# wen-yuan-zhang/Fast-Learning-NeRF

Measured on AMD Instinct MI355X. Metric: training rays/sec (Lego-like 800x800, 64+128 samples) + PSNR@N-iters, higher is better.
Workload: dtype f32; 1 GPU; nerf-ours Lego full 800x800 (BASELINE configs[1]), SURVEY 8(d) throughput protocol: 4096 uniformly drawn rays per GPU per step, 64+128 samples, use_viewdirs, white_bkgd, perturb=1, U[0,1) targets, random-init nets, leaf-error table on, fp32-width bf16x6 kernels, plain backward (FASTNERF_COMPACT=0); parallelism=dp1, math_mode=bf16x6, backward=plain (every sample)

## Files before the change

### fast-learning-nerf_amd/_lib.py

```python
import ctypes as C
import os

import torch

HERE = os.path.dirname(os.path.abspath(__file__))
LIB_PATH = os.environ.get('FASTNERF_LIB') or os.path.join(HERE, 'libfastnerf.so')

P = C.c_void_p
I = C.c_int
L = C.c_int64
F = C.c_float
D = C.c_double
U64 = C.c_uint64



class StepArgs(C.Structure):
    _fields_ = (
        [('n', L)] + [(k, P) for k in ('rays_o', 'rays_d', 'target', 't_rand', 'u', 'noise0', 'noise1')]
        + [('seed0', U64), ('seed1', U64), ('leaf_tag', P), ('table', P), ('net_floats', L)]
        + [(k, P) for k in ('params', 'grads', 'adam_m', 'adam_v', 'packed_fwd_c', 'packed_bwd_c', 'packed_fwd_f', 'packed_bwd_f',
                            'rays11', 'z0', 'raw0', 'act0', 'rgb0', 'disp0', 'acc0', 'w0', 'depth0',
                            'z1', 'z_samples', 'z_std', 'raw1', 'act1', 'rgb1', 'disp1', 'acc1', 'w1', 'depth1',
                            'g_rgb', 'g_rgb0', 'loss2', 'draw_ws', 'act_ws', 'dact_ws', 'partial_ws', 'live_ws', 'counts')]
        + [(k, D) for k in ('focal', 'lr', 'beta1', 'beta2', 'eps')]
        + [(k, F) for k in ('near_plane', 'far_plane', 'grad_scale')]
        + [(k, I) for k in ('math_mode', 'N_samples', 'N_importance', 'lindisp', 'perturb', 'white_bkgd', 'ndc', 'H', 'W', 'live',
                            'fwd_flags', 'max_leaves', 'adam_t')]
        + [('occ', P), ('occ_counts', P)])


class MapGrads(C.Structure):
    _fields_ = [(k, P) for k in ('g_disp1', 'g_acc1', 'g_depth1', 'g_disp0', 'g_acc0', 'g_depth0')]


class StepAux(C.Structure):
    _fields_ = ([(k, P) for k in ('depth_target', 'depth_weight', 'acc_target', 'acc_weight', 'g_depth1', 'g_acc1', 'g_depth0',
                                  'g_acc0', 'loss4')]
                + [('lambda_depth', F), ('lambda_acc', F)])


class OccGrid(C.Structure):
    _fields_ = [('words', P), ('lo', F * 3), ('inv', F * 3), ('n', C.c_int32 * 3), ('outside_occupied', C.c_int32)]


OCC_MAX_LEVELS = 8


class OccCascade(C.Structure):
    _fields_ = [('levels', C.c_int32), ('reserved', C.c_int32), ('level', OccGrid * OCC_MAX_LEVELS)]


STEP_FORWARD, STEP_BWD_FINE, STEP_BWD_COARSE, STEP_UPDATE = 1, 2, 4, 8

SIGNATURES = {
    'fastnerf_version': (I, []),
    'fastnerf_last_error': (C.c_char_p, []),
    'fastnerf_device_cus': (I, []),
    'fastnerf_x6_pair_launches': (L, []),
    'fastnerf_gen_rays': (I, [I, I, F, F, F, F, P, P, P, P]),
    'fastnerf_gen_rays_pixels': (I, [L, P, P, F, F, F, F, P, P, P]),
    'fastnerf_ndc_rays': (I, [L, I, I, D, F, P, P, P, P, P]),
    'fastnerf_pack_rays': (I, [L, P, P, F, F, I, I, I, D, P, P]),
    'fastnerf_sample_coarse': (I, [L, I, P, I, I, P, U64, P, P]),
    'fastnerf_posenc': (I, [L, I, P, P, P]),
    'fastnerf_mlp_pack': (I, [P, P, P, P]),
    'fastnerf_mlp_fwd': (I, [L, I, P, P, P, P, P, P, P]),
    'fastnerf_mlp_bwd_partial_floats': (L, []),
    'fastnerf_mlp_bwd': (I, [L, I, P, P, P, P, P, P, P, P]),
    'fastnerf_raw2outputs_fwd': (I, [L, I, P, P, P, P, I, P, P, P, P, P, P]),
    'fastnerf_raw2outputs_bwd': (I, [L, I, P, P, P, P, I, P, P, P]),
    'fastnerf_raw2outputs_bwd_full': (I, [L, I, P, P, P, P, I, P, P, P, P, P, P, P, P, P]),
    'fastnerf_sample_pdf_merge': (I, [L, I, I, P, P, I, P, U64, P, P, P, P]),
    'fastnerf_sample_pdf': (I, [L, I, I, P, P, I, P, U64, P, P]),
    'fastnerf_mse_leafmax': (I, [L, P, P, P, F, P, P, P, P, I, P, P]),
    'fastnerf_aux_loss': (I, [L] + [P] * 8 + [F, F, F] + [P] * 5 + [P]),
    'fastnerf_adam_step': (I, [L, P, P, P, P, D, D, D, D, I, P]),
    'fastnerf_net_floats': (L, [I, I]),
    'fastnerf_mlp_act_floats': (L, [I, L]),
    'fastnerf_mlp_pack_ex': (I, [I, P, P, P, P]),
    'fastnerf_mlp_fwd_ex': (I, [I, L, I, P, P, P, P, P, P, P]),
    'fastnerf_mlp_bwd_ex': (I, [I, L, I, P, P, P, P, P, P, P, P]),
    'fastnerf_mlp_bf16_floats': (L, [I, I, L]),
    'fastnerf_mlp_bf16_partial_floats': (L, []),
    'fastnerf_mlp_bf16_pack': (I, [I, P, P, P, P]),
    'fastnerf_mlp_bf16_fwd': (I, [I, L, I, P, P, P, P, P, P, P]),
    'fastnerf_mlp_bf16_bwd': (I, [I, L, I, P, P, P, P, P, P, P, P]),
    'fastnerf_render_rays_fwd': (I, [I, L, I, I, P, I, I, I, I, P, P, P, P, U64, U64, P, P, P, P] + [P] * 18 + [P]),
    'fastnerf_render_rays_fwd_ex': (I, [I, L, I, I, P, I, I, I, I, P, P, P, P, U64, U64, P, P, P, P] + [P] * 18 + [I, P]),
    'fastnerf_mlp_bf16_fwd_flags': (I, [I, L, I, P, P, P, P, P, I, P]),
    'fastnerf_mlp_fwd_flags_ex': (I, [I, L, I, P, P, P, P, P, I, P]),
    'fastnerf_render_rays_bwd': (I, [I, L, I, I, P, I] + [P] * 20),
    'fastnerf_render_rays_bwd_maps': (I, [I, L, I, I, P, I] + [P] * 19 + [P] * 4 + [C.POINTER(MapGrads), P]),
    'fastnerf_pp_intersect_sphere': (I, [L, P, P, P, P]),
    'fastnerf_pp_fg_depths': (I, [L, I, F, P, I, P, U64, P, P]),
    'fastnerf_pp_sample_pdf_merge': (I, [L, I, I, P, P, I, P, U64, P, P, P]),
    'fastnerf_pp_perturb_samples': (I, [L, I, P, P, U64, P, P]),
    'fastnerf_pp_sample_pdf': (I, [L, I, I, P, P, I, P, U64, P, P]),
    'fastnerf_pp_depth2pts_outside': (I, [L, I, P, P, P, P, P, P]),
    'fastnerf_pp_composite_fwd': (I, [L, I, I, P, P, P, P, P, P, P, P, P]),
    'fastnerf_pp_composite_bwd': (I, [L, I, I, P, P, P, P, P, P, P, P]),
    'fastnerf_pp_gen_rays': (I, [I, I, P, P, P, P, P]),
    'fastnerf_leaf_sumcount': (I, [L, P, P, P, I, P, P, P]),
    'fastnerf_tree_adjust_mean': (L, [P, P, P, I, D]),
    'fastnerf_tree_create': (P, [I, I, I, I]),
    'fastnerf_tree_destroy': (None, [P]),
    'fastnerf_tree_num_leaves': (I, [P, I]),
    'fastnerf_tree_max_leaves': (I, [P]),
    'fastnerf_tree_min_area': (D, [P, I]),
    'fastnerf_tree_get_leaves': (I, [P, I, P]),
    'fastnerf_tree_set_leaves': (I, [P, I, I, P, D]),
    'fastnerf_tree_leaf_plan': (I, [P, I, D, I, P]),
    'fastnerf_tree_adjust': (L, [P, P, I, D]),
    'fastnerf_tree_epoch_plan': (L, [P, D, I, P, P]),
    'fastnerf_epoch_rays': (I, [L, I, P, P, P, P, I, I, I, F, F, F, F, U64, I] + [P] * 10 + [P]),
    'fastnerf_epoch_rays_shard': (I, [L, I, P, P, P, P, I, I, I, F, F, F, F, U64, I] + [P] * 5 + [L, I, I] + [P] * 5 + [P]),
    'fastnerf_epoch_shard_rows': (L, [L, L, I, I]),
    'fastnerf_gauss_noise': (I, [L, F, U64, P, P]),
    'fastnerf_compact_ws_ints': (L, [L]),
    'fastnerf_compact_live': (I, [L, P, P, P, P, P]),
    'fastnerf_mlp_bf16_fwd_live': (I, [I, L, I, P, P, P, P, P, P, P, P]),
    'fastnerf_mlp_bf16_bwd_live': (I, [I, L, I, P, P, P, P, P, P, P, P, P, P]),
    'fastnerf_mlp_fwd_live_ex': (I, [I, L, I, P, P, P, P, P, P, P, P]),
    'fastnerf_mlp_bwd_live_ex': (I, [I, L, I, P, P, P, P, P, P, P, P, P, P]),
    'fastnerf_render_rays_bwd_live': (I, [I, L, I, I, P, I] + [P] * 22 + [P]),
    'fastnerf_render_rays_bwd_live_maps': (I, [I, L, I, I, P, I] + [P] * 22 + [P] * 4 + [C.POINTER(MapGrads), P]),
    'fastnerf_mlp_x6_packed_floats': (L, [I, I]),
    'fastnerf_mlp_x6_pack': (I, [I, P, P, P, P]),
    'fastnerf_mlp_fold_offset': (L, [I, I]),
    'fastnerf_mlp_x6_fwd': (I, [I, L, I, P, P, P, P, P, P, I, P]),
    'fastnerf_mlp_x6_bwd': (I, [I, L, I, P, P, P, P, P, P, P, P]),
    'fastnerf_mlp_x6_fwd_live': (I, [I, L, I, P, P, P, P, P, P, P, P]),
    'fastnerf_mlp_x6_bwd_live': (I, [I, L, I, P, P, P, P, P, P, P, P, P, P]),
    'fastnerf_step_args_size': (L, []),
    'fastnerf_train_step': (I, [C.POINTER(StepArgs), I, P]),
    'fastnerf_step_aux_size': (L, []),
    'fastnerf_train_step_aux': (I, [C.POINTER(StepArgs), C.POINTER(StepAux), I, P]),
    'fastnerf_comm_unique_id': (I, [C.c_char_p]),
    'fastnerf_comm_init': (I, [C.POINTER(P), C.c_char_p, I, I]),
    'fastnerf_comm_destroy': (I, [P]),
    'fastnerf_allreduce_grads': (I, [P, P, L, C.c_float, P]),
    'fastnerf_allreduce_leaf_table': (I, [P, P, L, P]),
    'fastnerf_allreduce_leaf_sumcount': (I, [P, P, P, L, P]),
    'fastnerf_leaf_table_reset': (I, [P, L, P]),
    'fastnerf_leaf_table_read': (I, [P, P, L, P]),
    'fastnerf_grid_points': (I, [L, L, P, L, P, L, P, L, P, P]),
    'fastnerf_grid_sigma': (I, [L, P, P, P]),
    'fastnerf_mc_ws_bytes': (L, [L, L, L]),
    'fastnerf_mc_count': (I, [P, L, L, L, F, P, P, P]),
    'fastnerf_mc_emit': (I, [P, L, L, L, F, P, P, P, P]),
    'fastnerf_mc_tables': (I, [P, P]),
    'fastnerf_occ_words': (L, [L, L, L]),
    'fastnerf_occ_build': (I, [P, L, L, L, F, I, P, P, P]),
    'fastnerf_occ_from_mask': (I, [P, L, L, L, P, P]),
    'fastnerf_occ_query': (I, [C.POINTER(OccGrid), L, P, P, P]),
    'fastnerf_occ_classify': (I, [C.POINTER(OccGrid), L, I, P, P, P, P, P, P, P]),
    'fastnerf_occ_query_cascade': (I, [C.POINTER(OccCascade), L, P, P, P]),
    'fastnerf_occ_classify_cascade': (I, [C.POINTER(OccCascade), L, I, P, P, P, P, P, P, P]),
    'fastnerf_occ_cell_points': (I, [C.POINTER(OccGrid), L, L, U64, P, P]),
    'fastnerf_occ_update': (I, [P, P, L, L, L, L, L, F, F, I, P, P, P, P]),
    'fastnerf_mlp_fwd_list_ex': (I, [I, L, I, P, P, P, P, P, P, P, I, P]),
    'fastnerf_mlp_bf16_fwd_list': (I, [I, L, I, P, P, P, P, P, P, P, I, P]),
    'fastnerf_mlp_x6_fwd_list': (I, [I, L, I, P, P, P, P, P, P, P, I, P]),
    'fastnerf_render_rays_fwd_occ': (I, [I, L, I, I, P, I, I, I, I, P, P, U64, U64, P, P, P, P, C.POINTER(OccGrid), P, P] + [P] * 16 + [I, P]),
    'fastnerf_render_rays_fwd_occ_cascade': (I, [I, L, I, I, P, I, I, I, I, P, P, U64, U64, P, P, P, P, C.POINTER(OccCascade), P, P] + [P] * 16 + [I, P]),
    'fastnerf_ert_classify': (I, [C.POINTER(OccGrid), C.POINTER(OccCascade), L, I, I, I, P, P, P, F, P, P, P, P, P]),
    'fastnerf_ert_advance': (I, [L, I, I, I, P, P, P, I, P, P, P, P]),
    'fastnerf_render_rays_fwd_ert': (I, [I, L, I, I, P, I, I, I, I, P, P, U64, U64, P, P, P, P, C.POINTER(OccGrid), C.POINTER(OccCascade), F, I,
                                         P, P, P] + [P] * 16 + [I, P]),
    'fastnerf_mlp_sigma_grad_ws_floats': (L, [I, L]),
    'fastnerf_mlp_sigma_grad': (I, [I, I, L, I, P, P, P, P, P, P, P, P, P]),
    'fastnerf_ray_grad_ws_floats': (L, [I, L, I]),
    'fastnerf_ray_grad': (I, [I, I, L, I, P, P, P, P, P, P, P, P, P, I, P, P]),
}

_lib = None


def lib():
    global _lib
    if _lib is None:
        if not os.path.exists(LIB_PATH):
            raise RuntimeError(
                f'{LIB_PATH} not found: build it with `python -c "import __graft_entry__ as g; g.build()"` '
                '(the HIP path has no CPU fallback)')
        l = C.CDLL(LIB_PATH)
        for name, (res, args) in SIGNATURES.items():
            fn = getattr(l, name)
            fn.restype = res
            fn.argtypes = args
        if l.fastnerf_step_args_size() != C.sizeof(StepArgs):
            raise RuntimeError('fn_step_args: the ctypes mirror does not match the library (stale libfastnerf.so?)')
        if l.fastnerf_step_aux_size() != C.sizeof(StepAux):
            raise RuntimeError('fn_step_aux: the ctypes mirror does not match the library (stale libfastnerf.so?)')
        _lib = l
    return _lib


def check(rc, what):
    if rc is None or rc < 0:
        msg = lib().fastnerf_last_error()
        raise RuntimeError(f'{what} failed ({rc}): {msg.decode() if msg else "?"}')
    return rc


def ptr(t):
    if t is None:
        return None
    assert t.is_contiguous(), 'tensor must be contiguous'
    return t.data_ptr()


def stream():
    return torch.cuda.current_stream().cuda_stream


def require_gpu(*tensors):
    for t in tensors:
        if t is not None and not t.is_cuda:
            raise RuntimeError('fastnerf ops run on the GPU only (no CPU fallback): got a CPU tensor')
```

### fast-learning-nerf_amd/csrc/composite.hip

```cpp
#include "common.h"

#define WAVE 64
#define MAXC 8

__device__ __forceinline__ float wave_sum(float v) {
#pragma unroll
  for (int o = 32; o > 0; o >>= 1) v += __shfl_xor(v, o, WAVE);
  return v;
}

__device__ __forceinline__ float wave_scan_mul(float v, int lane) {
#pragma unroll
  for (int o = 1; o < WAVE; o <<= 1) {
    float t = __shfl_up(v, o, WAVE);
    if (lane >= o) v *= t;
  }
  return v;
}
__device__ __forceinline__ float wave_suffix_add(float v, int lane) {
#pragma unroll
  for (int o = 1; o < WAVE; o <<= 1) {
    const float t = __shfl_down(v, o, WAVE);
    if (lane + o < WAVE) v += t;
  }
  const float above = __shfl_down(v, 1, WAVE);
  return lane == WAVE - 1 ? 0.0f : above;
}

__device__ __forceinline__ void wave_suffix_add2(float& a, float& b, int lane) {
#pragma unroll
  for (int o = 1; o < WAVE; o <<= 1) {
    const float ta = __shfl_down(a, o, WAVE), tb = __shfl_down(b, o, WAVE);
    if (lane + o < WAVE) {
      a += ta;
      b += tb;
    }
  }
  const float aa = __shfl_down(a, 1, WAVE), ab = __shfl_down(b, 1, WAVE);
  a = lane == WAVE - 1 ? 0.0f : aa;
  b = lane == WAVE - 1 ? 0.0f : ab;
}

__device__ __forceinline__ float sigmoidf(float x) { return 1.0f / (1.0f + expf(-x)); }

struct SampleVals {
  float alpha, t, dist, z, sig;
  float c[3];
};

struct CompCfg {
  int act_abs;
  float eps;
  int last_mode;
  int use_dnorm;
  int flip;
};
__device__ __forceinline__ CompCfg nerf_cfg() { return CompCfg{0, 1e-10f, 0, 1, 0}; }

template <bool WITH_RGB>
__device__ __forceinline__ void eval_chunk(int S, int C, int lane, const float* __restrict__ raw,
                                           const float* __restrict__ z, const float* __restrict__ noise, float dnorm,
                                           SampleVals v[MAXC], int& cnt, const CompCfg cfg, float far) {
  const int s0 = lane * C;
  cnt = 0;
#pragma unroll
  for (int j = 0; j < MAXC; ++j) {
    if (j >= C) break;
    const int s = s0 + j;
    if (s >= S) break;
    const float4 r = *reinterpret_cast<const float4*>(raw + (int64_t)s * 4);
    const float zs = cfg.flip ? z[S - 1 - s] : z[s];
    float dist;
    if (s + 1 < S) {
      const float zn = cfg.flip ? z[S - 2 - s] : z[s + 1];
      dist = cfg.flip ? fsub(zs, zn) : fsub(zn, zs);
    } else {
      dist = cfg.last_mode ? fsub(far, zs) : 1e10f;
    }
    if (cfg.use_dnorm) dist = fmul(dist, dnorm);
    float sig = r.w;
    if (noise) sig = fadd(sig, noise[s]);
    const float rs = cfg.act_abs ? fabsf(sig) : fmaxf(sig, 0.0f);
    const float alpha = fsub(1.0f, expf(-fmul(rs, dist)));
    v[j].alpha = alpha;
    v[j].t = fadd(fsub(1.0f, alpha), cfg.eps);
    v[j].dist = dist;
    v[j].z = zs;
    v[j].sig = sig;
    if (WITH_RGB) {
      v[j].c[0] = sigmoidf(r.x);
      v[j].c[1] = sigmoidf(r.y);
      v[j].c[2] = sigmoidf(r.z);
    }
    cnt = j + 1;
  }
}

__global__ void __launch_bounds__(256) raw2outputs_fwd_kernel(int64_t n, int S, const float* __restrict__ raw,
                                                               const float* __restrict__ z,
                                                               const float* __restrict__ rays,
                                                               const float* __restrict__ noise, int white,
                                                               float* __restrict__ rgb_map, float* __restrict__ disp,
                                                               float* __restrict__ acc, float* __restrict__ weights,
                                                               float* __restrict__ depth, const CompCfg cfg,
                                                               const float* __restrict__ far,
                                                               float* __restrict__ lambda) {
  const int lane = threadIdx.x & 63;
  const int C = (S + WAVE - 1) / WAVE;
  const int64_t wave0 = ((int64_t)blockIdx.x * blockDim.x + threadIdx.x) >> 6;
  const int64_t nwaves = ((int64_t)gridDim.x * blockDim.x) >> 6;
  for (int64_t r = wave0; r < n; r += nwaves) {
    const float* rr = rays + r * 11;
    const float dnorm = sqrtf(fadd(fadd(fmul(rr[3], rr[3]), fmul(rr[4], rr[4])), fmul(rr[5], rr[5])));
    SampleVals v[MAXC];
    int cnt;
    eval_chunk<true>(S, C, lane, raw + r * S * 4, z + r * S, noise ? noise + r * S : nullptr, dnorm, v, cnt, cfg,
                     far ? far[r] : 0.f);
    float prod = 1.0f;
#pragma unroll
    for (int j = 0; j < MAXC; ++j)
      if (j < cnt) prod *= v[j].t;
    const float incl = wave_scan_mul(prod, lane);
    float T = __shfl_up(incl, 1, WAVE);
    if (lane == 0) T = 1.0f;
    if (lambda) {
      const float tot = __shfl(incl, WAVE - 1, WAVE);
      if (lane == 0) lambda[r] = tot;
    }
    float sr = 0.f, sg = 0.f, sb = 0.f, sd = 0.f, sa = 0.f;
#pragma unroll
    for (int j = 0; j < MAXC; ++j) {
      if (j < cnt) {
        const float w = v[j].alpha * T;
        if (weights) weights[r * S + lane * C + j] = w;
        sr += w * v[j].c[0];
        sg += w * v[j].c[1];
        sb += w * v[j].c[2];
        sd += w * v[j].z;
        sa += w;
        T *= v[j].t;
      }
    }
    sr = wave_sum(sr); sg = wave_sum(sg); sb = wave_sum(sb); sd = wave_sum(sd); sa = wave_sum(sa);
    if (lane == 0) {
      if (white) {
        const float bg = fsub(1.0f, sa);
        sr = fadd(sr, bg); sg = fadd(sg, bg); sb = fadd(sb, bg);
      }
      rgb_map[r * 3 + 0] = sr; rgb_map[r * 3 + 1] = sg; rgb_map[r * 3 + 2] = sb;
      if (disp) {
        const float q = sd / sa;
        disp[r] = (q != q) ? q : 1.0f / fmaxf(1e-10f, q);
      }
      if (acc) acc[r] = sa;
      if (depth) depth[r] = sd;
    }
  }
}

__global__ void __launch_bounds__(256) raw2outputs_bwd_kernel(int64_t n, int S, const float* __restrict__ raw,
                                                               const float* __restrict__ z,
                                                               const float* __restrict__ rays,
                                                               const float* __restrict__ noise, int white,
                                                               const float* __restrict__ g_rgb,
                                                               float* __restrict__ draw, const CompCfg cfg,
                                                               const float* __restrict__ far,
                                                               const float* __restrict__ g_lambda) {
  const int lane = threadIdx.x & 63;
  const int C = (S + WAVE - 1) / WAVE;
  const int64_t wave0 = ((int64_t)blockIdx.x * blockDim.x + threadIdx.x) >> 6;
  const int64_t nwaves = ((int64_t)gridDim.x * blockDim.x) >> 6;
  for (int64_t r = wave0; r < n; r += nwaves) {
    const float* rr = rays + r * 11;
    const float dnorm = sqrtf(fadd(fadd(fmul(rr[3], rr[3]), fmul(rr[4], rr[4])), fmul(rr[5], rr[5])));
    const float g0 = g_rgb[r * 3], g1 = g_rgb[r * 3 + 1], g2 = g_rgb[r * 3 + 2];
    const float gbg = white ? (g0 + g1 + g2) : 0.0f;
    SampleVals v[MAXC];
    int cnt;
    eval_chunk<true>(S, C, lane, raw + r * S * 4, z + r * S, noise ? noise + r * S : nullptr, dnorm, v, cnt, cfg,
                     far ? far[r] : 0.f);
    float prod = 1.0f;
#pragma unroll
    for (int j = 0; j < MAXC; ++j)
      if (j < cnt) prod *= v[j].t;
    const float incl = wave_scan_mul(prod, lane);
    float T0 = __shfl_up(incl, 1, WAVE);
    if (lane == 0) T0 = 1.0f;
    const float lam_term = g_lambda ? g_lambda[r] * __shfl(incl, WAVE - 1, WAVE) : 0.0f;
    float w[MAXC], G[MAXC], Tj[MAXC];
    float gw_chunk = 0.f;
    float T = T0;
#pragma unroll
    for (int j = 0; j < MAXC; ++j) {
      if (j < cnt) {
        Tj[j] = T;
        w[j] = v[j].alpha * T;
        G[j] = g0 * v[j].c[0] + g1 * v[j].c[1] + g2 * v[j].c[2] - gbg;
        gw_chunk += G[j] * w[j];
        T *= v[j].t;
      }
    }
    float suffix = wave_suffix_add(gw_chunk, lane);
    float4 out[MAXC];
#pragma unroll
    for (int j = MAXC - 1; j >= 0; --j) {
      if (j < cnt) {
        const float dalpha = G[j] * Tj[j] - (suffix + lam_term) / v[j].t;
        const float dact = dalpha * v[j].dist * (1.0f - v[j].alpha);
        const float dsig = cfg.act_abs ? ((v[j].sig > 0.0f) ? dact : ((v[j].sig < 0.0f) ? -dact : 0.0f))
                                       : ((v[j].sig > 0.0f) ? dact : 0.0f);
        out[j].x = g0 * w[j] * v[j].c[0] * (1.0f - v[j].c[0]);
        out[j].y = g1 * w[j] * v[j].c[1] * (1.0f - v[j].c[1]);
        out[j].z = g2 * w[j] * v[j].c[2] * (1.0f - v[j].c[2]);
        out[j].w = dsig;
        suffix += G[j] * w[j];
      }
    }
#pragma unroll
    for (int j = 0; j < MAXC; ++j)
      if (j < cnt) *reinterpret_cast<float4*>(draw + (r * S + lane * C + j) * 4) = out[j];
  }
}

__global__ void __launch_bounds__(256) raw2outputs_bwd_full_kernel(
    int64_t n, int S, const float* __restrict__ raw, const float* __restrict__ z, const float* __restrict__ rays,
    const float* __restrict__ noise, int white, const float* __restrict__ acc_f, const float* __restrict__ depth_f,
    const float* __restrict__ g_rgb, const float* __restrict__ g_disp, const float* __restrict__ g_acc,
    const float* __restrict__ g_w, const float* __restrict__ g_depth, float* __restrict__ draw) {
  const CompCfg cfg = nerf_cfg();
  const int lane = threadIdx.x & 63;
  const int C = (S + WAVE - 1) / WAVE;
  const int64_t wave0 = ((int64_t)blockIdx.x * blockDim.x + threadIdx.x) >> 6;
  const int64_t nwaves = ((int64_t)gridDim.x * blockDim.x) >> 6;
  const bool ray_terms = g_acc || g_depth || g_disp;
  for (int64_t r = wave0; r < n; r += nwaves) {
    const float* rr = rays + r * 11;
    const float dnorm = sqrtf(fadd(fadd(fmul(rr[3], rr[3]), fmul(rr[4], rr[4])), fmul(rr[5], rr[5])));
    const float g0 = g_rgb ? g_rgb[r * 3] : 0.0f, g1 = g_rgb ? g_rgb[r * 3 + 1] : 0.0f, g2 = g_rgb ? g_rgb[r * 3 + 2] : 0.0f;
    const float gbg = white ? (g0 + g1 + g2) : 0.0f;
    const float ga0 = g_acc ? g_acc[r] : 0.0f, gd0 = g_depth ? g_depth[r] : 0.0f;
    float ga = ga0, gd = gd0;
    float kd = 0.0f;
    if (g_disp) {
      const float gq = g_disp[r];
      if (gq != 0.0f) {
        const float a = acc_f[r], dep = depth_f[r], q = dep / a;
        if (q != q) {
          ga = q; gd = q;
        } else if (q >= 1e-10f) {
          const float disp = 1.0f / q;
          const float gqe = q == 1e-10f ? 0.5f * gq : gq;
          const float k = gqe * disp / a;
          ga += k;
          gd -= k * disp;
          kd = gqe / dep / dep;
        }
      }
    }
    const float zlast = ray_terms ? z[r * S + S - 1] : 0.0f;
    SampleVals v[MAXC];
    int cnt;
    eval_chunk<true>(S, C, lane, raw + r * S * 4, z + r * S, noise ? noise + r * S : nullptr, dnorm, v, cnt, cfg, 0.f);
    float prod = 1.0f;
#pragma unroll
    for (int j = 0; j < MAXC; ++j)
      if (j < cnt) prod *= v[j].t;
    const float incl = wave_scan_mul(prod, lane);
    float T0 = __shfl_up(incl, 1, WAVE);
    if (lane == 0) T0 = 1.0f;
    float zprev = 0.0f;
#pragma unroll
    for (int j = 0; j < MAXC; ++j)
      if (j < cnt) zprev = v[j].z;
    zprev = __shfl_up(zprev, 1, WAVE);
    float w[MAXC], G[MAXC], Tj[MAXC], h[MAXC];
    float gw_chunk = 0.f, h_chunk = 0.f, dlast = 0.f;
    float T = T0;
#pragma unroll
    for (int j = 0; j < MAXC; ++j) {
      if (j < cnt) {
        Tj[j] = T;
        w[j] = v[j].alpha * T;
        G[j] = g0 * v[j].c[0] + g1 * v[j].c[1] + g2 * v[j].c[2] - gbg;
        if (g_w) G[j] = G[j] + g_w[r * S + lane * C + j];
        gw_chunk += G[j] * w[j];
        if (ray_terms) {
          const float dz = v[j].z - zprev;
          h[j] = (ga * cfg.eps + gd * (dz + cfg.eps * v[j].z)) * T;
          h_chunk += h[j];
          zprev = v[j].z;
          dlast += w[j] * (zlast - v[j].z);
        }
        T *= v[j].t;
      }
    }
    float suffix = gw_chunk, suffix_h = h_chunk, end_term = 0.f;
    if (ray_terms)
      wave_suffix_add2(suffix, suffix_h, lane);
    else
      suffix = wave_suffix_add(gw_chunk, lane);
    if (ray_terms) {
      float coef = ga + gd * zlast;
      if (kd != 0.0f) coef = (ga0 + gd0 * zlast) - kd * wave_sum(dlast);
      end_term = coef * __shfl(incl, WAVE - 1, WAVE);
    }
    float4 out[MAXC];
#pragma unroll
    for (int j = MAXC - 1; j >= 0; --j) {
      if (j < cnt) {
        float dalpha;
        if (ray_terms) {
          dalpha = G[j] * Tj[j] - (suffix - (end_term - suffix_h)) / v[j].t;
          suffix_h += h[j];
        } else {
          dalpha = G[j] * Tj[j] - (suffix + 0.0f) / v[j].t;
        }
        const float dact = dalpha * v[j].dist * (1.0f - v[j].alpha);
        out[j].x = g0 * w[j] * v[j].c[0] * (1.0f - v[j].c[0]);
        out[j].y = g1 * w[j] * v[j].c[1] * (1.0f - v[j].c[1]);
        out[j].z = g2 * w[j] * v[j].c[2] * (1.0f - v[j].c[2]);
        out[j].w = (v[j].sig > 0.0f) ? dact : 0.0f;
        suffix += G[j] * w[j];
      }
    }
#pragma unroll
    for (int j = 0; j < MAXC; ++j)
      if (j < cnt) *reinterpret_cast<float4*>(draw + (r * S + lane * C + j) * 4) = out[j];
  }
}

__device__ __forceinline__ int lower_bound_f(const float* a, int n, float x) {
  int lo = 0, hi = n;
  while (lo < hi) {
    const int mid = (lo + hi) >> 1;
    if (a[mid] < x) lo = mid + 1; else hi = mid;
  }
  return lo;
}
__device__ __forceinline__ int upper_bound_f(const float* a, int n, float x) {
  int lo = 0, hi = n;
  while (lo < hi) {
    const int mid = (lo + hi) >> 1;
    if (a[mid] <= x) lo = mid + 1; else hi = mid;
  }
  return lo;
}

__global__ void __launch_bounds__(256) sample_pdf_merge_kernel(int64_t n, int S, int Ni, int NP, int bins_mode,
                                                                int variant,
                                                                const float* __restrict__ z,
                                                                const float* __restrict__ weights, int det,
                                                                const float* __restrict__ u_in, uint64_t seed,
                                                                float* __restrict__ z_out,
                                                                float* __restrict__ z_samples,
                                                                float* __restrict__ z_std) {
  extern __shared__ __attribute__((aligned(16))) float smem[];
  const int lane = threadIdx.x & 63;
  const int wib = threadIdx.x >> 6;
  const int per_wave = 3 * S + NP;
  float* zs = smem + wib * per_wave;
  float* cdf = zs + S;
  float* bins = cdf + S;
  float* smp = bins + S;
  const int M = S - 1;
  const int NW = S - 2;
  const int CW = (NW + WAVE - 1) / WAVE;
  const int64_t wave0 = ((int64_t)blockIdx.x * blockDim.x + threadIdx.x) >> 6;
  const int64_t nwaves = ((int64_t)gridDim.x * blockDim.x) >> 6;
  for (int64_t r = wave0; r < n; r += nwaves) {
    if (bins_mode) {
      for (int k = lane; k < M; k += WAVE) bins[k] = z[r * M + k];
    } else {
      for (int s = lane; s < S; s += WAVE) zs[s] = z[r * S + s];
      __builtin_amdgcn_wave_barrier();
      for (int k = lane; k < M; k += WAVE) bins[k] = fmul(0.5f, fadd(zs[k + 1], zs[k]));
    }
    float wl[MAXC];
    double csum = 0.0;
#pragma unroll
    for (int j = 0; j < MAXC; ++j) {
      const int k = lane * CW + j;
      wl[j] = (j < CW && k < NW) ? fadd(bins_mode ? weights[r * NW + k] : weights[r * S + k + 1], variant ? 1e-6f : 1e-5f) : 0.f;
      csum += (double)wl[j];
    }
    double totd = csum;
#pragma unroll
    for (int o = 32; o > 0; o >>= 1) totd += __shfl_xor(totd, o, WAVE);
    const float tot = (float)totd;
    double run = 0.0;
#pragma unroll
    for (int j = 0; j < MAXC; ++j) {
      wl[j] = wl[j] / tot;
      run += (double)wl[j];
    }
    double incl = run;
#pragma unroll
    for (int o = 1; o < WAVE; o <<= 1) {
      const double t = __shfl_up(incl, o, WAVE);
      if (lane >= o) incl += t;
    }
    double base = incl - run;
    if (lane == 0) cdf[0] = 0.f;
#pragma unroll
    for (int j = 0; j < MAXC; ++j) {
      const int k = lane * CW + j;
      if (j < CW && k < NW) {
        base += (double)wl[j];
        cdf[k + 1] = (float)base;
      }
    }
    __builtin_amdgcn_wave_barrier();
    float lsum = 0.f;
    for (int i = lane; i < NP; i += WAVE) {
      float smpl = __builtin_inff();
      if (i < Ni) {
        float u;
        if (u_in) {
          u = u_in[r * Ni + i];
        } else if (det) {
          const float step = 1.0f / (float)(Ni - 1);
          u = (Ni == 1) ? 0.0f : ((i < Ni / 2) ? fmul(step, (float)i) : fsub(1.0f, fmul(step, (float)(Ni - 1 - i))));
        } else {
          uint32_t o[4];
          const uint64_t idx = (uint64_t)r * Ni + i;
          philox4x32((uint32_t)idx, (uint32_t)(idx >> 32), 0x70646673u, 0u, (uint32_t)seed, (uint32_t)(seed >> 32), o);
          u = u01(o[0]);
        }
        const int inds = upper_bound_f(cdf, variant ? NW : M, u);
        const int below = inds - 1 > 0 ? inds - 1 : 0;
        const int above = inds < M - 1 ? inds : M - 1;
        const float c0 = cdf[below], c1 = cdf[above];
        const float b0 = bins[below], b1 = bins[above];
        float denom = fsub(c1, c0);
        if (denom < (variant ? 1e-6f : 1e-5f)) denom = 1.0f;
        const float t = fsub(u, c0) / denom;
        smpl = variant ? fadd(b0, fmul(t, fadd(fsub(b1, b0), 1e-6f))) : fadd(b0, fmul(t, fsub(b1, b0)));
        if (z_samples) z_samples[r * Ni + i] = smpl;
        lsum += smpl;
      }
      smp[i] = smpl;
    }
    if (z_std) {
      const float mean = wave_sum(lsum) / (float)Ni;
      float lv = 0.f;
      for (int i = lane; i < Ni; i += WAVE) {
        const float d = smp[i] - mean;
        lv += d * d;
      }
      const float var = wave_sum(lv) / (float)Ni;
      if (lane == 0) z_std[r] = sqrtf(var);
    }
    __builtin_amdgcn_wave_barrier();
    if (bins_mode) continue;
    for (int k = 2; k <= NP; k <<= 1) {
      for (int j = k >> 1; j > 0; j >>= 1) {
        for (int i = lane; i < NP; i += WAVE) {
          const int ixj = i ^ j;
          if (ixj > i) {
            const float a = smp[i], b = smp[ixj];
            const bool up = ((i & k) == 0);
            if ((a > b) == up) { smp[i] = b; smp[ixj] = a; }
          }
        }
        __builtin_amdgcn_wave_barrier();
      }
    }
    const int So = S + Ni;
    for (int s = lane; s < S; s += WAVE) {
      const float x = zs[s];
      z_out[r * So + s + lower_bound_f(smp, Ni, x)] = x;
    }
    for (int i = lane; i < Ni; i += WAVE) {
      const float x = smp[i];
      z_out[r * So + i + upper_bound_f(zs, S, x)] = x;
    }
    __builtin_amdgcn_wave_barrier();
  }
}

static inline int grid_waves(int64_t n) {
  int64_t g = (n + 3) / 4;
  if (g < 1) g = 1;
  if (g > 4096) g = 4096;
  return (int)g;
}

extern "C" int fastnerf_raw2outputs_fwd(int64_t n, int S, const float* raw, const float* z, const float* rays11,
                                        const float* noise, int white_bkgd, float* rgb_map, float* disp, float* acc,
                                        float* weights, float* depth, fn_stream_t stream) {
  FN_CHECK_ARG(n >= 0 && S >= 1 && S <= WAVE * MAXC, "n>=0, 1<=S<=512");
  FN_CHECK_ARG(n == 0 || (raw && z && rays11 && rgb_map), "null pointer");
  if (n == 0) return 0;
  hipLaunchKernelGGL(raw2outputs_fwd_kernel, dim3(grid_waves(n)), dim3(256), 0, fn::S(stream), n, S, raw, z, rays11,
                     noise, white_bkgd, rgb_map, disp, acc, weights, depth, CompCfg{0, 1e-10f, 0, 1, 0},
                     (const float*)nullptr, (float*)nullptr);
  FN_LAUNCH_CHECK();
  return 0;
}

extern "C" int fastnerf_raw2outputs_bwd(int64_t n, int S, const float* raw, const float* z, const float* rays11,
                                        const float* noise, int white_bkgd, const float* g_rgb, float* draw,
                                        fn_stream_t stream) {
  FN_CHECK_ARG(n >= 0 && S >= 1 && S <= WAVE * MAXC, "n>=0, 1<=S<=512");
  FN_CHECK_ARG(n == 0 || (raw && z && rays11 && g_rgb && draw), "null pointer");
  if (n == 0) return 0;
  hipLaunchKernelGGL(raw2outputs_bwd_kernel, dim3(grid_waves(n)), dim3(256), 0, fn::S(stream), n, S, raw, z, rays11,
                     noise, white_bkgd, g_rgb, draw, CompCfg{0, 1e-10f, 0, 1, 0}, (const float*)nullptr,
                     (const float*)nullptr);
  FN_LAUNCH_CHECK();
  return 0;
}

extern "C" int fastnerf_raw2outputs_bwd_full(int64_t n, int S, const float* raw, const float* z, const float* rays11,
                                             const float* noise, int white_bkgd, const float* acc, const float* depth,
                                             const float* g_rgb, const float* g_disp, const float* g_acc, const float* g_w,
                                             const float* g_depth, float* draw, fn_stream_t stream) {
  FN_CHECK_ARG(n >= 0 && S >= 1 && S <= WAVE * MAXC, "n>=0, 1<=S<=512");
  FN_CHECK_ARG(n == 0 || (raw && z && rays11 && draw && (!g_disp || (acc && depth))), "null pointer");
  if (n == 0) return 0;
  hipLaunchKernelGGL(raw2outputs_bwd_full_kernel, dim3(grid_waves(n)), dim3(256), 0, fn::S(stream), n, S, raw, z, rays11,
                     noise, white_bkgd, acc, depth, g_rgb, g_disp, g_acc, g_w, g_depth, draw);
  FN_LAUNCH_CHECK();
  return 0;
}

__global__ void __launch_bounds__(256) ert_advance_kernel(int64_t n, int S, int s0, int s1, const float* __restrict__ raw,
                                                           const float* __restrict__ z, const float* __restrict__ rays, int first,
                                                           float* __restrict__ trans, const int* __restrict__ seg_count,
                                                           int* __restrict__ total) {
  const int lane = threadIdx.x & 63;
  const int W = s1 - s0;
  const int C = (W + WAVE - 1) / WAVE;
  const int64_t wave0 = ((int64_t)blockIdx.x * blockDim.x + threadIdx.x) >> 6;
  const int64_t nwaves = ((int64_t)gridDim.x * blockDim.x) >> 6;
  const CompCfg cfg = nerf_cfg();
  for (int64_t r = wave0; r < n; r += nwaves) {
    const float* rr = rays + r * 11;
    const float dnorm = sqrtf(fadd(fadd(fmul(rr[3], rr[3]), fmul(rr[4], rr[4])), fmul(rr[5], rr[5])));
    SampleVals v[MAXC];
    int cnt;
    eval_chunk<false>(S - s0 < W + 1 ? S - s0 : W + 1, C, lane, raw + (r * S + s0) * 4, z + r * S + s0, nullptr, dnorm, v, cnt, cfg, 0.f);
    float prod = 1.0f;
#pragma unroll
    for (int j = 0; j < MAXC; ++j)
      if (j < cnt && lane * C + j < W) prod *= v[j].t;
#pragma unroll
    for (int o = 32; o > 0; o >>= 1) prod *= __shfl_xor(prod, o, WAVE);
    if (lane == 0) trans[r] = first ? prod : trans[r] * prod;
  }
  if (total && blockIdx.x == 0 && threadIdx.x == 0) {
    total[0] = (first ? 0 : total[0]) + seg_count[0];
    total[1] = (int)(n * S);
  }
}

extern "C" int fastnerf_ert_advance(int64_t n, int S, int s0, int s1, const float* raw, const float* z, const float* rays11, int first,
                                    float* trans, const int32_t* seg_count, int32_t* total, fn_stream_t stream) {
  FN_CHECK_ARG(n > 0 && S >= 1 && S <= WAVE * MAXC && n * (int64_t)S < ((int64_t)1 << 31), "n > 0, 1 <= S <= 512, n * S < 2^31");
  FN_CHECK_ARG(s0 >= 0 && s0 < s1 && s1 <= S, "0 <= s0 < s1 <= S");
  FN_CHECK_ARG(raw && z && rays11 && trans && (!total || seg_count), "non-null pointers (seg_count with total)");
  hipLaunchKernelGGL(ert_advance_kernel, dim3(grid_waves(n)), dim3(256), 0, fn::S(stream), n, S, s0, s1, raw, z, rays11, first ? 1 : 0,
                     trans, seg_count, total);
  FN_LAUNCH_CHECK();
  return 0;
}

extern "C" int fastnerf_sample_pdf_merge(int64_t n, int S, int Ni, const float* z, const float* weights, int det,
                                         const float* u, uint64_t seed, float* z_out, float* z_samples, float* z_std,
                                         fn_stream_t stream) {
  FN_CHECK_ARG(n >= 0 && S >= 3 && S <= WAVE * MAXC && Ni >= 1 && Ni <= 1024, "n>=0, 3<=S<=512, 1<=Ni<=1024");
  FN_CHECK_ARG(n == 0 || (z && weights && z_out), "null pointer");
  if (n == 0) return 0;
  int NP = 1;
  while (NP < Ni) NP <<= 1;
  const size_t lds = (size_t)4 * (3 * S + NP) * sizeof(float);
  hipLaunchKernelGGL(sample_pdf_merge_kernel, dim3(grid_waves(n)), dim3(256), lds, fn::S(stream), n, S, Ni, NP, 0, 0, z,
                     weights, det, u, seed, z_out, z_samples, z_std);
  FN_LAUNCH_CHECK();
  return 0;
}

extern "C" int fastnerf_sample_pdf(int64_t n, int M, int Ni, const float* bins, const float* weights, int det,
                                   const float* u, uint64_t seed, float* samples, fn_stream_t stream) {
  FN_CHECK_ARG(n >= 0 && M >= 2 && M + 1 <= WAVE * MAXC && Ni >= 1 && Ni <= 1024, "n>=0, 2<=M<=511, 1<=Ni<=1024");
  FN_CHECK_ARG(n == 0 || (bins && weights && samples), "null pointer");
  if (n == 0) return 0;
  int NP = 1;
  while (NP < Ni) NP <<= 1;
  const int S = M + 1;
  const size_t lds = (size_t)4 * (3 * S + NP) * sizeof(float);
  hipLaunchKernelGGL(sample_pdf_merge_kernel, dim3(grid_waves(n)), dim3(256), lds, fn::S(stream), n, S, Ni, NP, 1, 0,
                     bins, weights, det, u, seed, (float*)nullptr, samples, (float*)nullptr);
  FN_LAUNCH_CHECK();
  return 0;
}


static inline CompCfg pp_cfg(int part) { return part == 0 ? CompCfg{1, 1e-6f, 1, 1, 0} : CompCfg{1, 1e-6f, 0, 0, 1}; }

extern "C" int fastnerf_pp_composite_fwd(int64_t n, int S, int part, const float* raw, const float* z,
                                         const float* rays11, const float* fg_far, float* rgb_map, float* weights,
                                         float* depth, float* lambda, fn_stream_t stream) {
  FN_CHECK_ARG(n >= 0 && S >= 2 && S <= WAVE * MAXC && (part == 0 || part == 1), "n>=0, 2<=S<=512, part in {0,1}");
  FN_CHECK_ARG(n == 0 || (raw && z && rays11 && rgb_map && (part == 1 || fg_far)), "null pointer");
  if (n == 0) return 0;
  hipLaunchKernelGGL(raw2outputs_fwd_kernel, dim3(grid_waves(n)), dim3(256), 0, fn::S(stream), n, S, raw, z, rays11,
                     (const float*)nullptr, 0, rgb_map, (float*)nullptr, (float*)nullptr, weights, depth, pp_cfg(part),
                     part == 0 ? fg_far : (const float*)nullptr, part == 0 ? lambda : (float*)nullptr);
  FN_LAUNCH_CHECK();
  return 0;
}

extern "C" int fastnerf_pp_composite_bwd(int64_t n, int S, int part, const float* raw, const float* z,
                                         const float* rays11, const float* fg_far, const float* g_rgb,
                                         const float* g_lambda, float* draw, fn_stream_t stream) {
  FN_CHECK_ARG(n >= 0 && S >= 2 && S <= WAVE * MAXC && (part == 0 || part == 1), "n>=0, 2<=S<=512, part in {0,1}");
  FN_CHECK_ARG(n == 0 || (raw && z && rays11 && g_rgb && draw && (part == 1 || fg_far)), "null pointer");
  if (n == 0) return 0;
  hipLaunchKernelGGL(raw2outputs_bwd_kernel, dim3(grid_waves(n)), dim3(256), 0, fn::S(stream), n, S, raw, z, rays11,
                     (const float*)nullptr, 0, g_rgb, draw, pp_cfg(part), part == 0 ? fg_far : (const float*)nullptr,
                     part == 0 ? g_lambda : (const float*)nullptr);
  FN_LAUNCH_CHECK();
  return 0;
}

extern "C" int fastnerf_pp_sample_pdf_merge(int64_t n, int S, int Ni, const float* z, const float* weights, int det,
                                            const float* u, uint64_t seed, float* z_out, float* z_samples,
                                            fn_stream_t stream) {
  FN_CHECK_ARG(n >= 0 && S >= 3 && S <= WAVE * MAXC && Ni >= 1 && Ni <= 1024, "n>=0, 3<=S<=512, 1<=Ni<=1024");
  FN_CHECK_ARG(n == 0 || (z && weights && z_out), "null pointer");
  if (n == 0) return 0;
  int NP = 1;
  while (NP < Ni) NP <<= 1;
  const size_t lds = (size_t)4 * (3 * S + NP) * sizeof(float);
  hipLaunchKernelGGL(sample_pdf_merge_kernel, dim3(grid_waves(n)), dim3(256), lds, fn::S(stream), n, S, Ni, NP, 0, 1, z,
                     weights, det, u, seed, z_out, z_samples, (float*)nullptr);
  FN_LAUNCH_CHECK();
  return 0;
}

extern "C" int fastnerf_pp_sample_pdf(int64_t n, int M, int Ni, const float* bins, const float* weights, int det, const float* u,
                                      uint64_t seed, float* samples, fn_stream_t stream) {
  FN_CHECK_ARG(n >= 0 && M >= 2 && M + 1 <= WAVE * MAXC && Ni >= 1 && Ni <= 1024, "n>=0, 2<=M<=511, 1<=Ni<=1024");
  FN_CHECK_ARG(n == 0 || (bins && weights && samples), "null pointer");
  if (n == 0) return 0;
  int NP = 1;
  while (NP < Ni) NP <<= 1;
  const int S = M + 1;
  const size_t lds = (size_t)4 * (3 * S + NP) * sizeof(float);
  hipLaunchKernelGGL(sample_pdf_merge_kernel, dim3(grid_waves(n)), dim3(256), lds, fn::S(stream), n, S, Ni, NP, 1, 1,
                     bins, weights, det, u, seed, (float*)nullptr, samples, (float*)nullptr);
  FN_LAUNCH_CHECK();
  return 0;
}
```

### fast-learning-nerf_amd/csrc/dw_pair.h

```cpp
#pragma once
#include <stdint.h>

struct DwJobDesc { int NO, KI, bias, rank1; };
inline DwJobDesc dw_job(int j, int pe_pad) {
  switch (j) {
    case 0: return {256, pe_pad, 1, 0};
    case 8: return {256, pe_pad, 0, 0};
    case 9: return {256, 256, 1, 1};
    case 10: return {128, 256, 1, 0};
    case 11: return {128, 32, 0, 0};
    default: return {256, 256, 1, 0};
  }
}
#define HEAD_MAX_WG 1024
inline int64_t dw_job_floats(int j, int pe_pad) {
  const DwJobDesc d = dw_job(j, pe_pad);
  return (int64_t)d.NO * d.KI + (d.bias ? d.NO : 0) + (d.rank1 ? d.KI : 0);
}
inline int64_t dw_job_base(int j, int ncu, int pe_pad) {
  static const int order[12] = {0, 8, 1, 2, 3, 4, 5, 6, 7, 9, 10, 11};
  int64_t o = 0;
  for (int i = 0; i < 12; ++i) {
    if (order[i] == j) return o;
    o += dw_job_floats(order[i], pe_pad) * ncu;
  }
  return o;
}
inline int64_t dw_partial_floats(int ncu) { return dw_job_base(12, ncu, 96) + (int64_t)HEAD_MAX_WG * 388; }

#define DW_TRUNK_JOBS 7
struct DwTrunk {
  const float* dY[DW_TRUNK_JOBS];
  const float* X[DW_TRUNK_JOBS];
  float* pw[DW_TRUNK_JOBS];
  float* pb[DW_TRUNK_JOBS];
};

struct RedSeg {
  int64_t src;
  int64_t wg_stride;
  int64_t dst;
  int nwg, rows, cols, ld, valid_cols;
  int dyn;
  int sc_cols;
  int64_t sc_dst;
};
#define MAX_SEGS 32
struct RedTable {
  RedSeg s[MAX_SEGS];
  int n;
};

struct DwDeferred {
  DwTrunk J;
  RedTable T;
  int64_t P, g_off;
  const float* params;
  float *partial, *grads;
  int kind;
};
```

### fast-learning-nerf_amd/csrc/mlp_bwd_dw.hip

```cpp
#include "mlp_common.h"
#include "dw_pair.h"
#include <atomic>

int fn_launch_dx(int mm, int grid, hipStream_t st, int64_t P, const float* draw, const float* act, const float* params, const float* packed_bwd,
                 float* dact, const NetLayout& L, const int* live_idx, const int* live_cnt, float* headws);

#define DW_MT 32

template <int WO, int WI, int TO, int TI, bool BIAS, bool RANK1>
__global__ void __launch_bounds__(WO * WI * 64, WO * WI / 4)
mlp_bwd_dw_kernel(int64_t P, const float* __restrict__ dY, int ldy, const float* __restrict__ X, int ldx,
                  const float* __restrict__ draw , float* __restrict__ partial_w,
                  float* __restrict__ partial_b, float* __restrict__ partial_r, const int* __restrict__ live_idx,
                  const int* __restrict__ live_cnt) {
  if (live_idx) P = (int64_t)__builtin_amdgcn_readfirstlane(*live_cnt);
  constexpr int NO = WO * TO * 32, KI = WI * TI * 32;
  constexpr int NTD = WO * WI * 64;
  constexpr int STAGE = DW_MT * (NO + KI) + DW_MT;
  extern __shared__ __attribute__((aligned(16))) float smem[];
  const int tid = threadIdx.x;
  const int lane = tid & 63;
  const int wave = __builtin_amdgcn_readfirstlane(tid >> 6);
  const int wo = wave / WI, wi = wave % WI;
  const int64_t ntile_all = (P + DW_MT - 1) / DW_MT;
  const int64_t per = (ntile_all + gridDim.x - 1) / gridDim.x;
  const int64_t t0 = blockIdx.x * per;
  int64_t t1 = t0 + per;
  if (t1 > ntile_all) t1 = ntile_all;

  f32x16 acc[TO][TI];
#pragma unroll
  for (int a = 0; a < TO; ++a)
#pragma unroll
    for (int b = 0; b < TI; ++b)
#pragma unroll
      for (int r = 0; r < 16; ++r) acc[a][b][r] = 0.f;
  float bsum = 0.f, rsum = 0.f;

  constexpr int YV = (DW_MT * NO / 4 + NTD - 1) / NTD;
  constexpr int XV = (DW_MT * KI / 4 + NTD - 1) / NTD;
  static_assert(DW_MT * NO % 4 == 0 && DW_MT * KI % 4 == 0 && NO <= NTD && KI <= NTD, "stage split");
  float4 ry[YV], rx[XV];
  float rda = 0.f;

  auto load_stage = [&](int64_t t) {
    const int64_t pbase = t * DW_MT;
#pragma unroll
    for (int i = 0; i < YV; ++i) {
      const int e = (i * NTD + tid) * 4;
      const int m = e / NO, c = e % NO;
      const int64_t p = pbase + m;
      ry[i] = (e < DW_MT * NO && p < P) ? *reinterpret_cast<const float4*>(dY + p * ldy + c)
                                        : make_float4(0.f, 0.f, 0.f, 0.f);
    }
#pragma unroll
    for (int i = 0; i < XV; ++i) {
      const int e = (i * NTD + tid) * 4;
      const int m = e / KI, c = e % KI;
      const int64_t p = pbase + m;
      rx[i] = (e < DW_MT * KI && p < P) ? *reinterpret_cast<const float4*>(X + p * ldx + c)
                                        : make_float4(0.f, 0.f, 0.f, 0.f);
    }
    if (RANK1 && tid < DW_MT) {
      const int64_t p = pbase + tid;
      rda = (p < P) ? draw[(live_idx ? (int64_t)live_idx[p] : p) * 4 + 3] : 0.f;
    }
  };
  auto store_stage = [&](float* st) {
#pragma unroll
    for (int i = 0; i < YV; ++i)
      if ((i * NTD + tid) * 4 < DW_MT * NO) *reinterpret_cast<float4*>(st + (i * NTD + tid) * 4) = ry[i];
#pragma unroll
    for (int i = 0; i < XV; ++i)
      if ((i * NTD + tid) * 4 < DW_MT * KI) *reinterpret_cast<float4*>(st + DW_MT * NO + (i * NTD + tid) * 4) = rx[i];
    if (RANK1 && tid < DW_MT) st[DW_MT * (NO + KI) + tid] = rda;
  };

  if (t0 < t1) {
    load_stage(t0);
    store_stage(smem);
  }
  __syncthreads();
  for (int64_t t = t0; t < t1; ++t) {
    float* cur = smem + ((t - t0) & 1) * STAGE;
    float* nxt = smem + (((t - t0) & 1) ^ 1) * STAGE;
    if (t + 1 < t1) load_stage(t + 1);
    const float* Ys = cur;
    const float* Xs = cur + DW_MT * NO;
    {
      float fa0[TO], fb0[TI], fa1[TO], fb1[TI];
      auto ldf = [&](float (&a)[TO], float (&b)[TI], int k2) {
        const int m = k2 * 2 + (lane >> 5);
#pragma unroll
        for (int i = 0; i < TO; ++i) a[i] = Ys[m * NO + (wo * TO + i) * 32 + (lane & 31)];
#pragma unroll
        for (int j = 0; j < TI; ++j) b[j] = Xs[m * KI + (wi * TI + j) * 32 + (lane & 31)];
      };
      auto mm = [&](const float (&a)[TO], const float (&b)[TI]) {
#pragma unroll
        for (int i = 0; i < TO; ++i)
#pragma unroll
          for (int j = 0; j < TI; ++j) acc[i][j] = mfma(a[i], b[j], acc[i][j]);
      };
      ldf(fa0, fb0, 0);
#pragma unroll
      for (int k2 = 0; k2 < DW_MT / 2; k2 += 2) {
        ldf(fa1, fb1, k2 + 1);
        __builtin_amdgcn_sched_barrier(0);
        mm(fa0, fb0);
        __builtin_amdgcn_sched_barrier(0);
        if (k2 + 2 < DW_MT / 2) ldf(fa0, fb0, k2 + 2);
        __builtin_amdgcn_sched_barrier(0);
        mm(fa1, fb1);
        __builtin_amdgcn_sched_barrier(0);
      }
    }
    if (BIAS) {
      if (tid < NO) {
#pragma unroll 8
        for (int m = 0; m < DW_MT; ++m) bsum += Ys[m * NO + tid];
      }
    }
    if (RANK1) {
      if (tid < KI) {
        const float* da = cur + DW_MT * (NO + KI);
#pragma unroll 8
        for (int m = 0; m < DW_MT; ++m) rsum = fmaf(da[m], Xs[m * KI + tid], rsum);
      }
    }
    if (t + 1 < t1) store_stage(nxt);
    __syncthreads();
  }
  float* pw = partial_w + (int64_t)blockIdx.x * NO * KI;
#pragma unroll
  for (int i = 0; i < TO; ++i)
#pragma unroll
    for (int j = 0; j < TI; ++j)
#pragma unroll
      for (int r = 0; r < 16; ++r) {
        const int o = (wo * TO + i) * 32 + crow(r, lane);
        const int c = (wi * TI + j) * 32 + (lane & 31);
        pw[(int64_t)o * KI + c] = acc[i][j][r];
      }
  if (BIAS && tid < NO) partial_b[(int64_t)blockIdx.x * NO + tid] = bsum;
  if (RANK1 && tid < KI) partial_r[(int64_t)blockIdx.x * KI + tid] = rsum;
}

template <int WO, int WI, int TO, int TI, bool BIAS, bool RANK1, int CTI2 = 0, int CTO2 = 0>
__device__ __forceinline__ void dw6_body(const int64_t P, const float* __restrict__ dY, const float* __restrict__ X,
                                         const float* __restrict__ draw, float* __restrict__ partial_w, float* __restrict__ partial_b,
                                         float* __restrict__ partial_r, const int* __restrict__ live_idx,
                                         const float* __restrict__ X2, const float* __restrict__ dY2, const int wg, const int nwg) {
  constexpr int NO = WO * TO * 32, KI = WI * TI * 32;
  constexpr int CTO = WO * TO, CTI = WI * TI, NTILE = CTO + CTI;
  constexpr int NW = WO * WI;
  constexpr int TPW = (NTILE + NW - 1) / NW;
  extern __shared__ __attribute__((aligned(16))) uint4 S6[];
  float* const DA = reinterpret_cast<float*>(S6 + 2 * NTILE * 192);
  const int tid = threadIdx.x;
  const int lane = tid & 63;
  const int wave = __builtin_amdgcn_readfirstlane(tid >> 6);
  const int wo = wave / WI, wi = wave % WI;
  const int64_t nq_all = (P + 15) / 16;
  const int64_t per = (nq_all + nwg - 1) / nwg;
  const int64_t q0 = wg * per;
  int64_t q1 = q0 + per;
  if (q1 > nq_all) q1 = nq_all;
  const int nq = (int)(q1 - q0);
  int64_t Pend = q1 * 16;
  if (Pend > P) Pend = P;

  f32x16 acc[TO][TI];
#pragma unroll
  for (int a = 0; a < TO; ++a)
#pragma unroll
    for (int b = 0; b < TI; ++b)
#pragma unroll
      for (int r = 0; r < 16; ++r) acc[a][b][r] = 0.f;
  float ssum[TPW];
#pragma unroll
  for (int k = 0; k < TPW; ++k) ssum[k] = 0.f;

  constexpr int CTI1 = CTI - CTI2, KI1 = CTI1 * 32, KI2 = CTI2 * 32;
  constexpr int CTO1 = CTO - CTO2, NO1 = CTO1 * 32, NO2 = CTO2 * 32;
  static_assert(!(RANK1 && CTO2) && !(CTI2 && CTO2), "one second tensor per job");
  const float* tsrc[TPW];
  bool tisy[TPW], tis2[TPW];
  constexpr bool KNOWN = (CTO % NW == 0) && (NTILE % NW == 0) && CTO2 == 0 && CTI2 == 0;
#pragma unroll
  for (int k = 0; k < TPW; ++k) {
    const int t = k * NW + wave;
    tisy[k] = KNOWN ? (k * NW < CTO) : (t < CTO);
    tis2[k] = (CTI2 > 0 && t >= CTO + CTI1) || (CTO2 > 0 && t >= CTO1 && t < CTO);
    tsrc[k] = tisy[k] ? (tis2[k] ? dY2 + q0 * (16 * NO2) + (t - CTO1) * 32 : dY + q0 * (16 * NO1) + t * 32)
                      : (tis2[k] ? X2 + q0 * (16 * KI2) + (t - CTO - CTI1) * 32 : X + q0 * (16 * KI1) + (t - CTO) * 32);
  }
  const int relmax = (int)(Pend - q0 * 16) - 1;
  const int col = lane & 31, half8 = (lane >> 5) * 8;
  const unsigned boffy = (unsigned)(half8 * NO1 + col) * 4u, boffy2 = (unsigned)(half8 * NO2 + col) * 4u,
                 boffx = (unsigned)(half8 * KI1 + col) * 4u, boffx2 = (unsigned)(half8 * KI2 + col) * 4u;
  struct Raw { float v[TPW][8]; };
  auto ldb = [](const float* base, unsigned byte_off) __attribute__((always_inline)) -> float {
    return *reinterpret_cast<const float*>(reinterpret_cast<const char*>(base) + byte_off);
  };
  auto load_raw = [&](Raw& r, int st, auto whole) __attribute__((always_inline)) {
    if constexpr (decltype(whole)::value) {
#pragma unroll
      for (int k = 0; k < TPW; ++k) {
        const int t = k * NW + wave;
        if (NTILE % NW == 0 || t < NTILE) {
          if (tisy[k] && CTO2 > 0 && tis2[k]) {
            const float* b = tsrc[k] + (int64_t)st * (16 * NO2);
#pragma unroll
            for (int e = 0; e < 8; ++e) r.v[k][e] = ldb(b, boffy2 + (unsigned)(e * NO2 * 4));
          } else if (tisy[k]) {
            const float* b = tsrc[k] + (int64_t)st * (16 * NO1);
#pragma unroll
            for (int e = 0; e < 8; ++e) r.v[k][e] = ldb(b, boffy + (unsigned)(e * NO1 * 4));
          } else if (CTI2 > 0 && tis2[k]) {
            const float* b = tsrc[k] + (int64_t)st * (16 * KI2);
#pragma unroll
            for (int e = 0; e < 8; ++e) r.v[k][e] = ldb(b, boffx2 + (unsigned)(e * KI2 * 4));
          } else {
            const float* b = tsrc[k] + (int64_t)st * (16 * KI1);
#pragma unroll
            for (int e = 0; e < 8; ++e) r.v[k][e] = ldb(b, boffx + (unsigned)(e * KI1 * 4));
          }
        }
      }
    } else {
      unsigned row[8];
#pragma unroll
      for (int e = 0; e < 8; ++e) { const int rr = st * 16 + half8 + e; row[e] = (unsigned)(rr < relmax ? rr : relmax); }
#pragma unroll
      for (int k = 0; k < TPW; ++k) {
        const int t = k * NW + wave;
        if (NTILE % NW == 0 || t < NTILE) {
#pragma unroll
          for (int e = 0; e < 8; ++e)
            r.v[k][e] = ldb(tsrc[k], (row[e] * (unsigned)(tisy[k] ? (tis2[k] ? NO2 : NO1) : (tis2[k] ? KI2 : KI1)) + (unsigned)col) * 4u);
        }
      }
    }
  };
  const int* const li = live_idx ? live_idx : reinterpret_cast<const int*>(draw);
  auto load_ix = [&](int st) __attribute__((always_inline)) -> int64_t {
    const int rr = st * 16 + (lane & 15);
    const int64_t p = q0 * 16 + (rr < relmax ? rr : relmax);
    const int64_t lv = li[p];
    return live_idx ? lv : p;
  };
  auto split_store = [&](const Raw& r, int buf, int st, auto whole) __attribute__((always_inline)) {
    const int nv = relmax + 1 - (st * 16 + half8);
#pragma unroll
    for (int k = 0; k < TPW; ++k) {
      const int t = k * NW + wave;
      if (NTILE % NW == 0 || t < NTILE) {
        float v[8];
#pragma unroll
        for (int e = 0; e < 8; ++e) v[e] = r.v[k][e];
        if constexpr (!decltype(whole)::value) {
#pragma unroll
          for (int e = 0; e < 8; ++e) v[e] = e < nv ? v[e] : 0.f;
        }
        uint4 h, m, l;
        uint4* d = S6 + ((buf * NTILE + t) * 3) * 64 + lane;
        split3_frag(make_float4(v[0], v[1], v[2], v[3]), make_float4(v[4], v[5], v[6], v[7]), h, m, l);
        d[0] = h; d[64] = m; d[128] = l;
        if (BIAS && (KNOWN ? (k * NW < CTO) : (t < CTO1))) ssum[k] += ((v[0] + v[1]) + (v[2] + v[3])) + ((v[4] + v[5]) + (v[6] + v[7]));
        if (RANK1 && (KNOWN ? (k * NW >= CTO) : (t >= CTO && t < CTO + CTI1))) {
          const float4 d0 = *reinterpret_cast<const float4*>(DA + (st & 1) * 16 + half8);
          const float4 d1 = *reinterpret_cast<const float4*>(DA + (st & 1) * 16 + half8 + 4);
          const float da[8] = {d0.x, d0.y, d0.z, d0.w, d1.x, d1.y, d1.z, d1.w};
#pragma unroll
          for (int e = 0; e < 8; ++e) ssum[k] = fmaf(da[e], v[e], ssum[k]);
        }
      }
    }
  };
  auto multiply = [&](int buf) __attribute__((always_inline)) {
    const uint4* Sb = S6 + buf * NTILE * 192 + lane;
    uint4 a[TO][3];
#pragma unroll
    for (int i = 0; i < TO; ++i)
#pragma unroll
      for (int pl = 0; pl < 3; ++pl) a[i][pl] = Sb[((wo * TO + i) * 3 + pl) * 64];
    constexpr int PA[6] = {2, 0, 1, 1, 0, 0}, PB[6] = {0, 2, 1, 0, 1, 0};
    constexpr int JP = TI >= 2 ? 2 : 1;
#pragma unroll
    for (int j0 = 0; j0 < TI; j0 += JP) {
      uint4 b[JP][3];
#pragma unroll
      for (int jj = 0; jj < JP; ++jj)
#pragma unroll
        for (int pl = 0; pl < 3; ++pl)
          if (j0 + jj < TI) b[jj][pl] = Sb[((CTO + wi * TI + j0 + jj) * 3 + pl) * 64];
#pragma unroll
      for (int t = 0; t < 6; ++t)
#pragma unroll
        for (int jj = 0; jj < JP; ++jj)
#pragma unroll
          for (int i = 0; i < TO; ++i)
            if (j0 + jj < TI) acc[i][j0 + jj] = mfma_bf16(a[i][PA[t]], b[jj][PB[t]], acc[i][j0 + jj]);
    }
  };
  auto publish = [&]() __attribute__((always_inline)) {
    asm volatile("s_waitcnt lgkmcnt(0)\n\ts_barrier" ::: "memory");
  };

  if (nq > 0) {
    constexpr std::true_type WHOLE{};
    constexpr std::false_type ANY{};
    Raw r0, r1;
    load_raw(r0, 0, ANY);
    load_raw(r1, 1, ANY);
    float dr0 = 0.f, dr1 = 0.f;
    int64_t ix0 = 0, ix1 = 0;
    const bool da_lane = RANK1 && wave == 0 && lane < 16;
    if (da_lane) {
      DA[lane] = draw[load_ix(0) * 4 + 3];
      DA[16 + lane] = draw[load_ix(1) * 4 + 3];
      dr0 = draw[load_ix(2) * 4 + 3];
      dr1 = draw[load_ix(3) * 4 + 3];
      ix0 = load_ix(4);
      ix1 = load_ix(5);
    }
    if (RANK1) publish();
    split_store(r0, 0, 0, ANY);
    load_raw(r0, 2, ANY);
    publish();
    auto mix = [&](auto sync) __attribute__((always_inline)) {
      if constexpr (KNOWN && !RANK1) interleave6<0, TO * TI * 6, TPW * 4 * 11 + (BIAS ? 8 : 0), decltype(sync)::value>();
    };
    auto pair = [&](int d, auto whole) __attribute__((always_inline)) {
      const int st = 2 * d;
      if (da_lane) { DA[lane] = dr0; dr0 = draw[ix0 * 4 + 3]; ix0 = load_ix(st + 6); }
      multiply(0);
      split_store(r1, 1, st + 1, whole);
      mix(std::integral_constant<int, 1>{});
      load_raw(r1, st + 3, whole);
      publish();
      if (da_lane) { DA[16 + lane] = dr1; dr1 = draw[ix1 * 4 + 3]; ix1 = load_ix(st + 7); }
      multiply(1);
      split_store(r0, 0, st + 2, whole);
      mix(std::integral_constant<int, 2>{});
      load_raw(r0, st + 4, whole);
      publish();
    };
    const int n2 = (nq + 1) / 2;
    const int nwhole = (relmax + 1) / 16;
    int dmain = nwhole >= 5 ? (nwhole - 3) / 2 : 0;
    if (dmain > n2) dmain = n2;
#pragma unroll 1
    for (int d = 0; d < dmain; ++d) pair(d, WHOLE);
#pragma unroll 1
    for (int d = dmain; d < n2; ++d) pair(d, ANY);
  }
  float* pw = partial_w + (int64_t)wg * NO * KI;
#pragma unroll
  for (int i = 0; i < TO; ++i)
#pragma unroll
    for (int j = 0; j < TI; ++j)
#pragma unroll
      for (int r = 0; r < 16; ++r) {
        const int o = (wo * TO + i) * 32 + crow(r, lane);
        const int c = (wi * TI + j) * 32 + (lane & 31);
        pw[(int64_t)o * KI + c] = acc[i][j][r];
      }
  if (BIAS || RANK1) {
#pragma unroll
    for (int k = 0; k < TPW; ++k) {
      const int t = k * NW + wave;
      if (NTILE % NW == 0 || t < NTILE) {
        const float sv = ssum[k] + __shfl_xor(ssum[k], 32, 64);
        if (lane < 32) {
          if (BIAS && t < CTO1) partial_b[(int64_t)wg * NO1 + t * 32 + lane] = sv;
          if (RANK1 && t >= CTO && t < CTO + CTI1) partial_r[(int64_t)wg * KI1 + (t - CTO) * 32 + lane] = sv;
        }
      }
    }
  }
}

template <int WO, int WI, int TO, int TI, bool BIAS, bool RANK1, int CTI2 = 0, int CTO2 = 0>
__global__ void __launch_bounds__(WO * WI * 64, WO * WI / 4)
mlp_bwd_dw6_kernel(int64_t P, const float* __restrict__ dY, const float* __restrict__ X,
                   const float* __restrict__ draw, float* __restrict__ partial_w, float* __restrict__ partial_b,
                   float* __restrict__ partial_r, const int* __restrict__ live_idx, const int* __restrict__ live_cnt,
                   const float* __restrict__ X2 = nullptr, const float* __restrict__ dY2 = nullptr) {
  if (live_idx) P = (int64_t)__builtin_amdgcn_readfirstlane(*live_cnt);
  dw6_body<WO, WI, TO, TI, BIAS, RANK1, CTI2, CTO2>(P, dY, X, draw, partial_w, partial_b, partial_r, live_idx, X2, dY2, (int)blockIdx.x,
                                                    (int)gridDim.x);
}

#define DW_QMAX 256
__host__ __device__ static inline int dw_trunk_chunks(int64_t P, int ncu) {
  const int unit = ncu >= 8 ? ncu / 8 : 1;
  const int64_t nq = (P + 15) / 16;
  int64_t k = (nq + (int64_t)unit * DW_QMAX - 1) / ((int64_t)unit * DW_QMAX);
  k = k < 1 ? 1 : (k > 8 ? 8 : k);
  return unit * (int)k;
}
__global__ void __launch_bounds__(512, 2)
mlp_bwd_dw6_trunk_kernel(int64_t P, DwTrunk J, const int* __restrict__ live_idx, const int* __restrict__ live_cnt, int ncu) {
  if (live_idx) P = (int64_t)__builtin_amdgcn_readfirstlane(*live_cnt);
  const int nact = dw_trunk_chunks(P, ncu);
  if ((int)blockIdx.x >= nact) return;
  const int job = (int)blockIdx.y;
  dw6_body<4, 2, 2, 4, true, false>(P, J.dY[job], J.X[job], nullptr, J.pw[job], J.pb[job], nullptr, live_idx, nullptr, nullptr,
                                    (int)blockIdx.x, nact);
}

struct DwTrunkPair {
  DwTrunk J[2];
  int64_t P[2];
};
__global__ void __launch_bounds__(512, 2)
mlp_bwd_dw6_trunk_pair_kernel(DwTrunkPair A, int ncu) {
  const int c0 = dw_trunk_chunks(A.P[0], ncu);
  int b = (int)blockIdx.x;
  const int pass = b >= DW_TRUNK_JOBS * c0 ? 1 : 0;
  if (pass) b -= DW_TRUNK_JOBS * c0;
  const int64_t P = A.P[pass];
  const int nact = pass ? dw_trunk_chunks(P, ncu) : c0;
  const int job = b / nact;
  if (job >= DW_TRUNK_JOBS) return;
  const DwTrunk& J = A.J[pass];
  dw6_body<4, 2, 2, 4, true, false>(P, J.dY[job], J.X[job], nullptr, J.pw[job], J.pb[job], nullptr, nullptr, nullptr, nullptr, b - job * nact,
                                    nact);
}

__global__ void __launch_bounds__(128) head_grads_kernel(int64_t P, const float* __restrict__ draw,
                                                          const float* __restrict__ hv,
                                                          float* __restrict__ partial, const int* __restrict__ live_idx,
                                                          const int* __restrict__ live_cnt) {
  const int k = threadIdx.x;
  if (live_idx) P = *live_cnt;
  auto dptr = [&](int64_t q) { return draw + (live_idx ? (int64_t)live_idx[q] : q) * 4; };
  const int64_t per = (P + gridDim.x - 1) / gridDim.x;
  const int64_t pa = blockIdx.x * per;
  int64_t pb = pa + per;
  if (pb > P) pb = P;
  float s0 = 0.f, s1 = 0.f, s2 = 0.f, sb = 0.f;
  int64_t p = pa;
  constexpr int NF = 16;
  for (; p + NF <= pb; p += NF) {
    float4 d[NF];
    float h[NF];
#pragma unroll
    for (int i = 0; i < NF; ++i) {
      d[i] = *reinterpret_cast<const float4*>(dptr(p + i));
      h[i] = hv[(p + i) * 128 + k];
    }
#pragma unroll
    for (int i = 0; i < NF; ++i) {
      s0 = fmaf(d[i].x, h[i], s0); s1 = fmaf(d[i].y, h[i], s1); s2 = fmaf(d[i].z, h[i], s2);
      if (k < 4) sb += (k == 0) ? d[i].x : (k == 1) ? d[i].y : (k == 2) ? d[i].z : d[i].w;
    }
  }
  for (; p < pb; ++p) {
    const float4 d = *reinterpret_cast<const float4*>(dptr(p));
    const float h = hv[p * 128 + k];
    s0 = fmaf(d.x, h, s0); s1 = fmaf(d.y, h, s1); s2 = fmaf(d.z, h, s2);
    if (k < 4) sb += (k == 0) ? d.x : (k == 1) ? d.y : (k == 2) ? d.z : d.w;
  }
  float* o = partial + (int64_t)blockIdx.x * 388;
  o[k] = s0; o[128 + k] = s1; o[256 + k] = s2;
  if (k < 4) o[384 + k] = sb;
}

#define HEAD_ROWS 256
__host__ __device__ static inline int head_group(int64_t ntiles) {
  const int64_t g = (ntiles + HEAD_ROWS - 1) / HEAD_ROWS;
  return g < 1 ? 1 : (int)g;
}
__host__ __device__ static inline int head_rows(int64_t P) {
  const int64_t ntiles = (P + TM - 1) / TM;
  const int g = head_group(ntiles);
  return (int)((ntiles + g - 1) / g);
}
__global__ void __launch_bounds__(128) head_group_kernel(int64_t P, const float* __restrict__ ws, float* __restrict__ out,
                                                          const int* __restrict__ live_cnt) {
  if (live_cnt) P = (int64_t)*live_cnt;
  const int64_t ntiles = (P + TM - 1) / TM;
  const int g = head_group(ntiles);
  const int col = (int)blockIdx.y * 128 + (int)threadIdx.x;
  const int64_t t0 = (int64_t)blockIdx.x * g;
  if (t0 >= ntiles || col >= 388) return;
  const int n = (int)(ntiles - t0 < g ? ntiles - t0 : g);
  const float* src = ws + t0 * 388 + col;
  constexpr int NF = 16;
  float s = 0.f;
  int i = 0;
  for (; i + NF <= n; i += NF) {
    float v[NF];
#pragma unroll
    for (int j = 0; j < NF; ++j) v[j] = src[(int64_t)(i + j) * 388];
#pragma unroll
    for (int j = 0; j < NF; ++j) s += v[j];
  }
  for (; i < n; ++i) s += src[(int64_t)i * 388];
  out[(int64_t)blockIdx.x * 388 + col] = s;
}


__global__ void __launch_bounds__(256) reduce_all_kernel(RedTable tab, const float* __restrict__ partial, float* __restrict__ grads,
                                                          float* __restrict__ scratch, int64_t P, const int* __restrict__ live_cnt, int ncu) {
  RedSeg sg = tab.s[blockIdx.y];
  if (sg.dyn) {
    if (live_cnt) P = (int64_t)*live_cnt;
    const int n = sg.dyn == 2 ? head_rows(P) : dw_trunk_chunks(P, ncu);
    sg.nwg = n < sg.nwg ? n : sg.nwg;
  }
  const int64_t total = (int64_t)sg.rows * sg.cols;
  const float* src = partial + sg.src;
  for (int64_t e = blockIdx.x * (int64_t)blockDim.x + threadIdx.x; e < total; e += (int64_t)gridDim.x * blockDim.x) {
    const int r = (int)(e / sg.cols), c = (int)(e % sg.cols);
    if (c >= sg.valid_cols) continue;
    constexpr int RS = 16;
    float a[RS];
#pragma unroll
    for (int i = 0; i < RS; ++i) a[i] = 0.f;
    int w = 0;
    for (; w + RS <= sg.nwg; w += RS) {
#pragma unroll
      for (int i = 0; i < RS; ++i) a[i] += src[(int64_t)(w + i) * sg.wg_stride + e];
    }
#pragma unroll
    for (int i = 0; i < RS - 1; ++i)
      if (w + i < sg.nwg) a[i] += src[(int64_t)(w + i) * sg.wg_stride + e];
#pragma unroll
    for (int h = RS / 2; h >= 1; h >>= 1)
#pragma unroll
      for (int i = 0; i < h; ++i) a[i] += a[i + h];
    if (c < sg.sc_cols) scratch[sg.sc_dst + (int64_t)r * sg.sc_cols + c] = a[0];
    else grads[sg.dst + (int64_t)r * sg.ld + c] = a[0];
  }
}

__global__ void __launch_bounds__(256) unfold_kernel(const float* __restrict__ G, const float* __restrict__ params, float* __restrict__ grads,
                                                      int64_t VW, int64_t VB, int64_t FW, int64_t FB) {
  __shared__ double As[16][17], Bs[16][17];
  const int tx = threadIdx.x & 15, ty = threadIdx.x >> 4;
  const int b = blockIdx.x;
  if (b == 384) {
    const int i = threadIdx.x;
    double s = 0.0;
    for (int o = 0; o < 128; ++o) s = fma((double)params[VW + (int64_t)o * 283 + i], (double)grads[VB + o], s);
    grads[FB + i] = (float)s;
    return;
  }
  const bool wf = b < 256;
  const int r0 = wf ? (b >> 4) * 16 : ((b - 256) >> 4) * 16, c0 = (b & 15) * 16;
  const int K = wf ? 128 : 256;
  double s = 0.0;
  for (int k0 = 0; k0 < K; k0 += 16) {
    if (wf) {
      As[ty][tx] = (double)params[VW + (int64_t)(k0 + ty) * 283 + r0 + tx];
      Bs[ty][tx] = (double)G[(k0 + ty) * 256 + c0 + tx];
    } else {
      As[tx][ty] = (double)G[(r0 + ty) * 256 + k0 + tx];
      Bs[tx][ty] = (double)params[FW + (int64_t)(c0 + ty) * 256 + k0 + tx];
    }
    __syncthreads();
#pragma unroll
    for (int k = 0; k < 16; ++k) s = fma(As[k][ty], Bs[k][tx], s);
    __syncthreads();
  }
  if (wf) grads[FW + (int64_t)(r0 + ty) * 256 + c0 + tx] = (float)s;
  else grads[VW + (int64_t)(r0 + ty) * 283 + c0 + tx] = (float)fma((double)grads[VB + r0 + ty], (double)params[FB + c0 + tx], s);
}

extern "C" int64_t fastnerf_mlp_bwd_partial_floats(void) {
  return dw_partial_floats(fn::device_cus());
}

template <int WO, int WI, int TO, int TI, bool BIAS, bool RANK1, int MM = MM_F32, int CTI2 = 0, int CTO2 = 0>
static int launch_dw(int64_t P, const float* dY, int ldy, const float* X, int ldx, const float* draw, float* base,
                     int nwg, hipStream_t st, const int* live_idx = nullptr, const int* live_cnt = nullptr,
                     const float* X2 = nullptr, const float* dY2 = nullptr, float* pr_at = nullptr) {
  constexpr int NO = WO * TO * 32, KI = WI * TI * 32;
  float* pw = base;
  float* pb = base + (int64_t)nwg * NO * KI;
  float* pr = pr_at ? pr_at : pb + (BIAS ? (int64_t)nwg * (NO - CTO2 * 32) : 0);
  if constexpr (MM == MM_X6) {
    if (ldy != NO - CTO2 * 32 || ldx != KI - CTI2 * 32 || (CTI2 > 0) != (X2 != nullptr) || (CTO2 > 0) != (dY2 != nullptr)) {
      fn::set_error("launch_dw: the bf16x6 dW kernel needs ld == width (and X2 / dY2 exactly when CTI2 / CTO2 > 0)");
      return -1;
    }
    constexpr int lds6 = 2 * (WO * TO + WI * TI) * 3 * 1024 + 128;
    auto kern6 = mlp_bwd_dw6_kernel<WO, WI, TO, TI, BIAS, RANK1, CTI2, CTO2>;
    static fn::DevOnce once6;
    if (int rc = fn::set_dyn_lds(reinterpret_cast<const void*>(kern6), once6, lds6)) return rc;
    hipLaunchKernelGGL(kern6, dim3(nwg), dim3(WO * WI * 64), lds6, st, P, dY, X, draw, pw, pb, pr, live_idx, live_cnt, X2, dY2);
    FN_LAUNCH_CHECK();
    return 0;
  } else {
    static_assert(MM == MM_F32 && CTI2 == 0 && CTO2 == 0, "two-tensor jobs exist for the bf16x6 dW kernel only");
    constexpr int STAGE = DW_MT * (NO + KI) + DW_MT;
    const size_t lds = 2 * STAGE * sizeof(float);
    auto kern = mlp_bwd_dw_kernel<WO, WI, TO, TI, BIAS, RANK1>;
    static fn::DevOnce once;
    if (int rc = fn::set_dyn_lds(reinterpret_cast<const void*>(kern), once, (int)lds)) return rc;
    hipLaunchKernelGGL(kern, dim3(nwg), dim3(WO * WI * 64), lds, st, P, dY, ldy, X, ldx, draw, pw, pb, pr, live_idx, live_cnt);
    FN_LAUNCH_CHECK();
    return 0;
  }
}

static void add_seg(RedTable& T, int64_t src, int64_t wg_stride, int nwg, int rows, int cols, int64_t dst, int ld,
                    int valid_cols, int dyn = 0, int sc_cols = 0, int64_t sc_dst = 0) {
  RedSeg& s = T.s[T.n++];
  s.src = src; s.wg_stride = wg_stride; s.nwg = nwg; s.rows = rows; s.cols = cols; s.dst = dst; s.ld = ld;
  s.valid_cols = valid_cols; s.dyn = dyn; s.sc_cols = sc_cols; s.sc_dst = sc_dst;
}

constexpr int DW_TRUNK_LDS = 2 * 16 * 3 * 1024 + 128;
static int trunk_chunks_fit(int64_t P, int ncu, int nwg) {
  if (dw_trunk_chunks(P, ncu) > nwg) {
    fn::set_error("mlp_bwd: the trunk launch needs %d chunks per job, the partial regions hold %d (a device with fewer than 8 CUs?)",
                  dw_trunk_chunks(P, ncu), nwg);
    return -1;
  }
  return 0;
}

static int bwd_reduce(const RedTable& T, const NetLayout& L, int64_t P, const float* params, float* partial, float* grads, int64_t g_off,
                      const int* live_cnt, int ncu, hipStream_t st) {
  hipLaunchKernelGGL(reduce_all_kernel, dim3(256, T.n), dim3(256), 0, st, T, partial, grads, partial, P, live_cnt, ncu);
  FN_LAUNCH_CHECK();
  hipLaunchKernelGGL(unfold_kernel, dim3(385), dim3(256), 0, st, partial + g_off, params, grads, L.VW, L.VB, L.FW, L.FB);
  FN_LAUNCH_CHECK();
  return 0;
}

namespace fn {
static float* head_workspace(int64_t ntiles, hipStream_t st) {
  const char* e = getenv("FASTNERF_HEAD_FROM_DX");
  if (e && e[0] == '0') return nullptr;
  static const WsName what = {
      "fastnerf: no memory for the per-tile head partials of the backward (%.1f MB): this stream keeps the head_grads launch\n", 1e-6};
  const StreamWs w = stream_ws(WS_HEAD_TILES, st, (ntiles > 0 ? ntiles : 1) * 388, what);
  if (w.p && e && e[0] == 'n') (void)hipMemsetAsync(w.p, 0xFF, sizeof(float) * (size_t)w.cap, st);
  return w.p;
}
}

template <int MM>
static int bwd_launch_t(int kind, int64_t n, int S, const float* draw, const float* act, const float* params,
                      const float* packed_bwd, float* dact, float* partial, float* grads, const int* live_idx,
                      const int* live_cnt, fn_stream_t stream, DwDeferred* defer = nullptr) {
  constexpr int MW = MM;
  const NetLayout& L = layout_of(kind);
  const int PEP = L.pe_pad;
  hipStream_t st = fn::S(stream);
  const int64_t P = n * S;
  const int64_t ntiles = (P + TM - 1) / TM;
  const int ncu = fn::device_cus();
  int grid = ncu * WG_PER_CU;
  if (ntiles < grid) grid = (int)ntiles;
  float* const headws = fn::head_workspace(ntiles, st);
  if (int rc_dx = fn_launch_dx(MM, grid, st, P, draw, act, params, packed_bwd, dact, L, live_idx, live_cnt, headws)) return rc_dx;

  const int nwg = ncu;
  RedTable T;
  T.n = 0;
  int rc;
  const float* a_pe = act + act_pe(P, PEP);
  auto region = [&](int j) { return partial + dw_job_base(j, ncu, PEP); };
  auto segs = [&](int j, int64_t dstW, int ld, int validc, int64_t dstB, int64_t dstR, int dyn = 0) {
    const DwJobDesc d = dw_job(j, PEP);
    const int64_t b = dw_job_base(j, ncu, PEP);
    add_seg(T, b, (int64_t)d.NO * d.KI, nwg, d.NO, d.KI, dstW, ld, validc, dyn);
    int64_t o = b + (int64_t)nwg * d.NO * d.KI;
    if (d.bias) { add_seg(T, o, d.NO, nwg, 1, d.NO, dstB, d.NO, d.NO, dyn); o += (int64_t)nwg * d.NO; }
    if (d.rank1) add_seg(T, o, d.KI, nwg, 1, d.KI, dstR, d.KI, d.KI, dyn);
  };
  if constexpr (MW == MM_X6) {
    if (PEP == 64) rc = launch_dw<8, 2, 2, 1, true, false, MW, 0, 8>(P, dact + dact_y(P, 0), 256, a_pe, 64, nullptr, region(0), nwg, st, live_idx, live_cnt, nullptr, dact + dact_y(P, 5));
    else rc = launch_dw<8, 1, 2, 3, true, false, MW, 0, 8>(P, dact + dact_y(P, 0), 256, a_pe, 96, nullptr, region(0), nwg, st, live_idx, live_cnt, nullptr, dact + dact_y(P, 5));
    if (rc) return rc;
    const int64_t b0 = dw_job_base(0, ncu, PEP);
    add_seg(T, b0, (int64_t)512 * PEP, nwg, 256, PEP, L.LW[0], L.in_pe, L.in_pe);
    add_seg(T, b0 + (int64_t)256 * PEP, (int64_t)512 * PEP, nwg, 256, PEP, L.LW[5], 256 + L.in_pe, L.in_pe);
    add_seg(T, b0 + (int64_t)nwg * 512 * PEP, 256, nwg, 1, 256, L.LB[0], 256, 256);
  } else {
    if (PEP == 64) rc = launch_dw<4, 1, 2, 2, true, false, MW>(P, dact + dact_y(P, 0), 256, a_pe, 64, nullptr, region(0), nwg, st, live_idx, live_cnt);
    else rc = launch_dw<4, 1, 2, 3, true, false, MW>(P, dact + dact_y(P, 0), 256, a_pe, 96, nullptr, region(0), nwg, st, live_idx, live_cnt);
    if (rc) return rc;
    segs(0, L.LW[0], L.in_pe, L.in_pe, L.LB[0], 0);
  }
  if constexpr (MW != MM_X6) {
    for (int l = 1; l < 8; ++l) {
      if ((rc = launch_dw<4, 2, 2, 4, true, false, MW>(P, dact + dact_y(P, l), 256, act + act_h(P, PEP, l - 1), 256, nullptr, region(l), nwg, st, live_idx, live_cnt))) return rc;
      segs(l, L.LW[l] + (l == 5 ? L.in_pe : 0), l == 5 ? 256 + L.in_pe : 256, 256, L.LB[l], 0);
    }
  }
  if constexpr (MW != MM_X6) {
    if (PEP == 64) rc = launch_dw<4, 1, 2, 2, false, false, MW>(P, dact + dact_y(P, 5), 256, a_pe, 64, nullptr, region(8), nwg, st, live_idx, live_cnt);
    else rc = launch_dw<4, 1, 2, 3, false, false, MW>(P, dact + dact_y(P, 5), 256, a_pe, 96, nullptr, region(8), nwg, st, live_idx, live_cnt);
    if (rc) return rc;
    segs(8, L.LW[5], 256 + L.in_pe, L.in_pe, 0, 0);
  }
  if constexpr (MW == MM_X6) {
    DwTrunk J;
    for (int l = 1; l < 8; ++l) {
      J.dY[l - 1] = dact + dact_y(P, l);
      J.X[l - 1] = act + act_h(P, PEP, l - 1);
      J.pw[l - 1] = region(l);
      J.pb[l - 1] = region(l) + (int64_t)nwg * 256 * 256;
    }
    if ((rc = trunk_chunks_fit(P, ncu, nwg))) return rc;
    if (defer) {
      defer->J = J;
    } else {
      static fn::DevOnce once_t;
      if ((rc = fn::set_dyn_lds(reinterpret_cast<const void*>(mlp_bwd_dw6_trunk_kernel), once_t, DW_TRUNK_LDS))) return rc;
      hipLaunchKernelGGL(mlp_bwd_dw6_trunk_kernel, dim3(dw_trunk_chunks(P, ncu), DW_TRUNK_JOBS), dim3(512), DW_TRUNK_LDS, st, P, J, live_idx, live_cnt, ncu);
      FN_LAUNCH_CHECK();
    }
    for (int l = 1; l < 8; ++l) segs(l, L.LW[l] + (l == 5 ? L.in_pe : 0), l == 5 ? 256 + L.in_pe : 256, 256, L.LB[l], 0, 1);
  }
  float* const pr_view = region(9);
  const int64_t g_off = dw_job_base(9, ncu, PEP) + (int64_t)nwg * 256;
  if constexpr (MW == MM_X6) {
    if ((rc = launch_dw<4, 3, 1, 3, true, true, MW, 1, 0>(P, dact + dact_yv(P), 128, act + act_h(P, PEP, 7), 256, draw, region(10), nwg, st,
                                                    live_idx, live_cnt, act + act_vpe(P, PEP), nullptr, pr_view))) return rc;
    const int64_t b10 = dw_job_base(10, ncu, PEP);
    add_seg(T, b10, 128 * 288, nwg, 128, 288, L.VW, 283, 283, 0, 256, g_off);
    add_seg(T, b10 + (int64_t)nwg * 128 * 288, 128, nwg, 1, 128, L.VB, 128, 128);
  } else {
    if ((rc = launch_dw<2, 4, 2, 2, true, true, MW>(P, dact + dact_yv(P), 128, act + act_h(P, PEP, 7), 256, draw, region(10), nwg, st, live_idx, live_cnt,
                                              nullptr, nullptr, pr_view))) return rc;
    const int64_t b10 = dw_job_base(10, ncu, PEP);
    add_seg(T, b10, 128 * 256, nwg, 128, 256, L.VW, 283, 256, 0, 256, g_off);
    add_seg(T, b10 + (int64_t)nwg * 128 * 256, 128, nwg, 1, 128, L.VB, 128, 128);
    if ((rc = launch_dw<4, 1, 1, 1, false, false, MW>(P, dact + dact_yv(P), 128, act + act_vpe(P, PEP), 32, nullptr, region(11), nwg, st, live_idx, live_cnt))) return rc;
    segs(11, L.VW + 256, 283, 27, 0, 0);
  }
  add_seg(T, dw_job_base(9, ncu, PEP), 256, nwg, 1, 256, L.AW, 256, 256);
  if (headws != nullptr) {
    const int64_t hb = dw_job_base(12, ncu, PEP);
    const int rows = ntiles < HEAD_ROWS ? (int)ntiles : HEAD_ROWS;
    hipLaunchKernelGGL(head_group_kernel, dim3(rows, 4), dim3(128), 0, st, P, headws, partial + hb, live_cnt);
    FN_LAUNCH_CHECK();
    add_seg(T, hb, 388, rows, 1, 388, L.RW, 388, 387, 2);
    add_seg(T, hb + 387, 388, rows, 1, 1, L.AB, 1, 1, 2);
  } else {
    const int hg = HEAD_MAX_WG;
    const int64_t hb = dw_job_base(12, ncu, PEP);
    hipLaunchKernelGGL(head_grads_kernel, dim3(hg), dim3(128), 0, st, P, draw, act + act_hv(P, PEP), partial + hb, live_idx, live_cnt);
    FN_LAUNCH_CHECK();
    add_seg(T, hb, 388, hg, 1, 388, L.RW, 388, 387);
    add_seg(T, hb + 387, 388, hg, 1, 1, L.AB, 1, 1);
  }
  if (defer) {
    defer->T = T; defer->P = P; defer->g_off = g_off; defer->params = params; defer->partial = partial; defer->grads = grads; defer->kind = kind;
    return 0;
  }
  return bwd_reduce(T, L, P, params, partial, grads, g_off, live_cnt, ncu, st);
}

namespace fn {
static std::atomic<int64_t> g_pair_launches{0};

bool x6_pair_workspace(int64_t P_coarse, fn_stream_t stream, float** dact2, float** partial2) {
  static const WsName what = {
      "fastnerf: no memory for the side workspace of the paired bf16x6 backward (%.2f GB): this stream keeps the per-pass trunk launches\n", 1e-9};
  const StreamWs d = stream_ws(WS_PAIR_DACT, S(stream), P_coarse * (int64_t)DACT_FLOATS, what);
  if (!d.p) return false;
  const StreamWs p = stream_ws(WS_PAIR_PARTIAL, S(stream), fastnerf_mlp_bwd_partial_floats(), what);
  if (!p.p) return false;
  *dact2 = d.p;
  *partial2 = p.p;
  return true;
}

int x6_pair_pass(DwDeferred* d, int64_t n, int S, const float* draw, const float* act, const float* params, const float* packed_bwd,
                 float* dact, float* partial, float* grads, fn_stream_t stream) {
  FN_CHECK_ARG(d && n > 0 && S >= 1, "d != NULL, n>0, S>=1");
  FN_CHECK_ARG(draw && act && params && packed_bwd && dact && partial && grads, "null pointer");
  return bwd_launch_t<MM_X6>(0, n, S, draw, act, params, packed_bwd, dact, partial, grads, nullptr, nullptr, stream, d);
}

int x6_pair_finish(const DwDeferred* fine, const DwDeferred* coarse, fn_stream_t stream) {
  hipStream_t st = S(stream);
  const int ncu = fn::device_cus();
  const DwDeferred* d[2] = {fine, coarse};
  DwTrunkPair A;
  int nwg = 0;
  for (int k = 0; k < 2; ++k) {
    A.J[k] = d[k]->J;
    A.P[k] = d[k]->P;
    nwg += DW_TRUNK_JOBS * dw_trunk_chunks(A.P[k], ncu);
  }
  static DevOnce once_p;
  if (int rc = set_dyn_lds(reinterpret_cast<const void*>(mlp_bwd_dw6_trunk_pair_kernel), once_p, DW_TRUNK_LDS)) return rc;
  hipLaunchKernelGGL(mlp_bwd_dw6_trunk_pair_kernel, dim3(nwg), dim3(512), DW_TRUNK_LDS, st, A, ncu);
  FN_LAUNCH_CHECK();
  g_pair_launches.fetch_add(1, std::memory_order_relaxed);
  for (int k = 0; k < 2; ++k)
    if (int rc = bwd_reduce(d[k]->T, layout_of(d[k]->kind), d[k]->P, d[k]->params, d[k]->partial, d[k]->grads, d[k]->g_off, nullptr, ncu, st)) return rc;
  return 0;
}
}
extern "C" int64_t fastnerf_x6_pair_launches(void) { return fn::g_pair_launches.load(std::memory_order_relaxed); }

static int bwd_launch(int kind, int64_t n, int S, const float* draw, const float* act, const float* params,
                      const float* packed_bwd, float* dact, float* partial, float* grads, const int* live_idx,
                      const int* live_cnt, fn_stream_t stream, int mm = MM_F32) {
  return mm == MM_X6 ? bwd_launch_t<MM_X6>(kind, n, S, draw, act, params, packed_bwd, dact, partial, grads, live_idx, live_cnt, stream)
                     : bwd_launch_t<MM_F32>(kind, n, S, draw, act, params, packed_bwd, dact, partial, grads, live_idx, live_cnt, stream);
}
extern "C" int fastnerf_mlp_bwd_ex(int kind, int64_t n, int S, const float* draw, const float* act,
                                   const float* params, const float* packed_bwd, float* dact, float* partial,
                                   float* grads, fn_stream_t stream) {
  FN_CHECK_ARG(kind >= 0 && kind <= 2 && n > 0 && S >= 1, "kind in 0..2, n>0, S>=1");
  FN_CHECK_ARG(draw && act && params && packed_bwd && dact && partial && grads, "null pointer");
  return bwd_launch(kind, n, S, draw, act, params, packed_bwd, dact, partial, grads, nullptr, nullptr, stream);
}
extern "C" int fastnerf_mlp_bwd_live_ex(int kind, int64_t n, int S, const float* draw, const float* act,
                                        const float* params, const float* packed_bwd, float* dact, float* partial,
                                        float* grads, const int32_t* live_idx, const int32_t* live_cnt,
                                        fn_stream_t stream) {
  FN_CHECK_ARG(kind >= 0 && kind <= 2 && n > 0 && S >= 1, "kind in 0..2, n>0, S>=1");
  FN_CHECK_ARG(draw && act && params && packed_bwd && dact && partial && grads && live_idx && live_cnt, "null pointer");
  return bwd_launch(kind, n, S, draw, act, params, packed_bwd, dact, partial, grads, live_idx, live_cnt, stream);
}
extern "C" int fastnerf_mlp_bwd(int64_t n, int S, const float* draw, const float* act, const float* params,
                                const float* packed_bwd, float* dact, float* partial, float* grads,
                                fn_stream_t stream) {
  return fastnerf_mlp_bwd_ex(0, n, S, draw, act, params, packed_bwd, dact, partial, grads, stream);
}

extern "C" int fastnerf_mlp_x6_bwd(int kind, int64_t n, int S, const float* draw, const float* act, const float* params,
                                   const float* packed_bwd, float* dact, float* partial, float* grads, fn_stream_t stream) {
  FN_CHECK_ARG(kind >= 0 && kind <= 2 && n > 0 && S >= 1, "kind in 0..2, n>0, S>=1");
  FN_CHECK_ARG(draw && act && params && packed_bwd && dact && partial && grads, "null pointer");
  return bwd_launch(kind, n, S, draw, act, params, packed_bwd, dact, partial, grads, nullptr, nullptr, stream, MM_X6);
}
extern "C" int fastnerf_mlp_x6_bwd_live(int kind, int64_t n, int S, const float* draw, const float* act, const float* params,
                                        const float* packed_bwd, float* dact, float* partial, float* grads,
                                        const int32_t* live_idx, const int32_t* live_cnt, fn_stream_t stream) {
  FN_CHECK_ARG(kind >= 0 && kind <= 2 && n > 0 && S >= 1, "kind in 0..2, n>0, S>=1");
  FN_CHECK_ARG(draw && act && params && packed_bwd && dact && partial && grads && live_idx && live_cnt, "null pointer");
  return bwd_launch(kind, n, S, draw, act, params, packed_bwd, dact, partial, grads, live_idx, live_cnt, stream, MM_X6);
}
```

### fast-learning-nerf_amd/csrc/mlp_pack.hip

```cpp
#include "mlp_common.h"

struct PackDesc {
  int64_t src_off;
  int64_t dst_off;
  int ld;
  int n_rows;
  int n_cols;
  int segA_pad, segA_valid, segB_valid;
  int col0;
  int transposed;
  int fold;
};
#define N_PACK 21
struct PackTable {
  PackDesc d[N_PACK];
  int64_t m_off;
};

__global__ void __launch_bounds__(256) fold_kernel(const float* __restrict__ params, int64_t VW, int64_t VB, int64_t FW, int64_t FB,
                                                    float* __restrict__ m_out, float* __restrict__ b_out, bool slack) {
  const int e = blockIdx.x * 256 + threadIdx.x;
  if (e < 128 * 256) {
    const int o = e >> 8, j = e & 255;
    const float* wv = params + VW + (int64_t)o * 283;
    const float* wf = params + FW + j;
    double s = 0.0;
#pragma unroll 8
    for (int i = 0; i < 256; ++i) s = fma((double)wv[i], (double)wf[(int64_t)i * 256], s);
    m_out[e] = (float)s;
    if (slack && e < 128 * 256 / 2) m_out[128 * 256 + e] = 0.f;
  } else if (e < 128 * 256 + 128) {
    const int o = e - 128 * 256;
    const float* wv = params + VW + (int64_t)o * 283;
    double s = (double)params[VB + o];
    for (int i = 0; i < 256; ++i) s = fma((double)wv[i], (double)params[FB + i], s);
    b_out[o] = (float)s;
    if (slack && o < 128 / 2) b_out[128 + o] = 0.f;
  }
}
static void launch_fold(const NetLayout& L, const float* params, float* packed_fwd, bool x6, hipStream_t st) {
  hipLaunchKernelGGL(fold_kernel, dim3(129), dim3(256), 0, st, params, L.VW, L.VB, L.FW, L.FB, packed_fwd + fold_plain(L.PFR, x6),
                     packed_fwd + fold_plain(L.PFB, x6), x6);
}

__global__ void __launch_bounds__(256) pack_kernel(PackTable tab, const float* __restrict__ params,
                                                    float* pf, float* __restrict__ pb) {
  const PackDesc d = tab.d[blockIdx.y];
  const int64_t total = (int64_t)d.n_rows * d.n_cols;
  float* dst = (d.transposed ? pb : pf) + d.dst_off;
  const float* src = params + d.src_off;
  const float* mraw = pf + tab.m_off;
  for (int64_t e = blockIdx.x * (int64_t)blockDim.x + threadIdx.x; e < total; e += (int64_t)gridDim.x * blockDim.x) {
    const int t = (int)(e & 3);
    const int l = (int)((e >> 2) & 63);
    const int64_t blk = e >> 8;
    float v = 0.f;
    if (!d.transposed) {
      const int KS = d.n_cols / 8;
      const int nt = (int)(blk / KS), ks = (int)(blk % KS);
      const int n = nt * 32 + (l & 31);
      const int kp = ks * 8 + (l >> 5) * 4 + t;
      int col = -1;
      if (kp < d.segA_pad) {
        if (kp < d.segA_valid) col = kp;
      } else {
        const int q = kp - d.segA_pad;
        if (q < d.segB_valid) col = d.segA_valid + q;
      }
      if (col >= 0) v = (d.fold && kp < d.segA_pad) ? mraw[n * 256 + col] : src[(int64_t)n * d.ld + col];
    } else {
      const int KS = d.n_rows / 8;
      const int jt = (int)(blk / KS), ks = (int)(blk % KS);
      const int o = ks * 8 + (l >> 5) * 4 + t;
      const int c = d.col0 + jt * 32 + (l & 31);
      v = d.fold ? mraw[o * 256 + c] : src[(int64_t)o * d.ld + c];
    }
    dst[e] = v;
  }
}

__global__ void __launch_bounds__(256) pack6_kernel(PackTable tab, const float* __restrict__ params,
                                                     uint4* pf, uint4* __restrict__ pb) {
  const PackDesc d = tab.d[blockIdx.y];
  constexpr int TW = 16, KW = 32;
  const int KS = (d.transposed ? d.n_rows : d.n_cols) / KW;
  const int NTL = (d.transposed ? d.n_cols : d.n_rows) / TW;
  const int64_t total = (int64_t)NTL * KS * 64;
  uint4* dst = (d.transposed ? pb : pf) + d.dst_off * 3 / 8;
  const float* src = params + d.src_off;
  const float* mraw = reinterpret_cast<const float*>(pf) + tab.m_off;
  for (int64_t e = blockIdx.x * (int64_t)blockDim.x + threadIdx.x; e < total; e += (int64_t)gridDim.x * blockDim.x) {
    const int l = (int)(e & 63);
    const int64_t blk = e >> 6;
    const int tile = (int)(blk / KS), ks = (int)(blk % KS);
    float v[8];
#pragma unroll
    for (int j = 0; j < 8; ++j) {
      const int kp = ks * KW + (l / TW) * 8 + j;
      v[j] = 0.f;
      if (!d.transposed) {
        const int n = tile * TW + (l % TW);
        int col = -1;
        if (kp < d.segA_pad) { if (kp < d.segA_valid) col = kp; }
        else { const int q = kp - d.segA_pad; if (q < d.segB_valid) col = d.segA_valid + q; }
        if (col >= 0) v[j] = (d.fold && kp < d.segA_pad) ? mraw[n * 256 + col] : src[(int64_t)n * d.ld + col];
      } else {
        const int c = d.col0 + tile * TW + (l % TW);
        v[j] = d.fold ? mraw[kp * 256 + c] : src[(int64_t)kp * d.ld + c];
      }
    }
    unsigned h[4], m[4], lo[4];
#pragma unroll
    for (int q = 0; q < 4; ++q) {
      split3_pair(v[2 * q], v[2 * q + 1], h[q], m[q], lo[q]);
    }
    uint4* o = dst + (blk * 3) * 64 + l;
    o[0] = make_uint4(h[0], h[1], h[2], h[3]);
    o[64] = make_uint4(m[0], m[1], m[2], m[3]);
    o[128] = make_uint4(lo[0], lo[1], lo[2], lo[3]);
  }
}

static PackTable make_pack_table(const NetLayout& L, bool x6) {
  PackTable T;
  T.m_off = fold_plain(L.PFR, x6);
  int n = 0;
  for (int l = 0; l < 8; ++l) {
    PackDesc d{};
    d.src_off = L.LW[l]; d.dst_off = L.PF[l]; d.n_rows = 256;
    d.ld = (l == 0) ? L.in_pe : (l == 5 ? 256 + L.in_pe : 256);
    d.n_cols = (l == 0) ? L.pe_pad : (l == 5 ? L.pe_pad + 256 : 256);
    if (l == 0) { d.segA_pad = L.pe_pad; d.segA_valid = L.in_pe; d.segB_valid = 0; }
    else if (l == 5) { d.segA_pad = L.pe_pad; d.segA_valid = L.in_pe; d.segB_valid = 256; }
    else { d.segA_pad = 256; d.segA_valid = 256; d.segB_valid = 0; }
    T.d[n++] = d;
  }
  { PackDesc d{}; d.src_off = L.FW; d.dst_off = L.PF[8]; d.ld = 256; d.n_rows = 256; d.n_cols = 256;
    d.segA_pad = 256; d.segA_valid = 256; T.d[n++] = d; }
  { PackDesc d{}; d.src_off = L.VW; d.dst_off = L.PF[9]; d.ld = 283; d.n_rows = 128; d.n_cols = 288;
    d.segA_pad = 256; d.segA_valid = 256; d.segB_valid = 27; T.d[n++] = d; }
  { PackDesc d{}; d.transposed = 1; d.src_off = L.VW; d.dst_off = L.PB[0]; d.ld = 283; d.n_rows = 128; d.n_cols = 256; d.col0 = 0; T.d[n++] = d; }
  { PackDesc d{}; d.transposed = 1; d.src_off = L.FW; d.dst_off = L.PB[1]; d.ld = 256; d.n_rows = 256; d.n_cols = 256; d.col0 = 0; T.d[n++] = d; }
  const int order[7] = {7, 6, 5, 4, 3, 2, 1};
  for (int j = 0; j < 7; ++j) {
    const int l = order[j];
    PackDesc d{}; d.transposed = 1; d.src_off = L.LW[l]; d.dst_off = L.PB[2 + j]; d.n_rows = 256; d.n_cols = 256;
    d.ld = (l == 5) ? 256 + L.in_pe : 256;
    d.col0 = (l == 5) ? L.in_pe : 0;
    T.d[n++] = d;
  }
  { PackDesc d{}; d.fold = 1; d.src_off = L.VW; d.dst_off = L.PFM; d.ld = 283; d.n_rows = 128; d.n_cols = 288;
    d.segA_pad = 256; d.segA_valid = 256; d.segB_valid = 27; T.d[n++] = d; }
  { PackDesc d{}; d.fold = 1; d.transposed = 1; d.src_off = L.VW; d.dst_off = L.PBM; d.ld = 256; d.n_rows = 128; d.n_cols = 256; d.col0 = 0; T.d[n++] = d; }
  return T;
}


extern "C" int64_t fastnerf_net_floats(int kind, int what) {
  if (kind < 0 || kind > 2) return -1;
  const NetLayout& L = layout_of(kind);
  return what == 0 ? L.n_params : what == 1 ? L.pf_total : what == 2 ? L.pb_total : what == 3 ? L.pe_pad : -1;
}
extern "C" int64_t fastnerf_mlp_act_floats(int kind, int64_t P) {
  if (kind < 0 || kind > 2 || P < 0) return -1;
  return act_floats(P, layout_of(kind).pe_pad);
}

extern "C" int fastnerf_mlp_pack_ex(int kind, const float* params, float* packed_fwd, float* packed_bwd,
                                    fn_stream_t stream) {
  FN_CHECK_ARG(kind >= 0 && kind <= 2 && params && packed_fwd && packed_bwd, "kind in 0..2, non-null pointers");
  static const PackTable T[3] = {make_pack_table(layout_of(0), false), make_pack_table(layout_of(1), false),
                                 make_pack_table(layout_of(2), false)};
  launch_fold(layout_of(kind), params, packed_fwd, false, fn::S(stream));
  FN_LAUNCH_CHECK();
  hipLaunchKernelGGL(pack_kernel, dim3(64, N_PACK), dim3(256), 0, fn::S(stream), T[kind], params, packed_fwd, packed_bwd);
  FN_LAUNCH_CHECK();
  return 0;
}
extern "C" int64_t fastnerf_mlp_x6_packed_floats(int kind, int which) {
  if (kind < 0 || kind > 2 || (which != 1 && which != 2)) return -1;
  const NetLayout& L = layout_of(kind);
  return (which == 1 ? L.pf_total : L.pb_total) * 3 / 2;
}
extern "C" int fastnerf_mlp_x6_pack(int kind, const float* params, float* packed_fwd, float* packed_bwd, fn_stream_t stream) {
  FN_CHECK_ARG(kind >= 0 && kind <= 2 && params && packed_fwd && packed_bwd, "kind in 0..2, non-null pointers");
  static const PackTable T[3] = {make_pack_table(layout_of(0), true), make_pack_table(layout_of(1), true),
                                 make_pack_table(layout_of(2), true)};
  launch_fold(layout_of(kind), params, packed_fwd, true, fn::S(stream));
  FN_LAUNCH_CHECK();
  hipLaunchKernelGGL(pack6_kernel, dim3(32, N_PACK), dim3(256), 0, fn::S(stream), T[kind], params,
                     reinterpret_cast<uint4*>(packed_fwd), reinterpret_cast<uint4*>(packed_bwd));
  FN_LAUNCH_CHECK();
  return 0;
}
extern "C" int fastnerf_mlp_pack(const float* params, float* packed_fwd, float* packed_bwd, fn_stream_t stream) {
  return fastnerf_mlp_pack_ex(0, params, packed_fwd, packed_bwd, stream);
}


extern "C" int64_t fastnerf_mlp_fold_offset(int kind, int what) {
  if (kind < 0 || kind > 2) return -1;
  const NetLayout& L = layout_of(kind);
  return what == 0 ? L.PFM : what == 1 ? L.PFB : what == 2 ? L.PFR : what == 3 ? L.PBM : -1;
}
```

### fast-learning-nerf_amd/csrc/render.cpp

```cpp
#include <stdint.h>
#include "../../include/fastnerf.h"
#include "dw_pair.h"

namespace fn {
void set_error(const char* fmt, ...);
const char* occ_cascade_fault(const fn_occ_cascade* c);
const char* occ_grid_fault(const fn_occ_grid* g);
bool x6_pair_workspace(int64_t P_coarse, fn_stream_t stream, float** dact2, float** partial2);
int x6_pair_pass(DwDeferred* d, int64_t n, int S, const float* draw, const float* act, const float* params, const float* packed_bwd,
                 float* dact, float* partial, float* grads, fn_stream_t stream);
int x6_pair_finish(const DwDeferred* fine, const DwDeferred* coarse, fn_stream_t stream);
}

struct MlpMode {
  int (*pack)(int kind, const float* params, float* packed_fwd, float* packed_bwd, fn_stream_t);
  int (*fwd)(int kind, int64_t n, int S, const float* rays11, const float* z, const float* params, const float* packed_fwd, float* raw,
             float* act, int flags, fn_stream_t);
  int (*fwd_list)(int kind, int64_t n, int S, const float* rays11, const float* z, const float* params, const float* packed_fwd,
                  float* raw, const int32_t* live_idx, const int32_t* live_cnt, int flags, fn_stream_t);
  int (*fwd_live)(int kind, int64_t n, int S, const float* rays11, const float* z, const float* params, const float* packed_fwd,
                  float* act, const int32_t* live_idx, const int32_t* live_cnt, fn_stream_t);
  int (*bwd)(int kind, int64_t n, int S, const float* draw, const float* act, const float* params, const float* packed_bwd, float* dact,
             float* partial, float* grads, fn_stream_t);
  int (*bwd_live)(int kind, int64_t n, int S, const float* draw, const float* act, const float* params, const float* packed_bwd,
                  float* dact, float* partial, float* grads, const int32_t* live_idx, const int32_t* live_cnt, fn_stream_t);
};

static int fwd_fp32(int kind, int64_t n, int S, const float* rays11, const float* z, const float* params, const float* packed_fwd,
                    float* raw, float* act, int flags, fn_stream_t stream) {
  return act ? fastnerf_mlp_fwd_ex(kind, n, S, rays11, z, params, packed_fwd, raw, act, stream)
             : fastnerf_mlp_fwd_flags_ex(kind, n, S, rays11, z, params, packed_fwd, raw, flags, stream);
}

static int fwd_bf16(int kind, int64_t n, int S, const float* rays11, const float* z, const float* params, const float* packed_fwd,
                    float* raw, float* act, int flags, fn_stream_t stream) {
  return act ? fastnerf_mlp_bf16_fwd(kind, n, S, rays11, z, params, packed_fwd, raw, act, stream)
             : fastnerf_mlp_bf16_fwd_flags(kind, n, S, rays11, z, params, packed_fwd, raw, flags, stream);
}

static const MlpMode modes[3] = {
    {fastnerf_mlp_pack_ex, fwd_fp32, fastnerf_mlp_fwd_list_ex, fastnerf_mlp_fwd_live_ex, fastnerf_mlp_bwd_ex, fastnerf_mlp_bwd_live_ex},
    {fastnerf_mlp_bf16_pack, fwd_bf16, fastnerf_mlp_bf16_fwd_list, fastnerf_mlp_bf16_fwd_live, fastnerf_mlp_bf16_bwd,
     fastnerf_mlp_bf16_bwd_live},
    {fastnerf_mlp_x6_pack, fastnerf_mlp_x6_fwd, fastnerf_mlp_x6_fwd_list, fastnerf_mlp_x6_fwd_live, fastnerf_mlp_x6_bwd,
     fastnerf_mlp_x6_bwd_live},
};

struct RrFwd {
  const char* fname;
  int math_mode;
  int64_t n;
  int N_samples, N_importance;
  const float* rays11;
  int lindisp, perturb, det, white_bkgd;
  const float *t_rand, *u, *noise0, *noise1;
  uint64_t seed0, seed1;
  const float *params_c, *packed_c, *params_f, *packed_f;
  float *z0, *raw0, *rgb0, *disp0, *acc0, *w0, *depth0, *z1, *z_samples, *z_std, *raw1, *rgb1, *disp1, *acc1, *w1, *depth1;
  int flags;
  fn_stream_t stream;
};

static bool rr_fwd_scalars(const RrFwd& a) {
  if (a.math_mode < 0 || a.math_mode > 2 || a.n < 0 || a.N_samples < 2 || a.N_importance < 0) {
    fn::set_error("%s: bad argument: math_mode in {0,1,2}, n>=0, N_samples>=2, N_importance>=0", a.fname);
    return false;
  }
  if (a.N_importance > 0 && a.N_samples < 3) {
    fn::set_error("%s: hierarchical sampling needs N_samples >= 3 (the inner weights of 2 samples are empty)", a.fname);
    return false;
  }
  return true;
}

static bool rr_fwd_coarse_ptrs(const RrFwd& a) {
  return a.rays11 && a.params_c && a.packed_c && a.z0 && a.raw0 && a.rgb0 && a.disp0 && a.acc0 && a.w0 && a.depth0;
}

template <class Net>
static int rr_fwd_chain(const RrFwd& a, Net&& net) {
  int rc;
  if ((rc = fastnerf_sample_coarse(a.n, a.N_samples, a.rays11, a.lindisp, a.perturb, a.t_rand, a.seed0, a.z0, a.stream))) return rc;
  if ((rc = net(0, a.N_samples, a.z0, a.params_c, a.packed_c, a.raw0, a.noise0))) return rc;
  if ((rc = fastnerf_raw2outputs_fwd(a.n, a.N_samples, a.raw0, a.z0, a.rays11, a.noise0, a.white_bkgd, a.rgb0, a.disp0, a.acc0, a.w0,
                                     a.depth0, a.stream)))
    return rc;
  if (a.N_importance == 0) return 0;
  if (!a.params_f || !a.packed_f || !a.z1 || !a.z_samples || !a.z_std || !a.raw1 || !a.rgb1 || !a.disp1 || !a.acc1 || !a.w1 ||
      !a.depth1) {
    fn::set_error("%s: null pointer (fine pass)", a.fname);
    return -1;
  }
  const int S1 = a.N_samples + a.N_importance;
  if ((rc = fastnerf_sample_pdf_merge(a.n, a.N_samples, a.N_importance, a.z0, a.w0, a.det, a.u, a.seed1, a.z1, a.z_samples, a.z_std,
                                      a.stream)))
    return rc;
  if ((rc = net(1, S1, a.z1, a.params_f, a.packed_f, a.raw1, a.noise1))) return rc;
  return fastnerf_raw2outputs_fwd(a.n, S1, a.raw1, a.z1, a.rays11, a.noise1, a.white_bkgd, a.rgb1, a.disp1, a.acc1, a.w1, a.depth1,
                                  a.stream);
}

extern "C" int fastnerf_render_rays_fwd_ex(int math_mode, int64_t n, int N_samples, int N_importance, const float* rays11,
                                        int lindisp, int perturb, int det, int white_bkgd, const float* t_rand, const float* u,
                                        const float* noise0, const float* noise1, uint64_t seed0, uint64_t seed1,
                                        const float* params_c, const float* packed_c, const float* params_f,
                                        const float* packed_f, float* z0, float* raw0, float* act0, float* rgb0,
                                        float* disp0, float* acc0, float* w0, float* depth0, float* z1,
                                        float* z_samples, float* z_std, float* raw1, float* act1, float* rgb1,
                                        float* disp1, float* acc1, float* w1, float* depth1, int flags, fn_stream_t stream) {
  const RrFwd a = {"fastnerf_render_rays_fwd", math_mode, n, N_samples, N_importance, rays11, lindisp, perturb, det, white_bkgd, t_rand,
                   u, noise0, noise1, seed0, seed1, params_c, packed_c, params_f, packed_f, z0, raw0, rgb0, disp0, acc0, w0, depth0, z1,
                   z_samples, z_std, raw1, rgb1, disp1, acc1, w1, depth1, flags, stream};
  if (!rr_fwd_scalars(a)) return -1;
  if (n == 0) return 0;
  if (!rr_fwd_coarse_ptrs(a)) {
    fn::set_error("%s: null pointer (coarse pass)", a.fname);
    return -1;
  }
  return rr_fwd_chain(a, [&](int pass, int S, const float* z, const float* params, const float* packed, float* raw, const float* noise) {
    float* act = pass ? act1 : act0;
    return modes[math_mode].fwd(0, n, S, rays11, z, params, packed, raw, act, (!act && !noise) ? flags : 0, stream);
  });
}

static int rr_fwd_occ(const RrFwd& a, const fn_occ_grid* grid, const fn_occ_cascade* cascade, int32_t* live_ws, int32_t* counts_out) {
  if (!rr_fwd_scalars(a)) return -1;
  if (a.n == 0) return 0;
  const int64_t P1 = a.n * (int64_t)(a.N_samples + a.N_importance);
  if (P1 >= ((int64_t)1 << 31)) {
    fn::set_error("%s: bad argument: n * (N_samples + N_importance) < 2^31 (lists index points with int32)", a.fname);
    return -1;
  }
  if (!rr_fwd_coarse_ptrs(a) || (!grid && !cascade) || !live_ws || !counts_out) {
    fn::set_error("%s: null pointer (coarse pass)", a.fname);
    return -1;
  }
  if (const char* fault = cascade ? fn::occ_cascade_fault(cascade) : nullptr) {
    fn::set_error("%s: bad argument: %s", a.fname, fault);
    return -1;
  }
  int32_t* idx = live_ws;
  int32_t* cws = live_ws + P1;
  return rr_fwd_chain(a, [&](int pass, int S, const float* z, const float* params, const float* packed, float* raw, const float*) {
    int32_t* cnt = counts_out + 2 * pass;
    if (int rc = cascade ? fastnerf_occ_classify_cascade(cascade, a.n, S, a.rays11, z, idx, cnt, raw, cws, a.stream)
                         : fastnerf_occ_classify(grid, a.n, S, a.rays11, z, idx, cnt, raw, cws, a.stream))
      return rc;
    return modes[a.math_mode].fwd_list(0, a.n, S, a.rays11, z, params, packed, raw, idx, cnt, a.flags, a.stream);
  });
}

extern "C" int fastnerf_render_rays_fwd_occ(int math_mode, int64_t n, int N_samples, int N_importance, const float* rays11, int lindisp,
                                            int perturb, int det, int white_bkgd, const float* t_rand, const float* u, uint64_t seed0,
                                            uint64_t seed1, const float* params_c, const float* packed_c, const float* params_f,
                                            const float* packed_f, const fn_occ_grid* grid, int32_t* live_ws, int32_t* counts_out,
                                            float* z0, float* raw0, float* rgb0, float* disp0, float* acc0, float* w0, float* depth0,
                                            float* z1, float* z_samples, float* z_std, float* raw1, float* rgb1, float* disp1,
                                            float* acc1, float* w1, float* depth1, int flags, fn_stream_t stream) {
  return rr_fwd_occ({"fastnerf_render_rays_fwd_occ", math_mode, n, N_samples, N_importance, rays11, lindisp, perturb, det, white_bkgd,
                     t_rand, u, nullptr, nullptr, seed0, seed1, params_c, packed_c, params_f, packed_f, z0, raw0, rgb0, disp0, acc0, w0,
                     depth0, z1, z_samples, z_std, raw1, rgb1, disp1, acc1, w1, depth1, flags, stream},
                    grid, nullptr, live_ws, counts_out);
}

extern "C" int fastnerf_render_rays_fwd_occ_cascade(int math_mode, int64_t n, int N_samples, int N_importance, const float* rays11,
                                                    int lindisp, int perturb, int det, int white_bkgd, const float* t_rand,
                                                    const float* u, uint64_t seed0, uint64_t seed1, const float* params_c,
                                                    const float* packed_c, const float* params_f, const float* packed_f,
                                                    const fn_occ_cascade* cascade, int32_t* live_ws, int32_t* counts_out, float* z0,
                                                    float* raw0, float* rgb0, float* disp0, float* acc0, float* w0, float* depth0,
                                                    float* z1, float* z_samples, float* z_std, float* raw1, float* rgb1, float* disp1,
                                                    float* acc1, float* w1, float* depth1, int flags, fn_stream_t stream) {
  return rr_fwd_occ({"fastnerf_render_rays_fwd_occ_cascade", math_mode, n, N_samples, N_importance, rays11, lindisp, perturb, det,
                     white_bkgd, t_rand, u, nullptr, nullptr, seed0, seed1, params_c, packed_c, params_f, packed_f, z0, raw0, rgb0,
                     disp0, acc0, w0, depth0, z1, z_samples, z_std, raw1, rgb1, disp1, acc1, w1, depth1, flags, stream},
                    nullptr, cascade, live_ws, counts_out);
}

extern "C" int fastnerf_render_rays_fwd_ert(int math_mode, int64_t n, int N_samples, int N_importance, const float* rays11, int lindisp,
                                            int perturb, int det, int white_bkgd, const float* t_rand, const float* u, uint64_t seed0,
                                            uint64_t seed1, const float* params_c, const float* packed_c, const float* params_f,
                                            const float* packed_f, const fn_occ_grid* grid, const fn_occ_cascade* cascade, float eps,
                                            int block, float* trans_ws, int32_t* live_ws, int32_t* counts_out, float* z0, float* raw0,
                                            float* rgb0, float* disp0, float* acc0, float* w0, float* depth0, float* z1,
                                            float* z_samples, float* z_std, float* raw1, float* rgb1, float* disp1, float* acc1,
                                            float* w1, float* depth1, int flags, fn_stream_t stream) {
  const RrFwd a = {"fastnerf_render_rays_fwd_ert", math_mode, n, N_samples, N_importance, rays11, lindisp, perturb, det, white_bkgd,
                   t_rand, u, nullptr, nullptr, seed0, seed1, params_c, packed_c, params_f, packed_f, z0, raw0, rgb0, disp0, acc0, w0,
                   depth0, z1, z_samples, z_std, raw1, rgb1, disp1, acc1, w1, depth1, flags, stream};
  if (!rr_fwd_scalars(a)) return -1;
  if (!(eps >= 0.f && eps < 1.f) || block < 1) {
    fn::set_error("%s: bad argument: 0 <= eps < 1, block >= 1", a.fname);
    return -1;
  }
  if (grid && cascade) {
    fn::set_error("%s: bad argument: at most one of grid / cascade", a.fname);
    return -1;
  }
  if (n == 0) return 0;
  const int S_img = N_samples + N_importance;
  const int64_t P1 = n * (int64_t)S_img;
  if (P1 >= ((int64_t)1 << 31) || S_img > 512) {
    fn::set_error("%s: bad argument: n * (N_samples + N_importance) < 2^31 (lists index points with int32), at most 512 samples per ray", a.fname);
    return -1;
  }
  if (!rr_fwd_coarse_ptrs(a) || !trans_ws || !live_ws || !counts_out) {
    fn::set_error("%s: null pointer (coarse pass)", a.fname);
    return -1;
  }
  if (N_importance > 0 && (!params_f || !packed_f || !z1 || !z_samples || !z_std || !raw1 || !rgb1 || !disp1 || !acc1 || !w1 || !depth1)) {
    fn::set_error("%s: null pointer (fine pass)", a.fname);
    return -1;
  }
  if (const char* fault = cascade ? fn::occ_cascade_fault(cascade) : (grid ? fn::occ_grid_fault(grid) : nullptr)) {
    fn::set_error("%s: bad argument: %s", a.fname, fault);
    return -1;
  }
  int32_t* idx = live_ws;
  int32_t* cws = live_ws + P1;
  int32_t* seg = cws + fastnerf_compact_ws_ints(P1);
  const int img = N_importance > 0 ? 1 : 0;
  return rr_fwd_chain(a, [&](int pass, int S, const float* z, const float* params, const float* packed, float* raw, const float*) {
    int32_t* cnt = counts_out + 2 * pass;
    int rc;
    if (pass != img) {
      if (!grid && !cascade) return modes[math_mode].fwd(0, n, S, rays11, z, params, packed, raw, nullptr, flags, stream);
      if ((rc = cascade ? fastnerf_occ_classify_cascade(cascade, n, S, rays11, z, idx, cnt, raw, cws, stream)
                        : fastnerf_occ_classify(grid, n, S, rays11, z, idx, cnt, raw, cws, stream)))
        return rc;
      return modes[math_mode].fwd_list(0, n, S, rays11, z, params, packed, raw, idx, cnt, flags, stream);
    }
    for (int s0 = 0; s0 < S; s0 += block) {
      const int s1 = (S - s0 > block) ? s0 + block : S;
      if ((rc = fastnerf_ert_classify(grid, cascade, n, S, s0, s1, rays11, z, s0 ? trans_ws : nullptr, eps, idx, seg, raw, cws, stream)))
        return rc;
      if ((rc = modes[math_mode].fwd_list(0, n, S, rays11, z, params, packed, raw, idx, seg, flags, stream))) return rc;
      if ((rc = fastnerf_ert_advance(n, S, s0, s1, raw, z, rays11, s0 == 0, trans_ws, seg, cnt, stream))) return rc;
    }
    return 0;
  });
}

extern "C" int fastnerf_render_rays_fwd(int math_mode, int64_t n, int N_samples, int N_importance, const float* rays11,
                                        int lindisp, int perturb, int det, int white_bkgd, const float* t_rand, const float* u,
                                        const float* noise0, const float* noise1, uint64_t seed0, uint64_t seed1,
                                        const float* params_c, const float* packed_c, const float* params_f,
                                        const float* packed_f, float* z0, float* raw0, float* act0, float* rgb0,
                                        float* disp0, float* acc0, float* w0, float* depth0, float* z1,
                                        float* z_samples, float* z_std, float* raw1, float* act1, float* rgb1,
                                        float* disp1, float* acc1, float* w1, float* depth1, fn_stream_t stream) {
  return fastnerf_render_rays_fwd_ex(math_mode, n, N_samples, N_importance, rays11, lindisp, perturb, det, white_bkgd, t_rand, u,
                                     noise0, noise1, seed0, seed1, params_c, packed_c, params_f, packed_f, z0, raw0, act0, rgb0,
                                     disp0, acc0, w0, depth0, z1, z_samples, z_std, raw1, act1, rgb1, disp1, acc1, w1, depth1, 0,
                                     stream);
}

struct PassMaps {
  const float *acc, *depth, *g_disp, *g_acc, *g_depth;
  bool any() const { return g_disp || g_acc || g_depth; }
};
static PassMaps pass_maps(const fn_map_grads* m, int pass, const float* acc, const float* depth) {
  if (!m) return {acc, depth, nullptr, nullptr, nullptr};
  return pass ? PassMaps{acc, depth, m->g_disp1, m->g_acc1, m->g_depth1} : PassMaps{acc, depth, m->g_disp0, m->g_acc0, m->g_depth0};
}
static int comp_bwd(int64_t n, int S, const float* raw, const float* z, const float* rays11, const float* noise, int white_bkgd,
                    const float* g_rgb, const PassMaps& m, float* draw, fn_stream_t stream) {
  if (!m.any()) return fastnerf_raw2outputs_bwd(n, S, raw, z, rays11, noise, white_bkgd, g_rgb, draw, stream);
  return fastnerf_raw2outputs_bwd_full(n, S, raw, z, rays11, noise, white_bkgd, m.acc, m.depth, g_rgb, m.g_disp, m.g_acc, nullptr,
                                       m.g_depth, draw, stream);
}

static int rr_bwd(int math_mode, int64_t n, int N_samples, int N_importance, const float* rays11,
                  int white_bkgd, const float* g_rgb, const float* g_rgb0, const float* noise0,
                  const float* noise1, const float* z0, const float* raw0, const float* act0,
                  const float* z1, const float* raw1, const float* act1, const float* params_c,
                  const float* packed_bwd_c, const float* params_f, const float* packed_bwd_f,
                  float* draw_ws, float* dact_ws, float* partial_ws, float* grads_c, float* grads_f,
                  const float* acc0, const float* depth0, const float* acc1, const float* depth1, const fn_map_grads* mg,
                  int passes, fn_stream_t stream) {
  if (math_mode < 0 || math_mode > 2 || n <= 0 || N_samples < 2 || N_importance < 0) {
    fn::set_error("fastnerf_render_rays_bwd: bad argument: math_mode in {0,1,2}, n>0, N_samples>=2, N_importance>=0");
    return -1;
  }
  if (!rays11 || !z0 || !raw0 || !act0 || !params_c || !packed_bwd_c || !draw_ws || !dact_ws || !partial_ws || !grads_c) {
    fn::set_error("fastnerf_render_rays_bwd: null pointer (coarse pass)");
    return -1;
  }
  int rc;
  auto mlp = [&](int S, const float* act, const float* params, const float* packed, float* grads) {
    return modes[math_mode].bwd(0, n, S, draw_ws, act, params, packed, dact_ws, partial_ws, grads, stream);
  };
  const float* g_coarse = g_rgb;
  PassMaps m_coarse = pass_maps(mg, 1, acc0, depth0);
  if (N_importance > 0) {
    const PassMaps m_fine = pass_maps(mg, 1, acc1, depth1);
    m_coarse = pass_maps(mg, 0, acc0, depth0);
    if ((!g_rgb && !m_fine.any()) || (!g_rgb0 && !m_coarse.any()) || !z1 || !raw1 || !act1 || !params_f || !packed_bwd_f || !grads_f) {
      fn::set_error("fastnerf_render_rays_bwd: null pointer (fine pass)");
      return -1;
    }
    if ((m_fine.g_disp && (!acc1 || !depth1)) || (m_coarse.g_disp && (!acc0 || !depth0))) {
      fn::set_error("fastnerf_render_rays_bwd: a disparity gradient needs the forward's acc and depth of its pass");
      return -1;
    }
    const int S1 = N_samples + N_importance;
    float *dact2 = nullptr, *partial2 = nullptr;
    if (passes == 3 && math_mode == 2 && fn::x6_pair_workspace(n * (int64_t)N_samples, stream, &dact2, &partial2)) {
      DwDeferred d_fine, d_coarse;
      if ((rc = comp_bwd(n, S1, raw1, z1, rays11, noise1, white_bkgd, g_rgb, m_fine, draw_ws, stream))) return rc;
      if ((rc = fn::x6_pair_pass(&d_fine, n, S1, draw_ws, act1, params_f, packed_bwd_f, dact_ws, partial_ws, grads_f, stream))) return rc;
      if ((rc = comp_bwd(n, N_samples, raw0, z0, rays11, noise0, white_bkgd, g_rgb0, m_coarse, draw_ws, stream))) return rc;
      if ((rc = fn::x6_pair_pass(&d_coarse, n, N_samples, draw_ws, act0, params_c, packed_bwd_c, dact2, partial2, grads_c, stream))) return rc;
      return fn::x6_pair_finish(&d_fine, &d_coarse, stream);
    }
    if (passes & 1) {
      if ((rc = comp_bwd(n, S1, raw1, z1, rays11, noise1, white_bkgd, g_rgb, m_fine, draw_ws, stream))) return rc;
      if ((rc = mlp(S1, act1, params_f, packed_bwd_f, grads_f))) return rc;
    }
    g_coarse = g_rgb0;
  }
  if (!g_coarse && !m_coarse.any()) {
    fn::set_error("fastnerf_render_rays_bwd: null gradient");
    return -1;
  }
  if (m_coarse.g_disp && (!acc0 || !depth0)) {
    fn::set_error("fastnerf_render_rays_bwd: a disparity gradient needs the forward's acc and depth of its pass");
    return -1;
  }
  if (!(passes & 2)) return 0;
  if ((rc = comp_bwd(n, N_samples, raw0, z0, rays11, noise0, white_bkgd, g_coarse, m_coarse, draw_ws, stream))) return rc;
  return mlp(N_samples, act0, params_c, packed_bwd_c, grads_c);
}

extern "C" int fastnerf_render_rays_bwd(int math_mode, int64_t n, int N_samples, int N_importance, const float* rays11,
                                        int white_bkgd, const float* g_rgb, const float* g_rgb0, const float* noise0,
                                        const float* noise1, const float* z0, const float* raw0, const float* act0,
                                        const float* z1, const float* raw1, const float* act1, const float* params_c,
                                        const float* packed_bwd_c, const float* params_f, const float* packed_bwd_f,
                                        float* draw_ws, float* dact_ws, float* partial_ws, float* grads_c, float* grads_f,
                                        fn_stream_t stream) {
  return rr_bwd(math_mode, n, N_samples, N_importance, rays11, white_bkgd, g_rgb, g_rgb0, noise0, noise1, z0, raw0, act0, z1, raw1,
                act1, params_c, packed_bwd_c, params_f, packed_bwd_f, draw_ws, dact_ws, partial_ws, grads_c, grads_f, nullptr, nullptr,
                nullptr, nullptr, nullptr, 3, stream);
}

extern "C" int fastnerf_render_rays_bwd_maps(int math_mode, int64_t n, int N_samples, int N_importance, const float* rays11,
                                             int white_bkgd, const float* g_rgb, const float* g_rgb0, const float* noise0,
                                             const float* noise1, const float* z0, const float* raw0, const float* act0,
                                             const float* z1, const float* raw1, const float* act1, const float* params_c,
                                             const float* packed_bwd_c, const float* params_f, const float* packed_bwd_f,
                                             float* draw_ws, float* dact_ws, float* partial_ws, float* grads_c, float* grads_f,
                                             const float* acc0, const float* depth0, const float* acc1, const float* depth1,
                                             const fn_map_grads* maps, fn_stream_t stream) {
  return rr_bwd(math_mode, n, N_samples, N_importance, rays11, white_bkgd, g_rgb, g_rgb0, noise0, noise1, z0, raw0, act0, z1, raw1,
                act1, params_c, packed_bwd_c, params_f, packed_bwd_f, draw_ws, dact_ws, partial_ws, grads_c, grads_f, acc0, depth0,
                acc1, depth1, maps, 3, stream);
}


static int rr_bwd_live(int math_mode, int64_t n, int N_samples, int N_importance, const float* rays11, int white_bkgd,
                       const float* g_rgb, const float* g_rgb0, const float* noise0, const float* noise1,
                       const float* z0, const float* raw0, const float* z1, const float* raw1,
                       const float* params_c, const float* packed_fwd_c, const float* packed_bwd_c,
                       const float* params_f, const float* packed_fwd_f, const float* packed_bwd_f,
                       float* draw_ws, float* act_ws, float* dact_ws, float* partial_ws, int32_t* live_ws,
                       float* grads_c, float* grads_f, int32_t* counts_out, const float* acc0, const float* depth0,
                       const float* acc1, const float* depth1, const fn_map_grads* mg, int passes, fn_stream_t stream) {
  if (math_mode < 0 || math_mode > 2 || n <= 0 || N_samples < 2 || N_importance < 0) {
    fn::set_error("fastnerf_render_rays_bwd_live: bad argument: math_mode in {0,1,2}, n>0, N_samples>=2, N_importance>=0");
    return -1;
  }
  if (!rays11 || !z0 || !raw0 || !params_c || !packed_fwd_c || !packed_bwd_c || !draw_ws || !act_ws || !dact_ws ||
      !partial_ws || !live_ws || !grads_c) {
    fn::set_error("fastnerf_render_rays_bwd_live: null pointer (coarse pass)");
    return -1;
  }
  const int S1 = N_samples + N_importance;
  int32_t* cnt = live_ws;
  int32_t* idx = live_ws + 4;
  int32_t* cws = idx + n * (int64_t)S1;
  int rc;
  auto pass = [&](int S, const float* z, const float* raw, const float* noise, const float* g, const PassMaps& m, const float* params,
                  const float* pf, const float* pb, float* grads, int32_t* cnt_out) -> int {
    if (m.g_disp && (!m.acc || !m.depth)) {
      fn::set_error("fastnerf_render_rays_bwd_live: a disparity gradient needs the forward's acc and depth of its pass");
      return -1;
    }
    if ((rc = comp_bwd(n, S, raw, z, rays11, noise, white_bkgd, g, m, draw_ws, stream))) return rc;
    if ((rc = fastnerf_compact_live(n * (int64_t)S, draw_ws, idx, cnt_out, cws, stream))) return rc;
    if ((rc = modes[math_mode].fwd_live(0, n, S, rays11, z, params, pf, act_ws, idx, cnt_out, stream))) return rc;
    return modes[math_mode].bwd_live(0, n, S, draw_ws, act_ws, params, pb, dact_ws, partial_ws, grads, idx, cnt_out, stream);
  };
  const float* g_coarse = g_rgb;
  int32_t* c_fine = counts_out ? counts_out : cnt;
  int32_t* c_coarse = counts_out ? counts_out + 2 : cnt + 2;
  PassMaps m_coarse = pass_maps(mg, 1, acc0, depth0);
  if (N_importance > 0) {
    const PassMaps m_fine = pass_maps(mg, 1, acc1, depth1);
    m_coarse = pass_maps(mg, 0, acc0, depth0);
    if ((!g_rgb && !m_fine.any()) || (!g_rgb0 && !m_coarse.any()) || !z1 || !raw1 || !params_f || !packed_fwd_f || !packed_bwd_f ||
        !grads_f) {
      fn::set_error("fastnerf_render_rays_bwd_live: null pointer (fine pass)");
      return -1;
    }
    if ((passes & 1) && (rc = pass(S1, z1, raw1, noise1, g_rgb, m_fine, params_f, packed_fwd_f, packed_bwd_f, grads_f, c_fine)))
      return rc;
    g_coarse = g_rgb0;
  }
  if (!g_coarse && !m_coarse.any()) {
    fn::set_error("fastnerf_render_rays_bwd_live: null gradient");
    return -1;
  }
  if (!(passes & 2)) return 0;
  return pass(N_samples, z0, raw0, noise0, g_coarse, m_coarse, params_c, packed_fwd_c, packed_bwd_c, grads_c, c_coarse);
}

extern "C" int fastnerf_render_rays_bwd_live(int math_mode, int64_t n, int N_samples, int N_importance, const float* rays11, int white_bkgd,
                                             const float* g_rgb, const float* g_rgb0, const float* noise0, const float* noise1,
                                             const float* z0, const float* raw0, const float* z1, const float* raw1,
                                             const float* params_c, const float* packed_fwd_c, const float* packed_bwd_c,
                                             const float* params_f, const float* packed_fwd_f, const float* packed_bwd_f,
                                             float* draw_ws, float* act_ws, float* dact_ws, float* partial_ws, int32_t* live_ws,
                                             float* grads_c, float* grads_f, int32_t* counts_out, fn_stream_t stream) {
  return rr_bwd_live(math_mode, n, N_samples, N_importance, rays11, white_bkgd, g_rgb, g_rgb0, noise0, noise1, z0, raw0, z1, raw1,
                     params_c, packed_fwd_c, packed_bwd_c, params_f, packed_fwd_f, packed_bwd_f, draw_ws, act_ws, dact_ws,
                     partial_ws, live_ws, grads_c, grads_f, counts_out, nullptr, nullptr, nullptr, nullptr, nullptr, 3, stream);
}

extern "C" int fastnerf_render_rays_bwd_live_maps(int math_mode, int64_t n, int N_samples, int N_importance, const float* rays11,
                                                  int white_bkgd, const float* g_rgb, const float* g_rgb0, const float* noise0,
                                                  const float* noise1, const float* z0, const float* raw0, const float* z1,
                                                  const float* raw1, const float* params_c, const float* packed_fwd_c,
                                                  const float* packed_bwd_c, const float* params_f, const float* packed_fwd_f,
                                                  const float* packed_bwd_f, float* draw_ws, float* act_ws, float* dact_ws,
                                                  float* partial_ws, int32_t* live_ws, float* grads_c, float* grads_f,
                                                  int32_t* counts_out, const float* acc0, const float* depth0, const float* acc1,
                                                  const float* depth1, const fn_map_grads* maps, fn_stream_t stream) {
  return rr_bwd_live(math_mode, n, N_samples, N_importance, rays11, white_bkgd, g_rgb, g_rgb0, noise0, noise1, z0, raw0, z1, raw1,
                     params_c, packed_fwd_c, packed_bwd_c, params_f, packed_fwd_f, packed_bwd_f, draw_ws, act_ws, dact_ws,
                     partial_ws, live_ws, grads_c, grads_f, counts_out, acc0, depth0, acc1, depth1, maps, 3, stream);
}


extern "C" int64_t fastnerf_step_args_size(void) { return (int64_t)sizeof(fn_step_args); }

extern "C" int64_t fastnerf_step_aux_size(void) { return (int64_t)sizeof(fn_step_aux); }

static int train_step(const fn_step_args* a, const fn_step_aux* aux, int phases, fn_stream_t stream) {
  if (aux && !aux->depth_target && !aux->acc_target) aux = nullptr;
  if (!a || a->math_mode < 0 || a->math_mode > 2 || a->n <= 0 || a->N_samples < 2 || a->N_importance < 0) {
    fn::set_error("fastnerf_train_step: bad argument: args != NULL, math_mode in {0,1,2}, n>0, N_samples>=2, N_importance>=0");
    return -1;
  }
  const bool two = a->N_importance > 0;
  if (!a->params || !a->grads || !a->packed_fwd_c || !a->packed_bwd_c || (two && (!a->packed_fwd_f || !a->packed_bwd_f)) ||
      a->net_floats <= 0) {
    fn::set_error("fastnerf_train_step: null network buffer");
    return -1;
  }
  if (a->occ) {
    if (!a->live) {
      fn::set_error("fastnerf_train_step: an occupancy grid needs the compacted step (live != 0): the plain backward has no list");
      return -1;
    }
    if (a->noise0 || a->noise1) {
      fn::set_error("fastnerf_train_step: an occupancy grid cannot be combined with sigma noise (it is added before the relu)");
      return -1;
    }
    if (!a->live_ws) {
      fn::set_error("fastnerf_train_step: an occupancy grid needs live_ws");
      return -1;
    }
  }
  const float* params_c = a->params;
  const float* params_f = two ? a->params + a->net_floats : nullptr;
  float* grads_c = a->grads;
  float* grads_f = two ? a->grads + a->net_floats : nullptr;
  const float* g_fine = two ? a->g_rgb : nullptr;
  int rc;
  if (phases & FN_STEP_FORWARD) {
    if (!a->rays_o || !a->rays_d || !a->target || !a->rays11 || !a->g_rgb || (two && !a->g_rgb0) || !a->loss2) {
      fn::set_error("fastnerf_train_step: null batch / output buffer");
      return -1;
    }
    if ((rc = fastnerf_pack_rays(a->n, a->rays_o, a->rays_d, a->near_plane, a->far_plane, a->ndc, a->H, a->W, a->focal, a->rays11,
                                 stream))) return rc;
    const bool save = !a->live;
    if (a->occ) {
      if ((rc = fastnerf_render_rays_fwd_occ(a->math_mode, a->n, a->N_samples, a->N_importance, a->rays11, a->lindisp,
                                             (a->perturb || a->t_rand) ? 1 : 0, a->perturb ? 0 : 1, a->white_bkgd, a->t_rand, a->u,
                                             a->seed0, a->seed1, params_c, a->packed_fwd_c, params_f, a->packed_fwd_f, a->occ,
                                             a->live_ws + 4, a->occ_counts ? a->occ_counts : a->live_ws, a->z0, a->raw0, a->rgb0,
                                             a->disp0, a->acc0, a->w0, a->depth0, a->z1, a->z_samples, a->z_std, a->raw1, a->rgb1,
                                             a->disp1, a->acc1, a->w1, a->depth1, a->fwd_flags, stream)))
        return rc;
    } else if ((rc = fastnerf_render_rays_fwd_ex(a->math_mode, a->n, a->N_samples, a->N_importance, a->rays11, a->lindisp,
                                          (a->perturb || a->t_rand) ? 1 : 0, a->perturb ? 0 : 1, a->white_bkgd, a->t_rand, a->u,
                                          a->noise0, a->noise1, a->seed0, a->seed1, params_c, a->packed_fwd_c, params_f,
                                          a->packed_fwd_f, a->z0, a->raw0, save ? a->act0 : nullptr, a->rgb0, a->disp0, a->acc0,
                                          a->w0, a->depth0, a->z1, a->z_samples, a->z_std, a->raw1, save ? a->act1 : nullptr,
                                          a->rgb1, a->disp1, a->acc1, a->w1, a->depth1, save ? 0 : a->fwd_flags, stream)))
      return rc;
    if ((rc = fastnerf_mse_leafmax(a->n, two ? a->rgb1 : a->rgb0, two ? a->rgb0 : nullptr, a->target, a->grad_scale, a->g_rgb,
                                   two ? a->g_rgb0 : nullptr, a->loss2, a->leaf_tag, a->max_leaves, a->table, stream)))
      return rc;
    if (aux && (rc = fastnerf_aux_loss(a->n, two ? a->depth1 : a->depth0, two ? a->acc1 : a->acc0, two ? a->depth0 : nullptr,
                                       two ? a->acc0 : nullptr, aux->depth_target, aux->depth_weight, aux->acc_target,
                                       aux->acc_weight, aux->lambda_depth, aux->lambda_acc, a->grad_scale, aux->g_depth1,
                                       aux->g_acc1, two ? aux->g_depth0 : nullptr, two ? aux->g_acc0 : nullptr, aux->loss4, stream)))
      return rc;
  }
  const int passes = ((phases & FN_STEP_BWD_FINE) ? 1 : 0) | ((phases & FN_STEP_BWD_COARSE) ? 2 : 0);
  if (passes) {
    const float* g_a = two ? g_fine : a->g_rgb;
    const float* g_b = two ? a->g_rgb0 : nullptr;
    fn_map_grads mg = {nullptr, nullptr, nullptr, nullptr, nullptr, nullptr};
    if (aux) {
      if ((aux->depth_target && (!aux->g_depth1 || (two && !aux->g_depth0))) || (aux->acc_target && (!aux->g_acc1 || (two && !aux->g_acc0)))) {
        fn::set_error("fastnerf_train_step_aux: null gradient buffer of a term whose target is set");
        return -1;
      }
      if (aux->depth_target) { mg.g_depth1 = aux->g_depth1; mg.g_depth0 = two ? aux->g_depth0 : nullptr; }
      if (aux->acc_target) { mg.g_acc1 = aux->g_acc1; mg.g_acc0 = two ? aux->g_acc0 : nullptr; }
    }
    const fn_map_grads* mgp = aux ? &mg : nullptr;
    if (a->live)
      rc = rr_bwd_live(a->math_mode, a->n, a->N_samples, a->N_importance, a->rays11, a->white_bkgd, g_a, g_b, a->noise0, a->noise1,
                       a->z0, a->raw0, a->z1, a->raw1, params_c, a->packed_fwd_c, a->packed_bwd_c, params_f, a->packed_fwd_f,
                       a->packed_bwd_f, a->draw_ws, a->act_ws, a->dact_ws, a->partial_ws, a->live_ws, grads_c, grads_f, a->counts,
                       a->acc0, a->depth0, a->acc1, a->depth1, mgp, passes, stream);
    else
      rc = rr_bwd(a->math_mode, a->n, a->N_samples, a->N_importance, a->rays11, a->white_bkgd, g_a, g_b, a->noise0, a->noise1, a->z0,
                  a->raw0, a->act0, a->z1, a->raw1, a->act1, params_c, a->packed_bwd_c, params_f, a->packed_bwd_f, a->draw_ws,
                  a->dact_ws, a->partial_ws, grads_c, grads_f, a->acc0, a->depth0, a->acc1, a->depth1, mgp, passes, stream);
    if (rc) return rc;
  }
  if (phases & FN_STEP_UPDATE) {
    if (!a->adam_m || !a->adam_v || a->adam_t < 1) {
      fn::set_error("fastnerf_train_step: update phase needs adam_m, adam_v and adam_t >= 1");
      return -1;
    }
    const int64_t total = a->net_floats * (two ? 2 : 1);
    if ((rc = fastnerf_adam_step(total, a->params, a->grads, a->adam_m, a->adam_v, a->lr, a->beta1, a->beta2, a->eps, a->adam_t,
                                 stream))) return rc;
    if ((rc = modes[a->math_mode].pack(0, params_c, a->packed_fwd_c, a->packed_bwd_c, stream))) return rc;
    if (two && (rc = modes[a->math_mode].pack(0, params_f, a->packed_fwd_f, a->packed_bwd_f, stream))) return rc;
  }
  return 0;
}

extern "C" int fastnerf_train_step(const fn_step_args* a, int phases, fn_stream_t stream) { return train_step(a, nullptr, phases, stream); }

extern "C" int fastnerf_train_step_aux(const fn_step_args* a, const fn_step_aux* aux, int phases, fn_stream_t stream) {
  return train_step(a, aux, phases, stream);
}
```

### include/fastnerf.h

```cpp
#ifndef FASTNERF_H
#define FASTNERF_H
#include <stdint.h>
#ifdef __cplusplus
extern "C" {
#endif

typedef void* fn_stream_t;

int fastnerf_version(void);
const char* fastnerf_last_error(void);
int fastnerf_device_cus(void);
int64_t fastnerf_x6_pair_launches(void);

int fastnerf_gen_rays(int H, int W, float fx, float fy, float cx, float cy, const float* c2w_host,
                      float* rays_o, float* rays_d, fn_stream_t stream);
int fastnerf_gen_rays_pixels(int64_t n, const int32_t* pix, const float* poses, float fx, float fy, float cx,
                             float cy, float* rays_o, float* rays_d, fn_stream_t stream);
int fastnerf_ndc_rays(int64_t n, int H, int W, double focal, float near, const float* rays_o, const float* rays_d,
                      float* out_o, float* out_d, fn_stream_t stream);
int fastnerf_pack_rays(int64_t n, const float* rays_o, const float* rays_d, float near, float far, int ndc, int H,
                       int W, double focal, float* rays11, fn_stream_t stream);
int fastnerf_sample_coarse(int64_t n, int S, const float* rays11, int lindisp, int perturb, const float* t_rand,
                           uint64_t seed, float* z, fn_stream_t stream);
int fastnerf_posenc(int64_t n, int L, const float* x, float* out, fn_stream_t stream);

#define FASTNERF_NET_PARAMS 595844
#define FASTNERF_PACKED_FWD 663680
#define FASTNERF_PACKED_BWD 589824
#define FASTNERF_ACT_FLOATS 2592
#define FASTNERF_ACT_SLACK 8192
#define FASTNERF_DACT_FLOATS 2432

int fastnerf_mlp_pack(const float* params, float* packed_fwd, float* packed_bwd, fn_stream_t stream);
int fastnerf_mlp_fwd(int64_t n, int S, const float* rays11, const float* z, const float* params,
                     const float* packed_fwd, float* raw, float* act, fn_stream_t stream);
int64_t fastnerf_mlp_bwd_partial_floats(void);
int fastnerf_mlp_bwd(int64_t n, int S, const float* draw, const float* act, const float* params,
                     const float* packed_bwd, float* dact, float* partial, float* grads, fn_stream_t stream);

int fastnerf_raw2outputs_fwd(int64_t n, int S, const float* raw, const float* z, const float* rays11,
                             const float* noise, int white_bkgd, float* rgb_map, float* disp, float* acc,
                             float* weights, float* depth, fn_stream_t stream);
int fastnerf_raw2outputs_bwd(int64_t n, int S, const float* raw, const float* z, const float* rays11,
                             const float* noise, int white_bkgd, const float* g_rgb, float* draw,
                             fn_stream_t stream);
int fastnerf_raw2outputs_bwd_full(int64_t n, int S, const float* raw, const float* z, const float* rays11,
                                  const float* noise, int white_bkgd, const float* acc, const float* depth,
                                  const float* g_rgb, const float* g_disp, const float* g_acc, const float* g_w,
                                  const float* g_depth, float* draw, fn_stream_t stream);
int fastnerf_sample_pdf_merge(int64_t n, int S, int Ni, const float* z, const float* weights, int det,
                              const float* u, uint64_t seed, float* z_out, float* z_samples, float* z_std,
                              fn_stream_t stream);

int fastnerf_sample_pdf(int64_t n, int M, int Ni, const float* bins, const float* weights, int det, const float* u,
                        uint64_t seed, float* samples, fn_stream_t stream);

int fastnerf_mse_leafmax(int64_t n, const float* rgb, const float* rgb0, const float* target, float grad_scale,
                         float* g_rgb, float* g_rgb0, float* loss2, const int32_t* leaf_tag, int max_leaves,
                         uint32_t* table, fn_stream_t stream);
int fastnerf_aux_loss(int64_t n, const float* depth1, const float* acc1, const float* depth0, const float* acc0,
                      const float* depth_target, const float* depth_weight, const float* acc_target, const float* acc_weight,
                      float lambda_depth, float lambda_acc, float grad_scale, float* g_depth1, float* g_acc1, float* g_depth0,
                      float* g_acc0, float* loss4, fn_stream_t stream);
int fastnerf_adam_step(int64_t n, float* params, const float* grads, float* m, float* v, double lr, double beta1,
                       double beta2, double eps, int step, fn_stream_t stream);

int64_t fastnerf_net_floats(int kind, int what);
int64_t fastnerf_mlp_act_floats(int kind, int64_t n_points);
int fastnerf_mlp_pack_ex(int kind, const float* params, float* packed_fwd, float* packed_bwd, fn_stream_t stream);
int fastnerf_mlp_fwd_ex(int kind, int64_t n, int S, const float* rays11, const float* z, const float* params,
                        const float* packed_fwd, float* raw, float* act, fn_stream_t stream);
int fastnerf_mlp_bwd_ex(int kind, int64_t n, int S, const float* draw, const float* act, const float* params,
                        const float* packed_bwd, float* dact, float* partial, float* grads, fn_stream_t stream);

int64_t fastnerf_mlp_bf16_floats(int kind, int what, int64_t n_points);
int64_t fastnerf_mlp_bf16_partial_floats(void);
int fastnerf_mlp_bf16_pack(int kind, const float* params, float* packed_fwd, float* packed_bwd, fn_stream_t stream);
int fastnerf_mlp_bf16_fwd(int kind, int64_t n, int S, const float* rays11, const float* z, const float* params,
                          const float* packed_fwd, float* raw, float* act, fn_stream_t stream);
int fastnerf_mlp_bf16_bwd(int kind, int64_t n, int S, const float* draw, const float* act, const float* params,
                          const float* packed_bwd, float* dact, float* partial, float* grads, fn_stream_t stream);

#define FN_FWD_SKIP_DEAD_RGB 1
int fastnerf_mlp_bf16_fwd_flags(int kind, int64_t n, int S, const float* rays11, const float* z, const float* params,
                                const float* packed_fwd, float* raw, int flags, fn_stream_t stream);
int fastnerf_mlp_fwd_flags_ex(int kind, int64_t n, int S, const float* rays11, const float* z, const float* params,
                              const float* packed_fwd, float* raw, int flags, fn_stream_t stream);

int fastnerf_render_rays_fwd(int math_mode, int64_t n, int N_samples, int N_importance, const float* rays11, int lindisp,
                             int perturb, int det, int white_bkgd, const float* t_rand, const float* u,
                             const float* noise0, const float* noise1, uint64_t seed0, uint64_t seed1,
                             const float* params_c, const float* packed_c, const float* params_f, const float* packed_f,
                             float* z0, float* raw0, float* act0, float* rgb0, float* disp0, float* acc0, float* w0,
                             float* depth0, float* z1, float* z_samples, float* z_std, float* raw1, float* act1,
                             float* rgb1, float* disp1, float* acc1, float* w1, float* depth1, fn_stream_t stream);
int fastnerf_render_rays_fwd_ex(int math_mode, int64_t n, int N_samples, int N_importance, const float* rays11, int lindisp,
                                int perturb, int det, int white_bkgd, const float* t_rand, const float* u,
                                const float* noise0, const float* noise1, uint64_t seed0, uint64_t seed1,
                                const float* params_c, const float* packed_c, const float* params_f, const float* packed_f,
                                float* z0, float* raw0, float* act0, float* rgb0, float* disp0, float* acc0, float* w0,
                                float* depth0, float* z1, float* z_samples, float* z_std, float* raw1, float* act1,
                                float* rgb1, float* disp1, float* acc1, float* w1, float* depth1, int flags, fn_stream_t stream);

int fastnerf_render_rays_bwd(int math_mode, int64_t n, int N_samples, int N_importance, const float* rays11, int white_bkgd,
                             const float* g_rgb, const float* g_rgb0, const float* noise0, const float* noise1,
                             const float* z0, const float* raw0, const float* act0, const float* z1, const float* raw1,
                             const float* act1, const float* params_c, const float* packed_bwd_c, const float* params_f,
                             const float* packed_bwd_f, float* draw_ws, float* dact_ws, float* partial_ws, float* grads_c,
                             float* grads_f, fn_stream_t stream);

int fastnerf_pp_gen_rays(int H, int W, const double* intrinsics_host, const double* c2w_host, float* rays_o,
                         float* rays_d, fn_stream_t stream);
int fastnerf_leaf_sumcount(int64_t n, const float* rgb, const float* target, const int32_t* leaf_tag, int max_leaves,
                           double* sum, int32_t* count, fn_stream_t stream);
int fastnerf_pp_intersect_sphere(int64_t n, const float* rays11, float* fg_far, int* n_outside, fn_stream_t stream);
int fastnerf_pp_fg_depths(int64_t n, int S, float near, const float* fg_far, int perturb, const float* t_rand,
                          uint64_t seed, float* z, fn_stream_t stream);
int fastnerf_pp_sample_pdf_merge(int64_t n, int S, int Ni, const float* z, const float* weights, int det,
                                 const float* u, uint64_t seed, float* z_out, float* z_samples, fn_stream_t stream);
int fastnerf_pp_perturb_samples(int64_t n, int S, const float* z_in, const float* t_rand, uint64_t seed, float* z_out,
                                fn_stream_t stream);
int fastnerf_pp_sample_pdf(int64_t n, int M, int Ni, const float* bins, const float* weights, int det, const float* u,
                           uint64_t seed, float* samples, fn_stream_t stream);
int fastnerf_pp_depth2pts_outside(int64_t n, int S, const float* ray_o, const float* ray_d, const float* depth, float* pts,
                                  float* depth_real, fn_stream_t stream);
int fastnerf_pp_composite_fwd(int64_t n, int S, int part, const float* raw, const float* z, const float* rays11,
                              const float* fg_far, float* rgb_map, float* weights, float* depth, float* lambda,
                              fn_stream_t stream);
int fastnerf_pp_composite_bwd(int64_t n, int S, int part, const float* raw, const float* z, const float* rays11,
                              const float* fg_far, const float* g_rgb, const float* g_lambda, float* draw,
                              fn_stream_t stream);

typedef struct fn_tree fn_tree;
fn_tree* fastnerf_tree_create(int H, int W, int n_images, int max_depth);
void fastnerf_tree_destroy(fn_tree* t);
int fastnerf_tree_num_leaves(const fn_tree* t, int image);
int fastnerf_tree_max_leaves(const fn_tree* t);
double fastnerf_tree_min_area(const fn_tree* t, int image);
int fastnerf_tree_get_leaves(const fn_tree* t, int image, double* out_host);
int fastnerf_tree_set_leaves(fn_tree* t, int image, int n_leaves, const double* boxes_host, double min_area);
int fastnerf_tree_leaf_plan(const fn_tree* t, int image, double ray_num_per_pixel, int last_epoch,
                            int32_t* out_host);
int64_t fastnerf_tree_adjust(fn_tree* t, const float* table_host, int max_leaves, double thres);
int64_t fastnerf_tree_adjust_mean(fn_tree* t, const double* sum_host, const int32_t* count_host, int max_leaves,
                                  double thres);


int64_t fastnerf_tree_epoch_plan(const fn_tree* t, double ray_num_per_pixel, int last_epoch, int32_t* out_host,
                                 int64_t* n_rays_host);
int fastnerf_epoch_rays(int64_t N, int L, const int32_t* plan, const int64_t* offs, const float* images,
                        const float* poses, int n_img, int H, int W, float fx, float fy, float cx, float cy,
                        uint64_t seed, int shuffle, const int32_t* n_weighted, const int64_t* seg_beg,
                        const int64_t* seg_end, const int32_t* order, const double* cum, float* rays_o, float* rays_d,
                        float* rgb, int32_t* tag, int32_t* pix, fn_stream_t stream);
int64_t fastnerf_epoch_shard_rows(int64_t N, int64_t batch, int row0, int stride);
int fastnerf_epoch_rays_shard(int64_t N, int L, const int32_t* plan, const int64_t* offs, const float* images,
                              const float* poses, int n_img, int H, int W, float fx, float fy, float cx, float cy,
                              uint64_t seed, int shuffle, const int32_t* n_weighted, const int64_t* seg_beg,
                              const int64_t* seg_end, const int32_t* order, const double* cum, int64_t batch, int row0, int stride,
                              float* rays_o, float* rays_d, float* rgb, int32_t* tag, int32_t* pix, fn_stream_t stream);

int fastnerf_gauss_noise(int64_t n, float std, uint64_t seed, float* out, fn_stream_t stream);

int64_t fastnerf_compact_ws_ints(int64_t n_points);
int fastnerf_compact_live(int64_t n_points, const float* draw, int32_t* live_idx, int32_t* count_out, int32_t* ws,
                          fn_stream_t stream);
int fastnerf_mlp_bf16_fwd_live(int kind, int64_t n, int S, const float* rays11, const float* z, const float* params,
                               const float* packed_fwd, float* act, const int32_t* live_idx, const int32_t* live_cnt,
                               fn_stream_t stream);
int fastnerf_mlp_bf16_bwd_live(int kind, int64_t n, int S, const float* draw, const float* act, const float* params,
                               const float* packed_bwd, float* dact, float* partial, float* grads,
                               const int32_t* live_idx, const int32_t* live_cnt, fn_stream_t stream);
int fastnerf_mlp_fwd_live_ex(int kind, int64_t n, int S, const float* rays11, const float* z, const float* params,
                             const float* packed_fwd, float* act, const int32_t* live_idx, const int32_t* live_cnt,
                             fn_stream_t stream);
int fastnerf_mlp_bwd_live_ex(int kind, int64_t n, int S, const float* draw, const float* act, const float* params,
                             const float* packed_bwd, float* dact, float* partial, float* grads,
                             const int32_t* live_idx, const int32_t* live_cnt, fn_stream_t stream);
int fastnerf_render_rays_bwd_live(int math_mode, int64_t n, int N_samples, int N_importance, const float* rays11, int white_bkgd,
                                  const float* g_rgb, const float* g_rgb0, const float* noise0, const float* noise1,
                                  const float* z0, const float* raw0, const float* z1, const float* raw1,
                                  const float* params_c, const float* packed_fwd_c, const float* packed_bwd_c,
                                  const float* params_f, const float* packed_fwd_f, const float* packed_bwd_f,
                                  float* draw_ws, float* act_ws, float* dact_ws, float* partial_ws, int32_t* live_ws,
                                  float* grads_c, float* grads_f, int32_t* counts_out, fn_stream_t stream);

typedef struct fn_map_grads {
  const float *g_disp1, *g_acc1, *g_depth1, *g_disp0, *g_acc0, *g_depth0;
} fn_map_grads;
int fastnerf_render_rays_bwd_maps(int math_mode, int64_t n, int N_samples, int N_importance, const float* rays11, int white_bkgd,
                                  const float* g_rgb, const float* g_rgb0, const float* noise0, const float* noise1,
                                  const float* z0, const float* raw0, const float* act0, const float* z1, const float* raw1,
                                  const float* act1, const float* params_c, const float* packed_bwd_c, const float* params_f,
                                  const float* packed_bwd_f, float* draw_ws, float* dact_ws, float* partial_ws, float* grads_c,
                                  float* grads_f, const float* acc0, const float* depth0, const float* acc1, const float* depth1,
                                  const fn_map_grads* maps, fn_stream_t stream);
int fastnerf_render_rays_bwd_live_maps(int math_mode, int64_t n, int N_samples, int N_importance, const float* rays11,
                                       int white_bkgd, const float* g_rgb, const float* g_rgb0, const float* noise0,
                                       const float* noise1, const float* z0, const float* raw0, const float* z1,
                                       const float* raw1, const float* params_c, const float* packed_fwd_c,
                                       const float* packed_bwd_c, const float* params_f, const float* packed_fwd_f,
                                       const float* packed_bwd_f, float* draw_ws, float* act_ws, float* dact_ws,
                                       float* partial_ws, int32_t* live_ws, float* grads_c, float* grads_f, int32_t* counts_out,
                                       const float* acc0, const float* depth0, const float* acc1, const float* depth1,
                                       const fn_map_grads* maps, fn_stream_t stream);

int64_t fastnerf_mlp_x6_packed_floats(int kind, int which);
int fastnerf_mlp_x6_pack(int kind, const float* params, float* packed_fwd, float* packed_bwd, fn_stream_t stream);
int64_t fastnerf_mlp_fold_offset(int kind, int what);
int fastnerf_mlp_x6_fwd(int kind, int64_t n, int S, const float* rays11, const float* z, const float* params,
                        const float* packed_fwd, float* raw, float* act, int flags, fn_stream_t stream);
int fastnerf_mlp_x6_bwd(int kind, int64_t n, int S, const float* draw, const float* act, const float* params,
                        const float* packed_bwd, float* dact, float* partial, float* grads, fn_stream_t stream);
int fastnerf_mlp_x6_fwd_live(int kind, int64_t n, int S, const float* rays11, const float* z, const float* params,
                             const float* packed_fwd, float* act, const int32_t* live_idx, const int32_t* live_cnt,
                             fn_stream_t stream);
int fastnerf_mlp_x6_bwd_live(int kind, int64_t n, int S, const float* draw, const float* act, const float* params,
                             const float* packed_bwd, float* dact, float* partial, float* grads, const int32_t* live_idx,
                             const int32_t* live_cnt, fn_stream_t stream);

#define FN_STEP_FORWARD 1
#define FN_STEP_BWD_FINE 2
#define FN_STEP_BWD_COARSE 4
#define FN_STEP_UPDATE 8
struct fn_occ_grid;
typedef struct fn_step_args {
  int64_t n;
  const float *rays_o, *rays_d, *target;
  const float *t_rand, *u, *noise0, *noise1;
  uint64_t seed0, seed1;
  const int32_t* leaf_tag;
  uint32_t* table;
  int64_t net_floats;
  float *params, *grads, *adam_m, *adam_v;
  float *packed_fwd_c, *packed_bwd_c, *packed_fwd_f, *packed_bwd_f;
  float *rays11, *z0, *raw0, *act0, *rgb0, *disp0, *acc0, *w0, *depth0;
  float *z1, *z_samples, *z_std, *raw1, *act1, *rgb1, *disp1, *acc1, *w1, *depth1;
  float *g_rgb, *g_rgb0, *loss2;
  float *draw_ws, *act_ws, *dact_ws, *partial_ws;
  int32_t *live_ws, *counts;
  double focal, lr, beta1, beta2, eps;
  float near_plane, far_plane, grad_scale;
  int32_t math_mode;
  int32_t N_samples, N_importance, lindisp, perturb, white_bkgd, ndc, H, W;
  int32_t live;
  int32_t fwd_flags;
  int32_t max_leaves, adam_t;
  const struct fn_occ_grid* occ;
  int32_t* occ_counts;
} fn_step_args;
int64_t fastnerf_step_args_size(void);
int fastnerf_train_step(const fn_step_args* args, int phases, fn_stream_t stream);
typedef struct fn_step_aux {
  const float *depth_target, *depth_weight, *acc_target, *acc_weight;
  float *g_depth1, *g_acc1, *g_depth0, *g_acc0, *loss4;
  float lambda_depth, lambda_acc;
} fn_step_aux;
int64_t fastnerf_step_aux_size(void);
int fastnerf_train_step_aux(const fn_step_args* args, const fn_step_aux* aux, int phases, fn_stream_t stream);

#define FASTNERF_COMM_ID_BYTES 128
typedef struct fn_comm fn_comm;
int fastnerf_comm_unique_id(char* id);
int fastnerf_comm_init(fn_comm** out, const char* id, int rank, int world);
int fastnerf_comm_destroy(fn_comm* comm);
int fastnerf_allreduce_grads(fn_comm* comm, float* grads, int64_t n, float scale, fn_stream_t stream);
int fastnerf_allreduce_leaf_table(fn_comm* comm, uint32_t* table, int64_t n, fn_stream_t stream);
int fastnerf_allreduce_leaf_sumcount(fn_comm* comm, double* sum, int32_t* count, int64_t n, fn_stream_t stream);
int fastnerf_leaf_table_reset(uint32_t* table, int64_t n, fn_stream_t stream);
int fastnerf_leaf_table_read(const uint32_t* table, float* host_out, int64_t n, fn_stream_t stream);

#define FASTNERF_MC_TRI_STRIDE 16
int fastnerf_grid_points(int64_t p0, int64_t n, const float* xs, int64_t nx, const float* ys, int64_t ny, const float* zs,
                         int64_t nz, float* rays11, fn_stream_t stream);
int fastnerf_grid_sigma(int64_t n, const float* raw, float* out, fn_stream_t stream);
int64_t fastnerf_mc_ws_bytes(int64_t nx, int64_t ny, int64_t nz);
int fastnerf_mc_count(const float* vol, int64_t nx, int64_t ny, int64_t nz, float thr, void* ws, int64_t* counts_host,
                      fn_stream_t stream);
int fastnerf_mc_emit(const float* vol, int64_t nx, int64_t ny, int64_t nz, float thr, void* ws, float* verts, int32_t* tris,
                     fn_stream_t stream);
int fastnerf_mc_tables(int8_t* tri_host, uint16_t* edge_host);


typedef struct fn_occ_grid {
  const uint32_t* words;
  float lo[3], inv[3];
  int32_t n[3];
  int32_t outside_occupied;
} fn_occ_grid;
int64_t fastnerf_occ_words(int64_t nx, int64_t ny, int64_t nz);
int fastnerf_occ_build(const float* vol, int64_t nx, int64_t ny, int64_t nz, float threshold, int dilate, uint32_t* words,
                       uint32_t* ws, fn_stream_t stream);
int fastnerf_occ_from_mask(const uint8_t* mask, int64_t nx, int64_t ny, int64_t nz, uint32_t* words, fn_stream_t stream);
int fastnerf_occ_query(const fn_occ_grid* grid, int64_t n, const float* pts, uint8_t* out, fn_stream_t stream);
int fastnerf_occ_classify(const fn_occ_grid* grid, int64_t n, int S, const float* rays11, const float* z, int32_t* live_idx,
                          int32_t* count_out, float* raw, int32_t* ws, fn_stream_t stream);
#define FN_OCC_MAX_LEVELS 8
typedef struct fn_occ_cascade {
  int32_t levels;
  int32_t reserved;
  fn_occ_grid level[FN_OCC_MAX_LEVELS];
} fn_occ_cascade;
int fastnerf_occ_query_cascade(const fn_occ_cascade* cascade, int64_t n, const float* pts, uint8_t* out, fn_stream_t stream);
int fastnerf_occ_classify_cascade(const fn_occ_cascade* cascade, int64_t n, int S, const float* rays11, const float* z,
                                  int32_t* live_idx, int32_t* count_out, float* raw, int32_t* ws, fn_stream_t stream);
int fastnerf_occ_cell_points(const fn_occ_grid* grid, int64_t c0, int64_t n, uint64_t seed, float* rays11, fn_stream_t stream);
int fastnerf_occ_update(const float* raw_c, const float* raw_f, int64_t c0, int64_t n, int64_t nx, int64_t ny, int64_t nz,
                        float decay, float threshold, int dilate, float* dens, uint32_t* words, uint32_t* ws, fn_stream_t stream);
int fastnerf_mlp_fwd_list_ex(int kind, int64_t n, int S, const float* rays11, const float* z, const float* params,
                             const float* packed_fwd, float* raw, const int32_t* live_idx, const int32_t* live_cnt, int flags,
                             fn_stream_t stream);
int fastnerf_mlp_bf16_fwd_list(int kind, int64_t n, int S, const float* rays11, const float* z, const float* params,
                               const float* packed_fwd, float* raw, const int32_t* live_idx, const int32_t* live_cnt, int flags,
                               fn_stream_t stream);
int fastnerf_mlp_x6_fwd_list(int kind, int64_t n, int S, const float* rays11, const float* z, const float* params,
                             const float* packed_fwd, float* raw, const int32_t* live_idx, const int32_t* live_cnt, int flags,
                             fn_stream_t stream);
int fastnerf_render_rays_fwd_occ(int math_mode, int64_t n, int N_samples, int N_importance, const float* rays11, int lindisp,
                                 int perturb, int det, int white_bkgd, const float* t_rand, const float* u, uint64_t seed0,
                                 uint64_t seed1, const float* params_c, const float* packed_c, const float* params_f,
                                 const float* packed_f, const fn_occ_grid* grid, int32_t* live_ws, int32_t* counts_out, float* z0,
                                 float* raw0, float* rgb0, float* disp0, float* acc0, float* w0, float* depth0, float* z1,
                                 float* z_samples, float* z_std, float* raw1, float* rgb1, float* disp1, float* acc1, float* w1,
                                 float* depth1, int flags, fn_stream_t stream);
int fastnerf_render_rays_fwd_occ_cascade(int math_mode, int64_t n, int N_samples, int N_importance, const float* rays11, int lindisp,
                                         int perturb, int det, int white_bkgd, const float* t_rand, const float* u, uint64_t seed0,
                                         uint64_t seed1, const float* params_c, const float* packed_c, const float* params_f,
                                         const float* packed_f, const fn_occ_cascade* cascade, int32_t* live_ws, int32_t* counts_out,
                                         float* z0, float* raw0, float* rgb0, float* disp0, float* acc0, float* w0, float* depth0,
                                         float* z1, float* z_samples, float* z_std, float* raw1, float* rgb1, float* disp1,
                                         float* acc1, float* w1, float* depth1, int flags, fn_stream_t stream);

int fastnerf_ert_classify(const fn_occ_grid* grid, const fn_occ_cascade* cascade, int64_t n, int S, int s0, int s1, const float* rays11,
                          const float* z, const float* trans, float eps, int32_t* live_idx, int32_t* count_out, float* raw,
                          int32_t* ws, fn_stream_t stream);
int fastnerf_ert_advance(int64_t n, int S, int s0, int s1, const float* raw, const float* z, const float* rays11, int first,
                         float* trans, const int32_t* seg_count, int32_t* total, fn_stream_t stream);
int fastnerf_render_rays_fwd_ert(int math_mode, int64_t n, int N_samples, int N_importance, const float* rays11, int lindisp,
                                 int perturb, int det, int white_bkgd, const float* t_rand, const float* u, uint64_t seed0,
                                 uint64_t seed1, const float* params_c, const float* packed_c, const float* params_f,
                                 const float* packed_f, const fn_occ_grid* grid, const fn_occ_cascade* cascade, float eps, int block,
                                 float* trans_ws, int32_t* live_ws, int32_t* counts_out, float* z0, float* raw0, float* rgb0,
                                 float* disp0, float* acc0, float* w0, float* depth0, float* z1, float* z_samples, float* z_std,
                                 float* raw1, float* rgb1, float* disp1, float* acc1, float* w1, float* depth1, int flags,
                                 fn_stream_t stream);

int64_t fastnerf_mlp_sigma_grad_ws_floats(int math_mode, int64_t n_points);
int fastnerf_mlp_sigma_grad(int math_mode, int kind, int64_t n, int S, const float* rays11, const float* z, const float* params,
                            const float* packed_fwd, const float* packed_bwd, float* ws, float* sigma, float* grad,
                            fn_stream_t stream);

int64_t fastnerf_ray_grad_ws_floats(int math_mode, int64_t n, int S);
int fastnerf_ray_grad(int math_mode, int kind, int64_t n, int S, const float* rays11, const float* z, const float* raw,
                      const float* noise, const float* draw, const float* act, const float* dact, const float* params, float* ws,
                      int accumulate, float* d_rays, fn_stream_t stream);

#ifdef __cplusplus
}
#endif
#endif
```

Before: 255,300 rays/s.

## Fuse fine composite, MSE loss and backward; pair coarse/fine reduce, unfold and pack launches

Adds a kernel that does the fine-network compositing forward, the MSE gradient and leaf-error table update, and the compositing backward in one pass. The separate mse_leafmax launch and the first fine backward composite launch go away, and the loss sum rides in a spare block of the coarse backward composite. It also merges the coarse and fine gradient reduce, unfold and parameter pack kernels into paired launches. The aim is to cut kernel launch count and re-reads of the ray buffers, at the cost of more complex control flow and duplicated compositing logic that must stay in sync with the existing kernels.

```diff
diff --git a/fast-learning-nerf_amd/_lib.py b/fast-learning-nerf_amd/_lib.py
--- a/fast-learning-nerf_amd/_lib.py
+++ b/fast-learning-nerf_amd/_lib.py
@@ -58,6 +58,8 @@
     'fastnerf_last_error': (C.c_char_p, []),
     'fastnerf_device_cus': (I, []),
     'fastnerf_x6_pair_launches': (L, []),
+    'fastnerf_net_pair_launches': (L, []),
+    'fastnerf_fused_loss_launches': (L, []),
     'fastnerf_gen_rays': (I, [I, I, F, F, F, F, P, P, P, P]),
     'fastnerf_gen_rays_pixels': (I, [L, P, P, F, F, F, F, P, P, P]),
     'fastnerf_ndc_rays': (I, [L, I, I, D, F, P, P, P, P, P]),
diff --git a/fast-learning-nerf_amd/csrc/composite.hip b/fast-learning-nerf_amd/csrc/composite.hip
--- a/fast-learning-nerf_amd/csrc/composite.hip
+++ b/fast-learning-nerf_amd/csrc/composite.hip
@@ -1,3 +1,4 @@
+#include <atomic>
 #include "common.h"
 
 #define WAVE 64
@@ -158,18 +159,14 @@
   }
 }
 
-__global__ void __launch_bounds__(256) raw2outputs_bwd_kernel(int64_t n, int S, const float* __restrict__ raw,
-                                                               const float* __restrict__ z,
-                                                               const float* __restrict__ rays,
-                                                               const float* __restrict__ noise, int white,
-                                                               const float* __restrict__ g_rgb,
-                                                               float* __restrict__ draw, const CompCfg cfg,
-                                                               const float* __restrict__ far,
-                                                               const float* __restrict__ g_lambda) {
+__device__ __forceinline__ void comp_bwd_rays(int64_t n, int S, const float* __restrict__ raw, const float* __restrict__ z,
+                                              const float* __restrict__ rays, const float* __restrict__ noise, int white,
+                                              const float* __restrict__ g_rgb, float* __restrict__ draw, const CompCfg cfg,
+                                              const float* __restrict__ far, const float* __restrict__ g_lambda, int block, int nblocks) {
   const int lane = threadIdx.x & 63;
   const int C = (S + WAVE - 1) / WAVE;
-  const int64_t wave0 = ((int64_t)blockIdx.x * blockDim.x + threadIdx.x) >> 6;
-  const int64_t nwaves = ((int64_t)gridDim.x * blockDim.x) >> 6;
+  const int64_t wave0 = ((int64_t)block * blockDim.x + threadIdx.x) >> 6;
+  const int64_t nwaves = ((int64_t)nblocks * blockDim.x) >> 6;
   for (int64_t r = wave0; r < n; r += nwaves) {
     const float* rr = rays + r * 11;
     const float dnorm = sqrtf(fadd(fadd(fmul(rr[3], rr[3]), fmul(rr[4], rr[4])), fmul(rr[5], rr[5])));
@@ -220,6 +217,191 @@
     for (int j = 0; j < MAXC; ++j)
       if (j < cnt) *reinterpret_cast<float4*>(draw + (r * S + lane * C + j) * 4) = out[j];
   }
+}
+__global__ void __launch_bounds__(256) raw2outputs_bwd_kernel(int64_t n, int S, const float* __restrict__ raw,
+                                                               const float* __restrict__ z,
+                                                               const float* __restrict__ rays,
+                                                               const float* __restrict__ noise, int white,
+                                                               const float* __restrict__ g_rgb,
+                                                               float* __restrict__ draw, const CompCfg cfg,
+                                                               const float* __restrict__ far,
+                                                               const float* __restrict__ g_lambda) {
+  comp_bwd_rays(n, S, raw, z, rays, noise, white, g_rgb, draw, cfg, far, g_lambda, (int)blockIdx.x, (int)gridDim.x);
+}
+
+__global__ void __launch_bounds__(256) raw2outputs_loss_bwd_kernel(
+    int64_t n, int S, const float* __restrict__ raw, const float* __restrict__ z, const float* __restrict__ rays,
+    const float* __restrict__ noise, int white, float* __restrict__ rgb_map, float* __restrict__ disp, float* __restrict__ acc,
+    float* __restrict__ weights, float* __restrict__ depth, const float* __restrict__ rgb0, const float* __restrict__ target, float gscale,
+    float* __restrict__ g_rgb, float* __restrict__ g_rgb0, const int32_t* __restrict__ tag,
+    int max_leaves, uint32_t* __restrict__ table, float* __restrict__ draw) {
+  const CompCfg cfg = nerf_cfg();
+  const int lane = threadIdx.x & 63;
+  const int C = (S + WAVE - 1) / WAVE;
+  const int64_t wave0 = ((int64_t)blockIdx.x * blockDim.x + threadIdx.x) >> 6;
+  const int64_t nwaves = ((int64_t)gridDim.x * blockDim.x) >> 6;
+  for (int64_t r = wave0; r < n; r += nwaves) {
+    const float* rr = rays + r * 11;
+    const float dnorm = sqrtf(fadd(fadd(fmul(rr[3], rr[3]), fmul(rr[4], rr[4])), fmul(rr[5], rr[5])));
+    SampleVals v[MAXC];
+    int cnt;
+    eval_chunk<true>(S, C, lane, raw + r * S * 4, z + r * S, noise ? noise + r * S : nullptr, dnorm, v, cnt, cfg, 0.f);
+    float prod = 1.0f;
+#pragma unroll
+    for (int j = 0; j < MAXC; ++j)
+      if (j < cnt) prod *= v[j].t;
+    const float incl = wave_scan_mul(prod, lane);
+    float T0 = __shfl_up(incl, 1, WAVE);
+    if (lane == 0) T0 = 1.0f;
+    float w[MAXC], Tj[MAXC];
+    float sr = 0.f, sg = 0.f, sb = 0.f, sd = 0.f, sa = 0.f;
+    float T = T0;
+#pragma unroll
+    for (int j = 0; j < MAXC; ++j) {
+      if (j < cnt) {
+        Tj[j] = T;
+        w[j] = v[j].alpha * T;
+        if (weights) weights[r * S + lane * C + j] = w[j];
+        sr += w[j] * v[j].c[0];
+        sg += w[j] * v[j].c[1];
+        sb += w[j] * v[j].c[2];
+        sd += w[j] * v[j].z;
+        sa += w[j];
+        T *= v[j].t;
+      }
+    }
+    sr = wave_sum(sr); sg = wave_sum(sg); sb = wave_sum(sb); sd = wave_sum(sd); sa = wave_sum(sa);
+    float g0 = 0.f, g1 = 0.f, g2 = 0.f;
+    if (lane == 0) {
+      if (white) {
+        const float bg = fsub(1.0f, sa);
+        sr = fadd(sr, bg); sg = fadd(sg, bg); sb = fadd(sb, bg);
+      }
+      rgb_map[r * 3 + 0] = sr; rgb_map[r * 3 + 1] = sg; rgb_map[r * 3 + 2] = sb;
+      if (disp) {
+        const float q = sd / sa;
+        disp[r] = (q != q) ? q : 1.0f / fmaxf(1e-10f, q);
+      }
+      if (acc) acc[r] = sa;
+      if (depth) depth[r] = sd;
+      const float px[3] = {sr, sg, sb};
+      float gg[3];
+      float emax = 0.f;
+#pragma unroll
+      for (int c = 0; c < 3; ++c) {
+        const float t = target[r * 3 + c];
+        const float d = fsub(px[c], t);
+        gg[c] = gscale * d;
+        g_rgb[r * 3 + c] = gg[c];
+        emax = fmaxf(emax, fabsf(fsub(t, px[c])));
+        g_rgb0[r * 3 + c] = gscale * fsub(rgb0[r * 3 + c], t);
+      }
+      if (table && tag) {
+        const int64_t slot = (int64_t)tag[r * 2] * max_leaves + tag[r * 2 + 1];
+        atomicMax(table + slot, __float_as_uint(emax));
+      }
+      g0 = gg[0]; g1 = gg[1]; g2 = gg[2];
+    }
+    g0 = __shfl(g0, 0, WAVE); g1 = __shfl(g1, 0, WAVE); g2 = __shfl(g2, 0, WAVE);
+    const float gbg = white ? (g0 + g1 + g2) : 0.0f;
+    const float lam_term = 0.0f;
+    float G[MAXC];
+    float gw_chunk = 0.f;
+#pragma unroll
+    for (int j = 0; j < MAXC; ++j) {
+      if (j < cnt) {
+        G[j] = g0 * v[j].c[0] + g1 * v[j].c[1] + g2 * v[j].c[2] - gbg;
+        gw_chunk += G[j] * w[j];
+      }
+    }
+    float suffix = wave_suffix_add(gw_chunk, lane);
+    float4 out[MAXC];
+#pragma unroll
+    for (int j = MAXC - 1; j >= 0; --j) {
+      if (j < cnt) {
+        const float dalpha = G[j] * Tj[j] - (suffix + lam_term) / v[j].t;
+        const float dact = dalpha * v[j].dist * (1.0f - v[j].alpha);
+        out[j].x = g0 * w[j] * v[j].c[0] * (1.0f - v[j].c[0]);
+        out[j].y = g1 * w[j] * v[j].c[1] * (1.0f - v[j].c[1]);
+        out[j].z = g2 * w[j] * v[j].c[2] * (1.0f - v[j].c[2]);
+        out[j].w = (v[j].sig > 0.0f) ? dact : 0.0f;
+        suffix += G[j] * w[j];
+      }
+    }
+#pragma unroll
+    for (int j = 0; j < MAXC; ++j)
+      if (j < cnt) *reinterpret_cast<float4*>(draw + (r * S + lane * C + j) * 4) = out[j];
+  }
+}
+
+__device__ __forceinline__ void loss_pair_block(int64_t n, const float* __restrict__ rgb_map, const float* __restrict__ rgb0,
+                                                const float* __restrict__ target, float inv_count, float* __restrict__ loss2) {
+  __shared__ float red[16];
+  const int lane = threadIdx.x & 63;
+  const int wave = threadIdx.x >> 6;
+  float se[4], se0[4];
+#pragma unroll
+  for (int q = 0; q < 4; ++q) { se[q] = 0.f; se0[q] = 0.f; }
+  for (int64_t i0 = 0; i0 < n; i0 += 1024) {
+    float t[4][3], x[4][3], x0[4][3];
+#pragma unroll
+    for (int q = 0; q < 4; ++q) {
+      const int64_t i = i0 + (wave * 4 + q) * 64 + lane;
+#pragma unroll
+      for (int c = 0; c < 3; ++c) {
+        t[q][c] = i < n ? target[i * 3 + c] : 0.f;
+        x[q][c] = i < n ? rgb_map[i * 3 + c] : 0.f;
+        x0[q][c] = i < n ? rgb0[i * 3 + c] : 0.f;
+      }
+    }
+#pragma unroll
+    for (int q = 0; q < 4; ++q) {
+      if (i0 + (wave * 4 + q) * 64 + lane < n) {
+#pragma unroll
+        for (int c = 0; c < 3; ++c) {
+          const float d = fsub(x[q][c], t[q][c]);
+          se[q] += d * d;
+          const float d0 = fsub(x0[q][c], t[q][c]);
+          se0[q] += d0 * d0;
+        }
+      }
+    }
+  }
+  float tot[2];
+#pragma unroll
+  for (int which = 0; which < 2; ++which) {
+#pragma unroll
+    for (int q = 0; q < 4; ++q) {
+      float x = which ? se0[q] : se[q];
+#pragma unroll
+      for (int o = 32; o > 0; o >>= 1) x += __shfl_xor(x, o, WAVE);
+      if (lane == 0) red[wave * 4 + q] = x;
+    }
+    __syncthreads();
+    float t = (threadIdx.x < 16) ? red[threadIdx.x] : 0.f;
+    if (wave == 0) {
+#pragma unroll
+      for (int o = 1; o < 16; o <<= 1) t += __shfl_xor(t, o, WAVE);
+    }
+    __syncthreads();
+    tot[which] = t;
+  }
+  if (threadIdx.x == 0) {
+    loss2[0] = tot[0] * inv_count;
+    loss2[1] = tot[1] * inv_count;
+  }
+}
+
+__global__ void __launch_bounds__(256) raw2outputs_bwd_loss_kernel(int64_t n, int S, const float* __restrict__ raw, const float* __restrict__ z,
+                                                                    const float* __restrict__ rays, const float* __restrict__ noise, int white,
+                                                                    const float* __restrict__ g_rgb, float* __restrict__ draw,
+                                                                    const float* __restrict__ rgb_map, const float* __restrict__ rgb0,
+                                                                    const float* __restrict__ target, float inv_count, float* __restrict__ loss2) {
+  if (blockIdx.x == 0) {
+    loss_pair_block(n, rgb_map, rgb0, target, inv_count, loss2);
+    return;
+  }
+  comp_bwd_rays(n, S, raw, z, rays, noise, white, g_rgb, draw, nerf_cfg(), nullptr, nullptr, (int)blockIdx.x - 1, (int)gridDim.x - 1);
 }
 
 __global__ void __launch_bounds__(256) raw2outputs_bwd_full_kernel(
@@ -511,6 +693,43 @@
   return 0;
 }
 
+namespace fn {
+static std::atomic<int64_t> g_fused_loss_launches{0};
+
+bool fused_loss_enabled() {
+  const char* e = getenv("FASTNERF_FUSED_LOSS");
+  return !(e && e[0] == '0');
+}
+
+int raw2outputs_loss_bwd(int64_t n, int S, const float* raw, const float* z, const float* rays11, const float* noise, int white_bkgd,
+                         float* rgb_map, float* disp, float* acc, float* weights, float* depth, const float* rgb0, const float* target,
+                         float grad_scale, float* g_rgb, float* g_rgb0, const int32_t* leaf_tag, int max_leaves, uint32_t* table, float* draw,
+                         fn_stream_t stream) {
+  FN_CHECK_ARG(n > 0 && n <= 65536 && S >= 1 && S <= WAVE * MAXC, "0<n<=65536, 1<=S<=512");
+  FN_CHECK_ARG(raw && z && rays11 && rgb_map && rgb0 && target && g_rgb && g_rgb0 && draw, "null pointer");
+  FN_CHECK_ARG(!(table && !leaf_tag) && (!table || max_leaves > 0), "table needs leaf_tag and max_leaves>0");
+  const float gscale = (float)(2.0 / (3.0 * (double)n) * (double)grad_scale);
+  hipLaunchKernelGGL(raw2outputs_loss_bwd_kernel, dim3(grid_waves(n)), dim3(256), 0, fn::S(stream), n, S, raw, z, rays11, noise, white_bkgd,
+                     rgb_map, disp, acc, weights, depth, rgb0, target, gscale, g_rgb, g_rgb0, leaf_tag, max_leaves, table, draw);
+  FN_LAUNCH_CHECK();
+  g_fused_loss_launches.fetch_add(1, std::memory_order_relaxed);
+  return 0;
+}
+
+int raw2outputs_bwd_loss(int64_t n, int S, const float* raw, const float* z, const float* rays11, const float* noise, int white_bkgd,
+                         const float* g_rgb, float* draw, const float* rgb_map, const float* rgb0, const float* target, float* loss2,
+                         fn_stream_t stream) {
+  FN_CHECK_ARG(n > 0 && n <= 65536 && S >= 1 && S <= WAVE * MAXC, "0<n<=65536, 1<=S<=512");
+  FN_CHECK_ARG(raw && z && rays11 && g_rgb && draw && rgb_map && rgb0 && target && loss2, "null pointer");
+  const float inv_count = (float)(1.0 / (3.0 * (double)n));
+  hipLaunchKernelGGL(raw2outputs_bwd_loss_kernel, dim3(grid_waves(n) + 1), dim3(256), 0, fn::S(stream), n, S, raw, z, rays11, noise, white_bkgd,
+                     g_rgb, draw, rgb_map, rgb0, target, inv_count, loss2);
+  FN_LAUNCH_CHECK();
+  return 0;
+}
+}
+extern "C" int64_t fastnerf_fused_loss_launches(void) { return fn::g_fused_loss_launches.load(std::memory_order_relaxed); }
+
 extern "C" int fastnerf_raw2outputs_bwd_full(int64_t n, int S, const float* raw, const float* z, const float* rays11,
                                              const float* noise, int white_bkgd, const float* acc, const float* depth,
                                              const float* g_rgb, const float* g_disp, const float* g_acc, const float* g_w,
diff --git a/fast-learning-nerf_amd/csrc/dw_pair.h b/fast-learning-nerf_amd/csrc/dw_pair.h
--- a/fast-learning-nerf_amd/csrc/dw_pair.h
+++ b/fast-learning-nerf_amd/csrc/dw_pair.h
@@ -51,6 +51,11 @@
   int n;
 };
 
+namespace fn {
+bool net_pair_enabled();
+void net_pair_count(int launches);
+}
+
 struct DwDeferred {
   DwTrunk J;
   RedTable T;
diff --git a/fast-learning-nerf_amd/csrc/mlp_bwd_dw.hip b/fast-learning-nerf_amd/csrc/mlp_bwd_dw.hip
--- a/fast-learning-nerf_amd/csrc/mlp_bwd_dw.hip
+++ b/fast-learning-nerf_amd/csrc/mlp_bwd_dw.hip
@@ -504,9 +504,8 @@
 }
 
 
-__global__ void __launch_bounds__(256) reduce_all_kernel(RedTable tab, const float* __restrict__ partial, float* __restrict__ grads,
-                                                          float* __restrict__ scratch, int64_t P, const int* __restrict__ live_cnt, int ncu) {
-  RedSeg sg = tab.s[blockIdx.y];
+__device__ __forceinline__ void reduce_seg(RedSeg sg, const float* __restrict__ partial, float* __restrict__ grads, float* __restrict__ scratch,
+                                           int64_t P, const int* __restrict__ live_cnt, int ncu) {
   if (sg.dyn) {
     if (live_cnt) P = (int64_t)*live_cnt;
     const int n = sg.dyn == 2 ? head_rows(P) : dw_trunk_chunks(P, ncu);
@@ -538,11 +537,34 @@
   }
 }
 
-__global__ void __launch_bounds__(256) unfold_kernel(const float* __restrict__ G, const float* __restrict__ params, float* __restrict__ grads,
-                                                      int64_t VW, int64_t VB, int64_t FW, int64_t FB) {
+__global__ void __launch_bounds__(256) reduce_all_kernel(RedTable tab, const float* __restrict__ partial, float* __restrict__ grads,
+                                                          float* __restrict__ scratch, int64_t P, const int* __restrict__ live_cnt, int ncu) {
+  reduce_seg(tab.s[blockIdx.y], partial, grads, scratch, P, live_cnt, ncu);
+}
+
+#define PAIR_SEGS 24
+struct RedNet {
+  float *partial, *grads;
+  const float* params;
+  int64_t P, g_off, VW, VB, FW, FB;
+  int n;
+};
+struct RedPair {
+  RedSeg s[2][PAIR_SEGS];
+  RedNet net[2];
+};
+__global__ void __launch_bounds__(256) reduce_all_pair_kernel(RedPair A, int ncu) {
+  int y = (int)blockIdx.y;
+  const int k = y >= A.net[0].n ? 1 : 0;
+  if (k) y -= A.net[0].n;
+  const RedNet& N = A.net[k];
+  reduce_seg(A.s[k][y], N.partial, N.grads, N.partial, N.P, nullptr, ncu);
+}
+
+__device__ __forceinline__ void unfold_block(const int b, const float* __restrict__ G, const float* __restrict__ params, float* __restrict__ grads,
+                                             int64_t VW, int64_t VB, int64_t FW, int64_t FB) {
   __shared__ double As[16][17], Bs[16][17];
   const int tx = threadIdx.x & 15, ty = threadIdx.x >> 4;
-  const int b = blockIdx.x;
   if (b == 384) {
     const int i = threadIdx.x;
     double s = 0.0;
@@ -569,6 +591,16 @@
   }
   if (wf) grads[FW + (int64_t)(r0 + ty) * 256 + c0 + tx] = (float)s;
   else grads[VW + (int64_t)(r0 + ty) * 283 + c0 + tx] = (float)fma((double)grads[VB + r0 + ty], (double)params[FB + c0 + tx], s);
+}
+#define UNFOLD_BLOCKS 385
+__global__ void __launch_bounds__(256) unfold_kernel(const float* __restrict__ G, const float* __restrict__ params, float* __restrict__ grads,
+                                                      int64_t VW, int64_t VB, int64_t FW, int64_t FB) {
+  unfold_block((int)blockIdx.x, G, params, grads, VW, VB, FW, FB);
+}
+__global__ void __launch_bounds__(256) unfold_pair_kernel(RedNet n0, RedNet n1) {
+  const int k = blockIdx.x >= UNFOLD_BLOCKS ? 1 : 0;
+  const RedNet& N = k ? n1 : n0;
+  unfold_block((int)blockIdx.x - k * UNFOLD_BLOCKS, N.partial + N.g_off, N.params, N.grads, N.VW, N.VB, N.FW, N.FB);
 }
 
 extern "C" int64_t fastnerf_mlp_bwd_partial_floats(void) {
@@ -629,7 +661,7 @@
                       const int* live_cnt, int ncu, hipStream_t st) {
   hipLaunchKernelGGL(reduce_all_kernel, dim3(256, T.n), dim3(256), 0, st, T, partial, grads, partial, P, live_cnt, ncu);
   FN_LAUNCH_CHECK();
-  hipLaunchKernelGGL(unfold_kernel, dim3(385), dim3(256), 0, st, partial + g_off, params, grads, L.VW, L.VB, L.FW, L.FB);
+  hipLaunchKernelGGL(unfold_kernel, dim3(UNFOLD_BLOCKS), dim3(256), 0, st, partial + g_off, params, grads, L.VW, L.VB, L.FW, L.FB);
   FN_LAUNCH_CHECK();
   return 0;
 }
@@ -763,6 +795,12 @@
 
 namespace fn {
 static std::atomic<int64_t> g_pair_launches{0};
+static std::atomic<int64_t> g_net_pair_launches{0};
+bool net_pair_enabled() {
+  const char* e = getenv("FASTNERF_PAIR_NETS");
+  return !(e && e[0] == '0');
+}
+void net_pair_count(int launches) { g_net_pair_launches.fetch_add(launches, std::memory_order_relaxed); }
 
 bool x6_pair_workspace(int64_t P_coarse, fn_stream_t stream, float** dact2, float** partial2) {
   static const WsName what = {
@@ -799,12 +837,27 @@
   hipLaunchKernelGGL(mlp_bwd_dw6_trunk_pair_kernel, dim3(nwg), dim3(512), DW_TRUNK_LDS, st, A, ncu);
   FN_LAUNCH_CHECK();
   g_pair_launches.fetch_add(1, std::memory_order_relaxed);
+  if (net_pair_enabled() && fine->T.n <= PAIR_SEGS && coarse->T.n <= PAIR_SEGS) {
+    RedPair R;
+    for (int k = 0; k < 2; ++k) {
+      const NetLayout& L = layout_of(d[k]->kind);
+      for (int i = 0; i < d[k]->T.n; ++i) R.s[k][i] = d[k]->T.s[i];
+      R.net[k] = RedNet{d[k]->partial, d[k]->grads, d[k]->params, d[k]->P, d[k]->g_off, L.VW, L.VB, L.FW, L.FB, d[k]->T.n};
+    }
+    hipLaunchKernelGGL(reduce_all_pair_kernel, dim3(256, R.net[0].n + R.net[1].n), dim3(256), 0, st, R, ncu);
+    FN_LAUNCH_CHECK();
+    hipLaunchKernelGGL(unfold_pair_kernel, dim3(2 * UNFOLD_BLOCKS), dim3(256), 0, st, R.net[0], R.net[1]);
+    FN_LAUNCH_CHECK();
+    net_pair_count(2);
+    return 0;
+  }
   for (int k = 0; k < 2; ++k)
     if (int rc = bwd_reduce(d[k]->T, layout_of(d[k]->kind), d[k]->P, d[k]->params, d[k]->partial, d[k]->grads, d[k]->g_off, nullptr, ncu, st)) return rc;
   return 0;
 }
 }
 extern "C" int64_t fastnerf_x6_pair_launches(void) { return fn::g_pair_launches.load(std::memory_order_relaxed); }
+extern "C" int64_t fastnerf_net_pair_launches(void) { return fn::g_net_pair_launches.load(std::memory_order_relaxed); }
 
 static int bwd_launch(int kind, int64_t n, int S, const float* draw, const float* act, const float* params,
                       const float* packed_bwd, float* dact, float* partial, float* grads, const int* live_idx,
diff --git a/fast-learning-nerf_amd/csrc/mlp_pack.hip b/fast-learning-nerf_amd/csrc/mlp_pack.hip
--- a/fast-learning-nerf_amd/csrc/mlp_pack.hip
+++ b/fast-learning-nerf_amd/csrc/mlp_pack.hip
@@ -1,4 +1,5 @@
 #include "mlp_common.h"
+#include "dw_pair.h"
 
 struct PackDesc {
   int64_t src_off;
@@ -17,8 +18,8 @@
   int64_t m_off;
 };
 
-__global__ void __launch_bounds__(256) fold_kernel(const float* __restrict__ params, int64_t VW, int64_t VB, int64_t FW, int64_t FB,
-                                                    float* __restrict__ m_out, float* __restrict__ b_out, bool slack) {
+__device__ __forceinline__ void fold_block(const float* __restrict__ params, int64_t VW, int64_t VB, int64_t FW, int64_t FB,
+                                           float* __restrict__ m_out, float* __restrict__ b_out, bool slack) {
   const int e = blockIdx.x * 256 + threadIdx.x;
   if (e < 128 * 256) {
     const int o = e >> 8, j = e & 255;
@@ -37,6 +38,20 @@
     b_out[o] = (float)s;
     if (slack && o < 128 / 2) b_out[128 + o] = 0.f;
   }
+}
+__global__ void __launch_bounds__(256) fold_kernel(const float* __restrict__ params, int64_t VW, int64_t VB, int64_t FW, int64_t FB,
+                                                    float* __restrict__ m_out, float* __restrict__ b_out, bool slack) {
+  fold_block(params, VW, VB, FW, FB, m_out, b_out, slack);
+}
+struct PackNets {
+  const float* params[2];
+  float* pf[2];
+  float* pb[2];
+};
+__global__ void __launch_bounds__(256) fold_pair_kernel(PackNets N, int64_t VW, int64_t VB, int64_t FW, int64_t FB, int64_t m_off, int64_t b_off,
+                                                         bool slack) {
+  const int k = (int)blockIdx.y;
+  fold_block(N.params[k], VW, VB, FW, FB, N.pf[k] + m_off, N.pf[k] + b_off, slack);
 }
 static void launch_fold(const NetLayout& L, const float* params, float* packed_fwd, bool x6, hipStream_t st) {
   hipLaunchKernelGGL(fold_kernel, dim3(129), dim3(256), 0, st, params, L.VW, L.VB, L.FW, L.FB, packed_fwd + fold_plain(L.PFR, x6),
@@ -79,8 +94,7 @@
   }
 }
 
-__global__ void __launch_bounds__(256) pack6_kernel(PackTable tab, const float* __restrict__ params,
-                                                     uint4* pf, uint4* __restrict__ pb) {
+__device__ __forceinline__ void pack6_block(const PackTable& tab, const float* __restrict__ params, uint4* pf, uint4* __restrict__ pb) {
   const PackDesc d = tab.d[blockIdx.y];
   constexpr int TW = 16, KW = 32;
   const int KS = (d.transposed ? d.n_rows : d.n_cols) / KW;
@@ -120,6 +134,14 @@
     o[128] = make_uint4(lo[0], lo[1], lo[2], lo[3]);
   }
 }
+__global__ void __launch_bounds__(256) pack6_kernel(PackTable tab, const float* __restrict__ params,
+                                                     uint4* pf, uint4* __restrict__ pb) {
+  pack6_block(tab, params, pf, pb);
+}
+__global__ void __launch_bounds__(256) pack6_pair_kernel(PackTable tab, PackNets N) {
+  const int k = (int)blockIdx.z;
+  pack6_block(tab, N.params[k], reinterpret_cast<uint4*>(N.pf[k]), reinterpret_cast<uint4*>(N.pb[k]));
+}
 
 static PackTable make_pack_table(const NetLayout& L, bool x6) {
   PackTable T;
@@ -182,13 +204,30 @@
   const NetLayout& L = layout_of(kind);
   return (which == 1 ? L.pf_total : L.pb_total) * 3 / 2;
 }
+static const PackTable& x6_pack_table(int kind) {
+  static const PackTable T[3] = {make_pack_table(layout_of(0), true), make_pack_table(layout_of(1), true),
+                                 make_pack_table(layout_of(2), true)};
+  return T[kind];
+}
+namespace fn {
+int x6_pack_pair(int kind, const float* params_a, float* pf_a, float* pb_a, const float* params_b, float* pf_b, float* pb_b, fn_stream_t stream) {
+  FN_CHECK_ARG(kind >= 0 && kind <= 2 && params_a && pf_a && pb_a && params_b && pf_b && pb_b, "kind in 0..2, non-null pointers");
+  const NetLayout& L = layout_of(kind);
+  const PackNets N = {{params_a, params_b}, {pf_a, pf_b}, {pb_a, pb_b}};
+  hipLaunchKernelGGL(fold_pair_kernel, dim3(129, 2), dim3(256), 0, S(stream), N, L.VW, L.VB, L.FW, L.FB, fold_plain(L.PFR, true),
+                     fold_plain(L.PFB, true), true);
+  FN_LAUNCH_CHECK();
+  hipLaunchKernelGGL(pack6_pair_kernel, dim3(32, N_PACK, 2), dim3(256), 0, S(stream), x6_pack_table(kind), N);
+  FN_LAUNCH_CHECK();
+  net_pair_count(2);
+  return 0;
+}
+}
 extern "C" int fastnerf_mlp_x6_pack(int kind, const float* params, float* packed_fwd, float* packed_bwd, fn_stream_t stream) {
   FN_CHECK_ARG(kind >= 0 && kind <= 2 && params && packed_fwd && packed_bwd, "kind in 0..2, non-null pointers");
-  static const PackTable T[3] = {make_pack_table(layout_of(0), true), make_pack_table(layout_of(1), true),
-                                 make_pack_table(layout_of(2), true)};
   launch_fold(layout_of(kind), params, packed_fwd, true, fn::S(stream));
   FN_LAUNCH_CHECK();
-  hipLaunchKernelGGL(pack6_kernel, dim3(32, N_PACK), dim3(256), 0, fn::S(stream), T[kind], params,
+  hipLaunchKernelGGL(pack6_kernel, dim3(32, N_PACK), dim3(256), 0, fn::S(stream), x6_pack_table(kind), params,
                      reinterpret_cast<uint4*>(packed_fwd), reinterpret_cast<uint4*>(packed_bwd));
   FN_LAUNCH_CHECK();
   return 0;
diff --git a/fast-learning-nerf_amd/csrc/render.cpp b/fast-learning-nerf_amd/csrc/render.cpp
--- a/fast-learning-nerf_amd/csrc/render.cpp
+++ b/fast-learning-nerf_amd/csrc/render.cpp
@@ -10,6 +10,15 @@
 int x6_pair_pass(DwDeferred* d, int64_t n, int S, const float* draw, const float* act, const float* params, const float* packed_bwd,
                  float* dact, float* partial, float* grads, fn_stream_t stream);
 int x6_pair_finish(const DwDeferred* fine, const DwDeferred* coarse, fn_stream_t stream);
+int x6_pack_pair(int kind, const float* params_a, float* pf_a, float* pb_a, const float* params_b, float* pf_b, float* pb_b, fn_stream_t stream);
+bool fused_loss_enabled();
+int raw2outputs_loss_bwd(int64_t n, int S, const float* raw, const float* z, const float* rays11, const float* noise, int white_bkgd,
+                         float* rgb_map, float* disp, float* acc, float* weights, float* depth, const float* rgb0, const float* target,
+                         float grad_scale, float* g_rgb, float* g_rgb0, const int32_t* leaf_tag, int max_leaves, uint32_t* table, float* draw,
+                         fn_stream_t stream);
+int raw2outputs_bwd_loss(int64_t n, int S, const float* raw, const float* z, const float* rays11, const float* noise, int white_bkgd,
+                         const float* g_rgb, float* draw, const float* rgb_map, const float* rgb0, const float* target, float* loss2,
+                         fn_stream_t stream);
 }
 
 struct MlpMode {
@@ -46,6 +55,19 @@
      fastnerf_mlp_x6_bwd_live},
 };
 
+struct FusedLoss {
+  const float* target;
+  float grad_scale;
+  float *g_rgb, *g_rgb0;
+  const int32_t* leaf_tag;
+  int max_leaves;
+  uint32_t* table;
+  float* draw;
+};
+struct LossTail {
+  const float *rgb1, *rgb0, *target;
+  float* loss2;
+};
 struct RrFwd {
   const char* fname;
   int math_mode;
@@ -59,6 +81,7 @@
   float *z0, *raw0, *rgb0, *disp0, *acc0, *w0, *depth0, *z1, *z_samples, *z_std, *raw1, *rgb1, *disp1, *acc1, *w1, *depth1;
   int flags;
   fn_stream_t stream;
+  const FusedLoss* fused;
 };
 
 static bool rr_fwd_scalars(const RrFwd& a) {
@@ -96,8 +119,34 @@
                                       a.stream)))
     return rc;
   if ((rc = net(1, S1, a.z1, a.params_f, a.packed_f, a.raw1, a.noise1))) return rc;
+  if (const FusedLoss* f = a.fused)
+    return fn::raw2outputs_loss_bwd(a.n, S1, a.raw1, a.z1, a.rays11, a.noise1, a.white_bkgd, a.rgb1, a.disp1, a.acc1, a.w1, a.depth1, a.rgb0,
+                                    f->target, f->grad_scale, f->g_rgb, f->g_rgb0, f->leaf_tag, f->max_leaves, f->table, f->draw, a.stream);
   return fastnerf_raw2outputs_fwd(a.n, S1, a.raw1, a.z1, a.rays11, a.noise1, a.white_bkgd, a.rgb1, a.disp1, a.acc1, a.w1, a.depth1,
                                   a.stream);
+}
+
+static int rr_fwd_plain(int math_mode, int64_t n, int N_samples, int N_importance, const float* rays11,
+                        int lindisp, int perturb, int det, int white_bkgd, const float* t_rand, const float* u,
+                        const float* noise0, const float* noise1, uint64_t seed0, uint64_t seed1,
+                        const float* params_c, const float* packed_c, const float* params_f,
+                        const float* packed_f, float* z0, float* raw0, float* act0, float* rgb0,
+                        float* disp0, float* acc0, float* w0, float* depth0, float* z1,
+                        float* z_samples, float* z_std, float* raw1, float* act1, float* rgb1,
+                        float* disp1, float* acc1, float* w1, float* depth1, int flags, const FusedLoss* fused, fn_stream_t stream) {
+  const RrFwd a = {"fastnerf_render_rays_fwd", math_mode, n, N_samples, N_importance, rays11, lindisp, perturb, det, white_bkgd, t_rand,
+                   u, noise0, noise1, seed0, seed1, params_c, packed_c, params_f, packed_f, z0, raw0, rgb0, disp0, acc0, w0, depth0, z1,
+                   z_samples, z_std, raw1, rgb1, disp1, acc1, w1, depth1, flags, stream, fused};
+  if (!rr_fwd_scalars(a)) return -1;
+  if (n == 0) return 0;
+  if (!rr_fwd_coarse_ptrs(a)) {
+    fn::set_error("%s: null pointer (coarse pass)", a.fname);
+    return -1;
+  }
+  return rr_fwd_chain(a, [&](int pass, int S, const float* z, const float* params, const float* packed, float* raw, const float* noise) {
+    float* act = pass ? act1 : act0;
+    return modes[math_mode].fwd(0, n, S, rays11, z, params, packed, raw, act, (!act && !noise) ? flags : 0, stream);
+  });
 }
 
 extern "C" int fastnerf_render_rays_fwd_ex(int math_mode, int64_t n, int N_samples, int N_importance, const float* rays11,
@@ -108,19 +157,9 @@
                                         float* disp0, float* acc0, float* w0, float* depth0, float* z1,
                                         float* z_samples, float* z_std, float* raw1, float* act1, float* rgb1,
                                         float* disp1, float* acc1, float* w1, float* depth1, int flags, fn_stream_t stream) {
-  const RrFwd a = {"fastnerf_render_rays_fwd", math_mode, n, N_samples, N_importance, rays11, lindisp, perturb, det, white_bkgd, t_rand,
-                   u, noise0, noise1, seed0, seed1, params_c, packed_c, params_f, packed_f, z0, raw0, rgb0, disp0, acc0, w0, depth0, z1,
-                   z_samples, z_std, raw1, rgb1, disp1, acc1, w1, depth1, flags, stream};
-  if (!rr_fwd_scalars(a)) return -1;
-  if (n == 0) return 0;
-  if (!rr_fwd_coarse_ptrs(a)) {
-    fn::set_error("%s: null pointer (coarse pass)", a.fname);
-    return -1;
-  }
-  return rr_fwd_chain(a, [&](int pass, int S, const float* z, const float* params, const float* packed, float* raw, const float* noise) {
-    float* act = pass ? act1 : act0;
-    return modes[math_mode].fwd(0, n, S, rays11, z, params, packed, raw, act, (!act && !noise) ? flags : 0, stream);
-  });
+  return rr_fwd_plain(math_mode, n, N_samples, N_importance, rays11, lindisp, perturb, det, white_bkgd, t_rand, u, noise0, noise1, seed0,
+                      seed1, params_c, packed_c, params_f, packed_f, z0, raw0, act0, rgb0, disp0, acc0, w0, depth0, z1, z_samples, z_std,
+                      raw1, act1, rgb1, disp1, acc1, w1, depth1, flags, nullptr, stream);
 }
 
 static int rr_fwd_occ(const RrFwd& a, const fn_occ_grid* grid, const fn_occ_cascade* cascade, int32_t* live_ws, int32_t* counts_out) {
@@ -277,7 +316,13 @@
                   const float* packed_bwd_c, const float* params_f, const float* packed_bwd_f,
                   float* draw_ws, float* dact_ws, float* partial_ws, float* grads_c, float* grads_f,
                   const float* acc0, const float* depth0, const float* acc1, const float* depth1, const fn_map_grads* mg,
-                  int passes, fn_stream_t stream) {
+                  int passes, fn_stream_t stream, bool fine_draw_done = false, const LossTail* tail = nullptr) {
+  auto comp_coarse = [&](const float* g, const PassMaps& m) {
+    if (tail && !m.any())
+      return fn::raw2outputs_bwd_loss(n, N_samples, raw0, z0, rays11, noise0, white_bkgd, g, draw_ws, tail->rgb1, tail->rgb0, tail->target,
+                                      tail->loss2, stream);
+    return comp_bwd(n, N_samples, raw0, z0, rays11, noise0, white_bkgd, g, m, draw_ws, stream);
+  };
   if (math_mode < 0 || math_mode > 2 || n <= 0 || N_samples < 2 || N_importance < 0) {
     fn::set_error("fastnerf_render_rays_bwd: bad argument: math_mode in {0,1,2}, n>0, N_samples>=2, N_importance>=0");
     return -1;
@@ -307,14 +352,14 @@
     float *dact2 = nullptr, *partial2 = nullptr;
     if (passes == 3 && math_mode == 2 && fn::x6_pair_workspace(n * (int64_t)N_samples, stream, &dact2, &partial2)) {
       DwDeferred d_fine, d_coarse;
-      if ((rc = comp_bwd(n, S1, raw1, z1, rays11, noise1, white_bkgd, g_rgb, m_fine, draw_ws, stream))) return rc;
+      if (!fine_draw_done && (rc = comp_bwd(n, S1, raw1, z1, rays11, noise1, white_bkgd, g_rgb, m_fine, draw_ws, stream))) return rc;
       if ((rc = fn::x6_pair_pass(&d_fine, n, S1, draw_ws, act1, params_f, packed_bwd_f, dact_ws, partial_ws, grads_f, stream))) return rc;
-      if ((rc = comp_bwd(n, N_samples, raw0, z0, rays11, noise0, white_bkgd, g_rgb0, m_coarse, draw_ws, stream))) return rc;
+      if ((rc = comp_coarse(g_rgb0, m_coarse))) return rc;
       if ((rc = fn::x6_pair_pass(&d_coarse, n, N_samples, draw_ws, act0, params_c, packed_bwd_c, dact2, partial2, grads_c, stream))) return rc;
       return fn::x6_pair_finish(&d_fine, &d_coarse, stream);
     }
     if (passes & 1) {
-      if ((rc = comp_bwd(n, S1, raw1, z1, rays11, noise1, white_bkgd, g_rgb, m_fine, draw_ws, stream))) return rc;
+      if (!fine_draw_done && (rc = comp_bwd(n, S1, raw1, z1, rays11, noise1, white_bkgd, g_rgb, m_fine, draw_ws, stream))) return rc;
       if ((rc = mlp(S1, act1, params_f, packed_bwd_f, grads_f))) return rc;
     }
     g_coarse = g_rgb0;
@@ -328,7 +373,7 @@
     return -1;
   }
   if (!(passes & 2)) return 0;
-  if ((rc = comp_bwd(n, N_samples, raw0, z0, rays11, noise0, white_bkgd, g_coarse, m_coarse, draw_ws, stream))) return rc;
+  if ((rc = comp_coarse(g_coarse, m_coarse))) return rc;
   return mlp(N_samples, act0, params_c, packed_bwd_c, grads_c);
 }
 
@@ -478,6 +523,8 @@
   float* grads_f = two ? a->grads + a->net_floats : nullptr;
   const float* g_fine = two ? a->g_rgb : nullptr;
   int rc;
+  bool fused = false;
+  bool loss_rides = false;
   if (phases & FN_STEP_FORWARD) {
     if (!a->rays_o || !a->rays_d || !a->target || !a->rays11 || !a->g_rgb || (two && !a->g_rgb0) || !a->loss2) {
       fn::set_error("fastnerf_train_step: null batch / output buffer");
@@ -486,6 +533,10 @@
     if ((rc = fastnerf_pack_rays(a->n, a->rays_o, a->rays_d, a->near_plane, a->far_plane, a->ndc, a->H, a->W, a->focal, a->rays11,
                                  stream))) return rc;
     const bool save = !a->live;
+    const FusedLoss fl = {a->target, a->grad_scale, a->g_rgb, a->g_rgb0, a->leaf_tag, a->max_leaves, a->table, a->draw_ws};
+    fused = two && save && !a->occ && !aux && (phases & FN_STEP_BWD_FINE) && a->n <= 65536 && a->N_samples + a->N_importance <= 512 &&
+            a->draw_ws && !(a->table && !a->leaf_tag) && (!a->table || a->max_leaves > 0) && fn::fused_loss_enabled();
+    loss_rides = fused && (phases & FN_STEP_BWD_COARSE);
     if (a->occ) {
       if ((rc = fastnerf_render_rays_fwd_occ(a->math_mode, a->n, a->N_samples, a->N_importance, a->rays11, a->lindisp,
                                              (a->perturb || a->t_rand) ? 1 : 0, a->perturb ? 0 : 1, a->white_bkgd, a->t_rand, a->u,
@@ -494,15 +545,18 @@
                                              a->disp0, a->acc0, a->w0, a->depth0, a->z1, a->z_samples, a->z_std, a->raw1, a->rgb1,
                                              a->disp1, a->acc1, a->w1, a->depth1, a->fwd_flags, stream)))
         return rc;
-    } else if ((rc = fastnerf_render_rays_fwd_ex(a->math_mode, a->n, a->N_samples, a->N_importance, a->rays11, a->lindisp,
-                                          (a->perturb || a->t_rand) ? 1 : 0, a->perturb ? 0 : 1, a->white_bkgd, a->t_rand, a->u,
-                                          a->noise0, a->noise1, a->seed0, a->seed1, params_c, a->packed_fwd_c, params_f,
-                                          a->packed_fwd_f, a->z0, a->raw0, save ? a->act0 : nullptr, a->rgb0, a->disp0, a->acc0,
-                                          a->w0, a->depth0, a->z1, a->z_samples, a->z_std, a->raw1, save ? a->act1 : nullptr,
-                                          a->rgb1, a->disp1, a->acc1, a->w1, a->depth1, save ? 0 : a->fwd_flags, stream)))
+    } else if ((rc = rr_fwd_plain(a->math_mode, a->n, a->N_samples, a->N_importance, a->rays11, a->lindisp,
+                                  (a->perturb || a->t_rand) ? 1 : 0, a->perturb ? 0 : 1, a->white_bkgd, a->t_rand, a->u,
+                                  a->noise0, a->noise1, a->seed0, a->seed1, params_c, a->packed_fwd_c, params_f,
+                                  a->packed_fwd_f, a->z0, a->raw0, save ? a->act0 : nullptr, a->rgb0, a->disp0, a->acc0,
+                                  a->w0, a->depth0, a->z1, a->z_samples, a->z_std, a->raw1, save ? a->act1 : nullptr,
+                                  a->rgb1, a->disp1, a->acc1, a->w1, a->depth1, save ? 0 : a->fwd_flags, fused ? &fl : nullptr, stream)))
       return rc;
-    if ((rc = fastnerf_mse_leafmax(a->n, two ? a->rgb1 : a->rgb0, two ? a->rgb0 : nullptr, a->target, a->grad_scale, a->g_rgb,
+    if (!fused && (rc = fastnerf_mse_leafmax(a->n, two ? a->rgb1 : a->rgb0, two ? a->rgb0 : nullptr, a->target, a->grad_scale, a->g_rgb,
                                    two ? a->g_rgb0 : nullptr, a->loss2, a->leaf_tag, a->max_leaves, a->table, stream)))
+      return rc;
+    if (fused && !loss_rides && (rc = fastnerf_mse_leafmax(a->n, a->rgb1, a->rgb0, a->target, a->grad_scale, nullptr, nullptr, a->loss2, nullptr,
+                                                         0, nullptr, stream)))
       return rc;
     if (aux && (rc = fastnerf_aux_loss(a->n, two ? a->depth1 : a->depth0, two ? a->acc1 : a->acc0, two ? a->depth0 : nullptr,
                                        two ? a->acc0 : nullptr, aux->depth_target, aux->depth_weight, aux->acc_target,
@@ -524,6 +578,7 @@
       if (aux->acc_target) { mg.g_acc1 = aux->g_acc1; mg.g_acc0 = two ? aux->g_acc0 : nullptr; }
     }
     const fn_map_grads* mgp = aux ? &mg : nullptr;
+    const LossTail tail = {a->rgb1, a->rgb0, a->target, a->loss2};
     if (a->live)
       rc = rr_bwd_live(a->math_mode, a->n, a->N_samples, a->N_importance, a->rays11, a->white_bkgd, g_a, g_b, a->noise0, a->noise1,
                        a->z0, a->raw0, a->z1, a->raw1, params_c, a->packed_fwd_c, a->packed_bwd_c, params_f, a->packed_fwd_f,
@@ -532,7 +587,7 @@
     else
       rc = rr_bwd(a->math_mode, a->n, a->N_samples, a->N_importance, a->rays11, a->white_bkgd, g_a, g_b, a->noise0, a->noise1, a->z0,
                   a->raw0, a->act0, a->z1, a->raw1, a->act1, params_c, a->packed_bwd_c, params_f, a->packed_bwd_f, a->draw_ws,
-                  a->dact_ws, a->partial_ws, grads_c, grads_f, a->acc0, a->depth0, a->acc1, a->depth1, mgp, passes, stream);
+                  a->dact_ws, a->partial_ws, grads_c, grads_f, a->acc0, a->depth0, a->acc1, a->depth1, mgp, passes, stream, fused, loss_rides ? &tail : nullptr);
     if (rc) return rc;
   }
   if (phases & FN_STEP_UPDATE) {
@@ -543,6 +598,8 @@
     const int64_t total = a->net_floats * (two ? 2 : 1);
     if ((rc = fastnerf_adam_step(total, a->params, a->grads, a->adam_m, a->adam_v, a->lr, a->beta1, a->beta2, a->eps, a->adam_t,
                                  stream))) return rc;
+    if (two && a->math_mode == 2 && fn::net_pair_enabled())
+      return fn::x6_pack_pair(0, params_c, a->packed_fwd_c, a->packed_bwd_c, params_f, a->packed_fwd_f, a->packed_bwd_f, stream);
     if ((rc = modes[a->math_mode].pack(0, params_c, a->packed_fwd_c, a->packed_bwd_c, stream))) return rc;
     if (two && (rc = modes[a->math_mode].pack(0, params_f, a->packed_fwd_f, a->packed_bwd_f, stream))) return rc;
   }
diff --git a/include/fastnerf.h b/include/fastnerf.h
--- a/include/fastnerf.h
+++ b/include/fastnerf.h
@@ -11,6 +11,8 @@
 const char* fastnerf_last_error(void);
 int fastnerf_device_cus(void);
 int64_t fastnerf_x6_pair_launches(void);
+int64_t fastnerf_net_pair_launches(void);
+int64_t fastnerf_fused_loss_launches(void);
 
 int fastnerf_gen_rays(int H, int W, float fx, float fy, float cx, float cy, const float* c2w_host,
                       float* rays_o, float* rays_d, fn_stream_t stream);
```

Result: no change. 255,600 rays/s (median of 4 runs) (+0.1%).
